# wuer5/OMGSR

Measured on AMD Instinct MI355X. Metric: SR images/sec, higher is better.
Workload: dtype fp16; 1 GPU; OMGSR-S 256->1024, batch=4/GPU, accurate tier (fp32 stream, fp16 MFMA operands + split corrections), tiled VAE 256/64; global_batch=4, latent_tile=64, tile_overlap=32, world_size=1, parallelism=dp1, weights=seeded random, SD2.1-base shapes

## Files before the change

include/omgsr_hip.h:

```cpp
#ifndef OMGSR_HIP_H
#define OMGSR_HIP_H

#include <stdint.h>

#ifdef __cplusplus
extern "C" {
#endif

#define OMGSR_E_BADARG (-1)
#define OMGSR_E_SHAPE (-2)
#define OMGSR_E_ARCH (-3)

#define OMGSR_ACT_NONE 0
#define OMGSR_ACT_SILU 1
#define OMGSR_ACT_GELU_TANH 2
#define OMGSR_ACT_GEGLU 3

#define OMGSR_OUT_BF16 0
#define OMGSR_OUT_F32 1

#define OMGSR_LAYOUT_NHWC 0
#define OMGSR_LAYOUT_T 1

#define OMGSR_EL_16 0
#define OMGSR_EL_F32 1
#define OMGSR_EL_SPLIT 2
#define OMGSR_EL_MX 3
#define OMGSR_EL_MX6 4
#define OMGSR_EL_MXFP8 5

#define OMGSR_DT_BF16 0
#define OMGSR_DT_F16 1
int omgsr_set_compute_dtype(int dtype);
int omgsr_get_compute_dtype(void);

int omgsr_abi_version(void);
int omgsr_check_device(void);
const char* omgsr_error_string(int code);

typedef struct omgsr_igemm_args {
    const void* in;
    const void* weight;
    const float* bias;
    const float* gate;
    const void* residual;
    void* out;
    int32_t N, H, W, Cin;
    int32_t Cout;
    int32_t Cout_pad, K_pad;
    int32_t R, S, stride, pad_top, pad_left, upsample;
    int32_t Ho, Wo;
    int32_t act, out_dtype, out_layout;
    int32_t t_rows, t_ld;
    int32_t out_ld;
    int32_t batch;
    int64_t in_bstride, w_bstride, out_bstride;
    float alpha;
    const void* weight_cm;
    void* workspace;
    float* gn_partial;
    int32_t gn_groups;
    int32_t gn_entries;
    int32_t res_el;
    int32_t in_split;
    int64_t sample_rows;
    int32_t out_lo_off;
    int32_t in_ld;
    int32_t w_split;
    const void* weight_ph;
    int32_t mx_chunks16;
    int32_t mx_scale_w1, mx_scale_a1, mx_scale_w2, mx_scale_a2;
    int32_t out_mx;
    int32_t group_tiles;
    uint32_t* overflow_flag;
    const float* gn_scale_shift;
    int32_t gn_nimg;
    int32_t gn_act;
    int32_t in_el;
    int32_t mx_fmt;
    int32_t mxf8;
    int32_t mxf8_reserved;
    const uint8_t* in_scale;
    const uint8_t* w_scale;
} omgsr_igemm_args;
int32_t omgsr_igemm_gn_fusable(const omgsr_igemm_args* a);
int32_t omgsr_igemm_out_mx6_ok(const omgsr_igemm_args* a);
int omgsr_groupnorm_scale_shift(const float* mean, const float* rstd, const float* gamma, const float* beta, float* out, int32_t nimg, int32_t C,
                                int32_t G, void* stream);
int omgsr_igemm(const omgsr_igemm_args* a, void* stream);
int omgsr_igemm_multi_plan(omgsr_igemm_args* args, int32_t count);
int omgsr_igemm_multi(const omgsr_igemm_args* args, int32_t count, void* stream);
int omgsr_set_batch_invariant(int on);
int64_t omgsr_igemm_workspace_bytes(const omgsr_igemm_args* a);
int32_t omgsr_igemm_gn_slots(const omgsr_igemm_args* a);
int32_t omgsr_igemm_gn_entries(const omgsr_igemm_args* a);

int omgsr_groupnorm_nchunk(int64_t HW);
int omgsr_groupnorm_stats(const void* x, float* partial, float* mean, float* rstd, float* var_out,
                          int32_t N, int64_t HW, int32_t C, int32_t G, float eps, int32_t x_el, void* stream);
int omgsr_groupnorm_finalize(const float* partial, float* mean, float* rstd, float* var_out, int32_t N,
                             int32_t nslot, int32_t G, int32_t entries, double count, float eps, void* stream);
int omgsr_groupnorm_partial(const void* x, float* partial, int32_t N, int64_t HW, int32_t C, int32_t G, int32_t x_el, void* stream);
#define OMGSR_GN_MAX_GROUPS 8
typedef struct omgsr_gn_merge_args {
    const float* partial[OMGSR_GN_MAX_GROUPS];
    double count[OMGSR_GN_MAX_GROUPS];
    float weight[OMGSR_GN_MAX_GROUPS];
    int32_t tiles[OMGSR_GN_MAX_GROUPS];
    int32_t nslot[OMGSR_GN_MAX_GROUPS];
    int32_t entries[OMGSR_GN_MAX_GROUPS];
    int32_t ngroups;
} omgsr_gn_merge_args;
int omgsr_groupnorm_finalize_merged(const omgsr_gn_merge_args* a, float* mean, float* rstd, float* var_out,
                                    int32_t N, int32_t G, float eps, void* stream);
int omgsr_groupnorm_apply(const void* x, void* y, const float* mean, const float* rstd,
                          const float* gamma, const float* beta, int32_t N, int64_t HW, int32_t C,
                          int32_t G, int32_t act, int32_t x_el, int32_t y_el, void* y2, int32_t y2_el, uint32_t* overflow_flag, void* stream);
int omgsr_groupnorm_apply_shared(const void* x, void* y, const float* mean, const float* rstd,
                                 const float* gamma, const float* beta, int32_t rows, int64_t HW, int32_t C,
                                 int32_t G, int32_t act, int32_t stat_rows, int32_t x_el, int32_t y_el, void* y2, int32_t y2_el,
                                 uint32_t* overflow_flag, void* stream);

int omgsr_layernorm(const void* x, void* y, const float* a, const float* b, int64_t rows, int32_t C,
                    float eps, int32_t x_el, int32_t y_el, void* stream);
int omgsr_quantize_mxfp8(const void* x, int32_t x_el, int64_t rows, int32_t K, int64_t x_ld, void* codes, void* scales, void* stream);
int omgsr_to_operand(const float* x, void* y, int64_t rows, int32_t C, int32_t y_el, uint32_t* overflow_flag, void* stream);
int omgsr_transpose_split(const float* x, void* y, int32_t B, int32_t L, int32_t C, int64_t ld, void* stream);

typedef struct omgsr_attn_args {
    const void* q; const void* k; const void* vt; void* o;
    int32_t B, H, D, Lq, Lk;
    int64_t q_ld, k_ld, vt_ld, o_ld;
    int64_t q_bstride, k_bstride, vt_bstride, o_bstride;
    float scale;
    int32_t o_lo_off;
    int32_t o_mx;
    int32_t q_lo_off;
    int32_t k_lo_off;
    int32_t p_split;
    int32_t reserved1;
    int64_t vt_lo_off;
    int32_t qkv_el;
    int32_t qkv_reserved;
    const uint8_t* q_scale;
    const uint8_t* k_scale;
    const uint8_t* vt_scale;
    int64_t q_sld, k_sld, vt_sld;
    int64_t q_sbstride, k_sbstride, vt_sbstride;
} omgsr_attn_args;
int omgsr_set_attention_defer_max(float log2_threshold);
int omgsr_attention(const omgsr_attn_args* a, void* stream);

int omgsr_softmax_rows(const float* s, void* p, int64_t rows, int32_t L, int32_t Lvalid, void* stream);
int omgsr_softmax_rows_split(const float* s, void* p, int64_t rows, int32_t L, int32_t Lvalid, void* stream);

int omgsr_rmsnorm_rope(void* x, const float* w, const float* w2, int32_t Lsplit, const float* cos_t, const float* sin_t, int32_t B,
                       int32_t L, int32_t H, int32_t D, int64_t ld, int32_t col0, int32_t pos0,
                       float eps, void* stream);
int omgsr_rmsnorm_rope_mxfp8(const void* x, const float* w, const float* w2, int32_t Lsplit, const float* cos_t, const float* sin_t, int32_t B,
                             int32_t L, int32_t H, int32_t D, int64_t ld, int32_t col0, int32_t pos0, float eps, void* codes, void* scales,
                             int64_t c_ld, int64_t s_ld, void* stream);

int omgsr_nchw_to_nhwc(const void* src, void* dst, int32_t N, int32_t C, int32_t H, int32_t W,
                       int32_t Cpad, int32_t src_dtype, int32_t dst_el, void* stream);
int omgsr_nhwc_to_nchw(const void* src, void* dst, int32_t N, int32_t C, int32_t H, int32_t W,
                       int32_t ld, int32_t dst_dtype, int32_t do_clamp, float lo, float hi, int32_t src_el, void* stream);
int omgsr_copy_channels(const void* src, void* dst, int64_t rows, int32_t C, int32_t src_ld,
                        int32_t dst_ld, int32_t dst_off, int32_t el, void* stream);
int omgsr_vae_sample(const void* moments, const float* eps, void* z, int64_t rows, int32_t C,
                     int32_t ld_out, float shift, float scale, int32_t el, void* stream);
int omgsr_axpby(const void* x, const void* y, void* out, int64_t n, float a, float b, float c, float d,
                int32_t bf16_steps, int32_t el, void* stream);
int omgsr_linear_f32(const float* x, const float* w, const float* b, float* y, int32_t rows, int32_t K, int32_t N,
                     int32_t silu_in, void* stream);
int omgsr_tile_accumulate(const void* tile, const float* w, float* acc, int32_t N, int32_t C,
                          int32_t th, int32_t tw, int32_t tile_ld, int32_t H, int32_t W, int32_t y0,
                          int32_t x0, int32_t tile_el, void* stream);
int omgsr_tile_normalise(const float* acc, const float* wsum, void* out, int32_t N, int64_t HW,
                         int32_t C, int32_t ld, int32_t out_el, void* stream);
int omgsr_crop_nhwc(const void* src, void* dst, int32_t N, int32_t H, int32_t W, int32_t C, int32_t y0,
                    int32_t x0, int32_t th, int32_t tw, int32_t el, void* stream);
int omgsr_paste_nhwc(const void* src, void* dst, int32_t N, int32_t C, int32_t sH, int32_t sW, int32_t sy0,
                     int32_t sx0, int32_t dH, int32_t dW, int32_t dy0, int32_t dx0, int32_t th, int32_t tw,
                     int32_t el, void* stream);
int omgsr_resize_nearest_exact_nhwc(const void* src, void* dst, int32_t N, int32_t H, int32_t W, int32_t C, int32_t Ho, int32_t Wo,
                                    float scale_y, float scale_x, int32_t el, void* stream);
int omgsr_flux_pack(const void* src, void* dst, int32_t N, int32_t H, int32_t W, int32_t C, int32_t ld,
                    int32_t dir, int32_t el, void* stream);

int omgsr_image_to_model_input(const uint8_t* img_hwc3, void* out_nhwc8, int32_t N, int32_t H, int32_t W, int32_t out_el, void* stream);
#define OMGSR_COLORFIX_NONE 0
#define OMGSR_COLORFIX_ADAIN 1
#define OMGSR_COLORFIX_WAVELET 2
int64_t omgsr_colorfix_workspace_bytes(int32_t N, int32_t H, int32_t W, int32_t method);
int omgsr_colorfix(const void* sr_nhwc, int32_t sr_ld, const uint8_t* src_hwc3, uint8_t* out_hwc3, void* workspace,
                   int32_t N, int32_t H, int32_t W, int32_t method, int32_t sr_el, void* stream);

int omgsr_resample_u8(const uint8_t* src, uint8_t* dst, const int32_t* bounds, const int32_t* kk, int32_t ksize,
                      int32_t N, int32_t Hin, int32_t Win, int32_t out_size, int32_t axis, void* stream);

int omgsr_timing_enable(int on);
int omgsr_timing_reset(void);
typedef struct omgsr_timing_entry { int32_t kind; float ms; double flops; double bytes; int64_t m, n, k; int32_t variant; int32_t stage; } omgsr_timing_entry;
int omgsr_timing_collect(omgsr_timing_entry* out, int cap);
int omgsr_timing_stage(int stage);
int omgsr_mfma_peak(int32_t iters, float* tflops, void* stream);

#ifdef __cplusplus
}
#endif
#endif
```

omgsr_amd/_lib.py:

```python
from __future__ import annotations

import ctypes as C
import os

import torch

from .build import lib_path

ABI_VERSION = 20


class OmgsrError(RuntimeError):
    pass


class IgemmArgs(C.Structure):
    _fields_ = [
        ("in_", C.c_void_p), ("weight", C.c_void_p), ("bias", C.c_void_p), ("gate", C.c_void_p),
        ("residual", C.c_void_p), ("out", C.c_void_p),
        ("N", C.c_int32), ("H", C.c_int32), ("W", C.c_int32), ("Cin", C.c_int32),
        ("Cout", C.c_int32), ("Cout_pad", C.c_int32), ("K_pad", C.c_int32),
        ("R", C.c_int32), ("S", C.c_int32), ("stride", C.c_int32), ("pad_top", C.c_int32),
        ("pad_left", C.c_int32), ("upsample", C.c_int32),
        ("Ho", C.c_int32), ("Wo", C.c_int32),
        ("act", C.c_int32), ("out_dtype", C.c_int32), ("out_layout", C.c_int32),
        ("t_rows", C.c_int32), ("t_ld", C.c_int32), ("out_ld", C.c_int32),
        ("batch", C.c_int32),
        ("in_bstride", C.c_int64), ("w_bstride", C.c_int64), ("out_bstride", C.c_int64),
        ("alpha", C.c_float), ("weight_cm", C.c_void_p), ("workspace", C.c_void_p),
        ("gn_partial", C.c_void_p), ("gn_groups", C.c_int32), ("gn_entries", C.c_int32),
        ("res_el", C.c_int32), ("in_split", C.c_int32), ("sample_rows", C.c_int64), ("out_lo_off", C.c_int32),
        ("in_ld", C.c_int32), ("w_split", C.c_int32), ("weight_ph", C.c_void_p), ("mx_chunks16", C.c_int32), ("mx_scale_w1", C.c_int32), ("mx_scale_a1", C.c_int32),
        ("mx_scale_w2", C.c_int32), ("mx_scale_a2", C.c_int32), ("out_mx", C.c_int32), ("group_tiles", C.c_int32), ("overflow_flag", C.c_void_p),
        ("gn_scale_shift", C.c_void_p), ("gn_nimg", C.c_int32), ("gn_act", C.c_int32), ("in_el", C.c_int32), ("mx_fmt", C.c_int32),
        ("mxf8", C.c_int32), ("mxf8_reserved", C.c_int32), ("in_scale", C.c_void_p), ("w_scale", C.c_void_p),
    ]


GN_MAX_GROUPS = 8


class GnMergeArgs(C.Structure):
    _fields_ = [("partial", C.c_void_p * GN_MAX_GROUPS), ("count", C.c_double * GN_MAX_GROUPS),
                ("weight", C.c_float * GN_MAX_GROUPS), ("tiles", C.c_int32 * GN_MAX_GROUPS),
                ("nslot", C.c_int32 * GN_MAX_GROUPS), ("entries", C.c_int32 * GN_MAX_GROUPS), ("ngroups", C.c_int32)]


class AttnArgs(C.Structure):
    _fields_ = [
        ("q", C.c_void_p), ("k", C.c_void_p), ("vt", C.c_void_p), ("o", C.c_void_p),
        ("B", C.c_int32), ("H", C.c_int32), ("D", C.c_int32), ("Lq", C.c_int32), ("Lk", C.c_int32),
        ("q_ld", C.c_int64), ("k_ld", C.c_int64), ("vt_ld", C.c_int64), ("o_ld", C.c_int64),
        ("q_bstride", C.c_int64), ("k_bstride", C.c_int64), ("vt_bstride", C.c_int64), ("o_bstride", C.c_int64),
        ("scale", C.c_float), ("o_lo_off", C.c_int32), ("o_mx", C.c_int32), ("q_lo_off", C.c_int32), ("k_lo_off", C.c_int32), ("p_split", C.c_int32),
        ("reserved1", C.c_int32), ("vt_lo_off", C.c_int64),
        ("qkv_el", C.c_int32), ("qkv_reserved", C.c_int32), ("q_scale", C.c_void_p), ("k_scale", C.c_void_p), ("vt_scale", C.c_void_p),
        ("q_sld", C.c_int64), ("k_sld", C.c_int64), ("vt_sld", C.c_int64), ("q_sbstride", C.c_int64), ("k_sbstride", C.c_int64),
        ("vt_sbstride", C.c_int64),
    ]


class TimingEntry(C.Structure):
    _fields_ = [("kind", C.c_int32), ("ms", C.c_float), ("flops", C.c_double), ("bytes", C.c_double),
                ("m", C.c_int64), ("n", C.c_int64), ("k", C.c_int64), ("variant", C.c_int32), ("stage", C.c_int32)]


_P, _I, _L, _F = C.c_void_p, C.c_int32, C.c_int64, C.c_float

SIGNATURES = {
    "omgsr_abi_version": (C.c_int, []),
    "omgsr_check_device": (C.c_int, []),
    "omgsr_set_compute_dtype": (C.c_int, [C.c_int]),
    "omgsr_get_compute_dtype": (C.c_int, []),
    "omgsr_error_string": (C.c_char_p, [C.c_int]),
    "omgsr_igemm": (C.c_int, [C.POINTER(IgemmArgs), _P]),
    "omgsr_igemm_multi_plan": (C.c_int, [C.POINTER(IgemmArgs), _I]),
    "omgsr_igemm_multi": (C.c_int, [C.POINTER(IgemmArgs), _I, _P]),
    "omgsr_set_batch_invariant": (C.c_int, [C.c_int]),
    "omgsr_set_attention_defer_max": (C.c_int, [C.c_float]),
    "omgsr_igemm_workspace_bytes": (C.c_int64, [C.POINTER(IgemmArgs)]),
    "omgsr_igemm_gn_slots": (C.c_int32, [C.POINTER(IgemmArgs)]),
    "omgsr_igemm_gn_entries": (C.c_int32, [C.POINTER(IgemmArgs)]),
    "omgsr_igemm_gn_fusable": (C.c_int32, [C.POINTER(IgemmArgs)]),
    "omgsr_igemm_out_mx6_ok": (C.c_int32, [C.POINTER(IgemmArgs)]),
    "omgsr_groupnorm_scale_shift": (C.c_int, [_P, _P, _P, _P, _P, _I, _I, _I, _P]),
    "omgsr_groupnorm_finalize": (C.c_int, [_P, _P, _P, _P, _I, _I, _I, _I, C.c_double, _F, _P]),
    "omgsr_groupnorm_partial": (C.c_int, [_P, _P, _I, _L, _I, _I, _I, _P]),
    "omgsr_groupnorm_finalize_merged": (C.c_int, [C.POINTER(GnMergeArgs), _P, _P, _P, _I, _I, _F, _P]),
    "omgsr_groupnorm_apply_shared": (C.c_int, [_P, _P, _P, _P, _P, _P, _I, _L, _I, _I, _I, _I, _I, _I, _P, _I, _P, _P]),
    "omgsr_image_to_model_input": (C.c_int, [_P, _P, _I, _I, _I, _I, _P]),
    "omgsr_colorfix_workspace_bytes": (C.c_int64, [_I, _I, _I, _I]),
    "omgsr_colorfix": (C.c_int, [_P, _I, _P, _P, _P, _I, _I, _I, _I, _I, _P]),
    "omgsr_groupnorm_nchunk": (C.c_int, [_L]),
    "omgsr_groupnorm_stats": (C.c_int, [_P, _P, _P, _P, _P, _I, _L, _I, _I, _F, _I, _P]),
    "omgsr_groupnorm_apply": (C.c_int, [_P, _P, _P, _P, _P, _P, _I, _L, _I, _I, _I, _I, _I, _P, _I, _P, _P]),
    "omgsr_layernorm": (C.c_int, [_P, _P, _P, _P, _L, _I, _F, _I, _I, _P]),
    "omgsr_resize_nearest_exact_nhwc": (C.c_int, [_P, _P, _I, _I, _I, _I, _I, _I, _F, _F, _I, _P]),
    "omgsr_transpose_split": (C.c_int, [_P, _P, _I, _I, _I, _L, _P]),
    "omgsr_to_operand": (C.c_int, [_P, _P, _L, _I, _I, _P, _P]),
    "omgsr_quantize_mxfp8": (C.c_int, [_P, _I, _L, _I, _L, _P, _P, _P]),
    "omgsr_attention": (C.c_int, [C.POINTER(AttnArgs), _P]),
    "omgsr_softmax_rows": (C.c_int, [_P, _P, _L, _I, _I, _P]),
    "omgsr_softmax_rows_split": (C.c_int, [_P, _P, _L, _I, _I, _P]),
    "omgsr_rmsnorm_rope": (C.c_int, [_P, _P, _P, _I, _P, _P, _I, _I, _I, _I, _L, _I, _I, _F, _P]),
    "omgsr_rmsnorm_rope_mxfp8": (C.c_int, [_P, _P, _P, _I, _P, _P, _I, _I, _I, _I, _L, _I, _I, _F, _P, _P, _L, _L, _P]),
    "omgsr_nchw_to_nhwc": (C.c_int, [_P, _P, _I, _I, _I, _I, _I, _I, _I, _P]),
    "omgsr_nhwc_to_nchw": (C.c_int, [_P, _P, _I, _I, _I, _I, _I, _I, _I, _F, _F, _I, _P]),
    "omgsr_copy_channels": (C.c_int, [_P, _P, _L, _I, _I, _I, _I, _I, _P]),
    "omgsr_vae_sample": (C.c_int, [_P, _P, _P, _L, _I, _I, _F, _F, _I, _P]),
    "omgsr_axpby": (C.c_int, [_P, _P, _P, _L, _F, _F, _F, _F, _I, _I, _P]),
    "omgsr_linear_f32": (C.c_int, [_P, _P, _P, _P, _I, _I, _I, _I, _P]),
    "omgsr_tile_accumulate": (C.c_int, [_P, _P, _P, _I, _I, _I, _I, _I, _I, _I, _I, _I, _I, _P]),
    "omgsr_tile_normalise": (C.c_int, [_P, _P, _P, _I, _L, _I, _I, _I, _P]),
    "omgsr_crop_nhwc": (C.c_int, [_P, _P, _I, _I, _I, _I, _I, _I, _I, _I, _I, _P]),
    "omgsr_paste_nhwc": (C.c_int, [_P, _P] + [_I] * 13 + [_P]),
    "omgsr_flux_pack": (C.c_int, [_P, _P, _I, _I, _I, _I, _I, _I, _I, _P]),
    "omgsr_resample_u8": (C.c_int, [_P, _P, _P, _P, _I, _I, _I, _I, _I, _I, _P]),
    "omgsr_timing_enable": (C.c_int, [C.c_int]),
    "omgsr_timing_reset": (C.c_int, []),
    "omgsr_timing_stage": (C.c_int, [C.c_int]),
    "omgsr_timing_collect": (C.c_int, [C.POINTER(TimingEntry), C.c_int]),
    "omgsr_mfma_peak": (C.c_int, [_I, C.POINTER(C.c_float), _P]),
}

_lib = None


def load(path: str | None = None):
    global _lib
    if _lib is not None:
        return _lib
    path = path or os.environ.get("OMGSR_HIP_LIB") or lib_path()
    if not os.path.isfile(path):
        raise OmgsrError(
            f"{path} not found: build it with `python -m omgsr_amd.build` (hipcc --offload-arch=gfx950). "
            "The OMGSR MI355X path has no CPU fallback.")
    lib = C.CDLL(path)
    for name, (res, args) in SIGNATURES.items():
        try:
            fn = getattr(lib, name)
        except AttributeError as e:
            raise OmgsrError(f"{path} does not export {name}") from e
        fn.restype = res
        fn.argtypes = args
    if lib.omgsr_abi_version() != ABI_VERSION:
        raise OmgsrError(f"ABI mismatch: library {lib.omgsr_abi_version()} vs binding {ABI_VERSION}; rebuild")
    _lib = lib
    return lib


def check(code: int, what: str = "") -> None:
    if code != 0:
        msg = load().omgsr_error_string(code)
        raise OmgsrError(f"{what}: {msg.decode() if msg else code} (code {code})")
```

omgsr_amd/csrc/elementwise.hip:

```cpp
#include "common.hip.h"
#include "../../include/omgsr_hip.h"
#include "timing.hip.h"
#include <string.h>
#include <type_traits>

namespace omgsr {
TimingState& timing_state() { static TimingState s; return s; }
static int g_compute_dtype = 0;
int compute_dtype() { return g_compute_dtype; }
}

namespace {

template <typename T> OMGSR_DEVINL float round_to(float x) { return (float)(T)x; }

template <typename SRC, typename T, int DEL>
__global__ void nchw_to_nhwc_kernel(const SRC* __restrict__ src, void* __restrict__ dst, int N, int C, int64_t HW, int Cpad) {
    const int ng = Cpad >> 3;
    const int64_t i = (int64_t)blockIdx.x * blockDim.x + threadIdx.x;
    const int64_t total = (int64_t)N * HW * ng;
    if (i >= total) return;
    const int g = (int)(i % ng);
    const int64_t pix = i / ng;
    const int n = (int)(pix / HW);
// ... 60 lines not shown
    __shared__ float tile[64][65];
    const int b = blockIdx.z, l0 = blockIdx.x * 64, c0 = blockIdx.y * 64;
    const float* xb = x + (int64_t)b * L * C;
    for (int i = threadIdx.x; i < 64 * 64; i += 256) {
        const int l = i >> 6, c = i & 63;
        tile[l][c] = (l0 + l < L && c0 + c < C) ? xb[(int64_t)(l0 + l) * C + c0 + c] : 0.0f;
    }
    __syncthreads();
    T* yb = y + (int64_t)b * 2 * C * ld;
    for (int i = threadIdx.x; i < 64 * 8; i += 256) {
        const int c = i >> 3, g = (i & 7) * 8;
        if (c0 + c >= C || l0 + g >= L) continue;
        float hi[8], lo[8];
#pragma unroll
        for (int e = 0; e < 8; ++e) {
            const float v = tile[g + e][c];
            const T h = (T)v;
            hi[e] = (float)h;
            lo[e] = v - hi[e];
        }
        T* dh = yb + (int64_t)(c0 + c) * ld + l0 + g;
        T* dl = dh + (int64_t)C * ld;
        if (l0 + g + 8 <= L) {
            *reinterpret_cast<u32x4_t*>(dh) = pack8<T>(hi);
            *reinterpret_cast<u32x4_t*>(dl) = pack8<T>(lo);
        } else {
            for (int e = 0; e < 8 && l0 + g + e < L; ++e) { dh[e] = (T)hi[e]; dl[e] = (T)lo[e]; }
        }
    }
}

template <typename T>
__global__ void vae_sample_kernel(const T* __restrict__ mom, const float* __restrict__ eps, T* __restrict__ z, int64_t rows,
                                  int C, int ld_out, float shift, float scale) {
    const int64_t i = (int64_t)blockIdx.x * blockDim.x + threadIdx.x;
    if (i >= rows * ld_out) return;
    const int c = (int)(i % ld_out);
    const int64_t r = i / ld_out;
    float out = 0.0f;
    if (c < C) {
        const float mu = (float)mom[r * 2 * C + c];
        float lv = (float)mom[r * 2 * C + C + c];
        lv = fminf(fmaxf(lv, -30.0f), 20.0f);
        out = ((mu + __expf(0.5f * lv) * eps[r * C + c]) - shift) * scale;
    }
    z[i] = (T)out;
}

template <typename T>
__global__ void axpby_kernel(const T* __restrict__ x, const T* __restrict__ y, T* __restrict__ out, int64_t n, float a,
                             float b, float c, float d, int steps) {
    const int64_t i = (int64_t)blockIdx.x * blockDim.x + threadIdx.x;
    if (i >= n) return;
    const float xv = (float)x[i];
    const float yv = y ? (float)y[i] : 0.0f;
    float v;
    if (steps) {
        const float t0 = (a == 1.0f) ? xv : round_to<T>(xv * a);
        const float t1 = y ? round_to<T>(yv * b) : 0.0f;
        v = y ? round_to<T>(t0 + t1) : t0;
        if (c != 0.0f) v = round_to<T>(v + c);
        if (d != 1.0f) v = round_to<T>(v * d);
    } else {
        v = (xv * a + yv * b + c) * d;
    }
    out[i] = (T)v;
}

template <typename T>
__global__ void tile_accumulate_kernel(const T* __restrict__ tile, const float* __restrict__ w, float* __restrict__ acc, int N,
                                       int C, int th, int tw, int tile_ld, int H, int W, int y0, int x0) {
    const int64_t i = (int64_t)blockIdx.x * blockDim.x + threadIdx.x;
    const int64_t total = (int64_t)N * th * tw * C;
    if (i >= total) return;
    const int c = (int)(i % C);
    int64_t r = i / C;
    const int x = (int)(r % tw); r /= tw;
    const int y = (int)(r % th);
    const int n = (int)(r / th);
    const float wv = w[y * tw + x];
    const float tv = tile ? (float)tile[(((int64_t)n * th + y) * tw + x) * tile_ld + c] : 1.0f;
    acc[(((int64_t)n * H + y0 + y) * W + x0 + x) * C + c] += tv * wv;
}

template <typename T>
__global__ void tile_normalise_kernel(const float* __restrict__ acc, const float* __restrict__ wsum, T* __restrict__ out, int N,
                                      int64_t HW, int C, int ld) {
    const int64_t i = (int64_t)blockIdx.x * blockDim.x + threadIdx.x;
    if (i >= (int64_t)N * HW * ld) return;
    const int c = (int)(i % ld);
    const int64_t pix = i / ld;
    float v = 0.0f;
    if (c < C) v = acc[pix * C + c] / wsum[pix % HW];
    out[i] = (T)v;
}

__global__ void crop_kernel(const u32x4_t* __restrict__ src, u32x4_t* __restrict__ dst, int N, int H, int W, int ng, int y0, int x0, int th,
                            int tw) {
    const int64_t i = (int64_t)blockIdx.x * blockDim.x + threadIdx.x;
    if (i >= (int64_t)N * th * tw * ng) return;
    const int g = (int)(i % ng);
    int64_t r = i / ng;
    const int x = (int)(r % tw); r /= tw;
    const int y = (int)(r % th);
    const int n = (int)(r / th);
    dst[i] = src[(((int64_t)n * H + y0 + y) * W + x0 + x) * ng + g];
}

__global__ void resize_nearest_exact_kernel(const u32x4_t* __restrict__ src, u32x4_t* __restrict__ dst, int N, int H, int W, int ng, int Ho, int Wo,
                                            float sy, float sx) {
    const int64_t i = (int64_t)blockIdx.x * blockDim.x + threadIdx.x;
    if (i >= (int64_t)N * Ho * Wo * ng) return;
    const int g = (int)(i % ng);
    int64_t r = i / ng;
    const int x = (int)(r % Wo); r /= Wo;
    const int y = (int)(r % Ho);
    const int n = (int)(r / Ho);
    int iy = (int)floorf((float)(((double)y + 0.5) * (double)sy)), ix = (int)floorf((float)(((double)x + 0.5) * (double)sx));
    iy = iy < H - 1 ? iy : H - 1;
    ix = ix < W - 1 ? ix : W - 1;
    dst[i] = src[(((int64_t)n * H + iy) * W + ix) * ng + g];
}

__global__ void paste_kernel(const u32x4_t* __restrict__ src, u32x4_t* __restrict__ dst, int N, int ng, int sH, int sW, int sy0, int sx0,
                             int dH, int dW, int dy0, int dx0, int th, int tw) {
    const int64_t i = (int64_t)blockIdx.x * blockDim.x + threadIdx.x;
    if (i >= (int64_t)N * th * tw * ng) return;
    const int g = (int)(i % ng);
    int64_t r = i / ng;
    const int x = (int)(r % tw); r /= tw;
    const int y = (int)(r % th);
    const int n = (int)(r / th);
    dst[(((int64_t)n * dH + dy0 + y) * dW + dx0 + x) * ng + g] = src[(((int64_t)n * sH + sy0 + y) * sW + sx0 + x) * ng + g];
}

template <typename E>
__global__ void flux_pack_kernel(const E* __restrict__ src, E* __restrict__ dst, int N, int H, int W, int C, int ld, int dir) {
    const int64_t i = (int64_t)blockIdx.x * blockDim.x + threadIdx.x;
    if (i >= (int64_t)N * H * W * C) return;
    const int c = (int)(i % C);
    int64_t r = i / C;
    const int x = (int)(r % W); r /= W;
    const int y = (int)(r % H);
    const int n = (int)(r / H);
    const int64_t nhwc = (((int64_t)n * H + y) * W + x) * ld + c;
    const int64_t tok = (((int64_t)n * (H / 2) + (y >> 1)) * (W / 2) + (x >> 1)) * (4 * C) + c * 4 + (y & 1) * 2 + (x & 1);
    if (dir == 0) dst[tok] = src[nhwc]; else dst[nhwc] = src[tok];
}

inline dim3 grid1d(int64_t total, int block = 256) { return dim3((unsigned)((total + block - 1) / block)); }

}

extern "C" int omgsr_abi_version(void) { return 20; }

extern "C" int omgsr_set_compute_dtype(int dtype) {
    if (dtype != OMGSR_DT_BF16 && dtype != OMGSR_DT_F16) return OMGSR_E_BADARG;
    omgsr::g_compute_dtype = dtype;
    return 0;
}
extern "C" int omgsr_get_compute_dtype(void) { return omgsr::g_compute_dtype; }

extern "C" int omgsr_check_device(void) {
    int dev = 0;
    if (hipGetDevice(&dev) != hipSuccess) return OMGSR_E_ARCH;
    hipDeviceProp_t prop;
    if (hipGetDeviceProperties(&prop, dev) != hipSuccess) return OMGSR_E_ARCH;
    return strncmp(prop.gcnArchName, "gfx950", 6) == 0 ? 0 : OMGSR_E_ARCH;
}

extern "C" const char* omgsr_error_string(int code) {
    switch (code) {
        case 0: return "success";
        case OMGSR_E_BADARG: return "omgsr: bad argument (null pointer or non-positive dimension)";
        case OMGSR_E_SHAPE: return "omgsr: shape/alignment not supported by the gfx950 kernel";
        case OMGSR_E_ARCH: return "omgsr: current device is not gfx950 (MI355X)";
        default: return code > 0 ? hipGetErrorString((hipError_t)code) : "omgsr: unknown error";
    }
}

extern "C" int omgsr_nchw_to_nhwc(const void* src, void* dst, int32_t N, int32_t C, int32_t H, int32_t W, int32_t Cpad,
                                  int32_t src_dtype, int32_t dst_el, void* stream) {
    if (!src || !dst || N <= 0 || C <= 0 || H <= 0 || W <= 0) return OMGSR_E_BADARG;
    if ((Cpad & 7) || Cpad < C) return OMGSR_E_SHAPE;
    hipStream_t st = (hipStream_t)stream;
    const int64_t HW = (int64_t)H * W, total = (int64_t)N * HW * (Cpad >> 3);
    omgsr::TimingScope ts(OMGSR_TK_ELT, 0.0, 2.0 * N * HW * (C + Cpad), st);
    if (dst_el != OMGSR_EL_16 && dst_el != OMGSR_EL_F32) return OMGSR_E_BADARG;
    if (src_dtype == 1 && dst_el == OMGSR_EL_F32) OMGSR_DISPATCH_T(hipLaunchKernelGGL((nchw_to_nhwc_kernel<float, T, 1>), grid1d(total), dim3(256), 0, st, (const float*)src, dst, N, C, HW, Cpad));
    else if (src_dtype == 1) OMGSR_DISPATCH_T(hipLaunchKernelGGL((nchw_to_nhwc_kernel<float, T, 0>), grid1d(total), dim3(256), 0, st, (const float*)src, dst, N, C, HW, Cpad));
    else if (dst_el == OMGSR_EL_F32) OMGSR_DISPATCH_T(hipLaunchKernelGGL((nchw_to_nhwc_kernel<T, T, 1>), grid1d(total), dim3(256), 0, st, (const T*)src, dst, N, C, HW, Cpad));
    else OMGSR_DISPATCH_T(hipLaunchKernelGGL((nchw_to_nhwc_kernel<T, T, 0>), grid1d(total), dim3(256), 0, st, (const T*)src, dst, N, C, HW, Cpad));
    return (int)hipGetLastError();
}

extern "C" int omgsr_nhwc_to_nchw(const void* src, void* dst, int32_t N, int32_t C, int32_t H, int32_t W, int32_t ld,
                                  int32_t dst_dtype, int32_t do_clamp, float lo, float hi, int32_t src_el, void* stream) {
    if (!src || !dst || N <= 0 || C <= 0 || H <= 0 || W <= 0 || ld < C) return OMGSR_E_BADARG;
    hipStream_t st = (hipStream_t)stream;
    const int64_t HW = (int64_t)H * W, total = (int64_t)N * C * HW;
    omgsr::TimingScope ts(OMGSR_TK_ELT, 0.0, 4.0 * total, st);
    if (src_el == OMGSR_EL_F32) {
        if (dst_dtype == 1) hipLaunchKernelGGL((nhwc_to_nchw_kernel<float, float>), grid1d(total), dim3(256), 0, st, (const float*)src, (float*)dst, N, C, HW, ld, do_clamp, lo, hi);
        else OMGSR_DISPATCH_T(hipLaunchKernelGGL((nhwc_to_nchw_kernel<T, float>), grid1d(total), dim3(256), 0, st, (const float*)src, (T*)dst, N, C, HW, ld, do_clamp, lo, hi));
    } else if (dst_dtype == 1) OMGSR_DISPATCH_T(hipLaunchKernelGGL((nhwc_to_nchw_kernel<float, T>), grid1d(total), dim3(256), 0, st, (const T*)src, (float*)dst, N, C, HW, ld, do_clamp, lo, hi));
    else OMGSR_DISPATCH_T(hipLaunchKernelGGL((nhwc_to_nchw_kernel<T, T>), grid1d(total), dim3(256), 0, st, (const T*)src, (T*)dst, N, C, HW, ld, do_clamp, lo, hi));
    return (int)hipGetLastError();
}

extern "C" int omgsr_copy_channels(const void* src, void* dst, int64_t rows, int32_t C, int32_t src_ld, int32_t dst_ld,
                                   int32_t dst_off, int32_t el, void* stream) {
    if (!src || !dst || rows <= 0 || C <= 0 || (el != OMGSR_EL_16 && el != OMGSR_EL_F32)) return OMGSR_E_BADARG;
    if ((C & 7) || (src_ld & 7) || (dst_ld & 7) || (dst_off & 7) || dst_off + C > dst_ld || src_ld < C) return OMGSR_E_SHAPE;
    hipStream_t st = (hipStream_t)stream;
    const int sh = el == OMGSR_EL_F32 ? 2 : 3;
    omgsr::TimingScope ts(OMGSR_TK_ELT, 0.0, (el == OMGSR_EL_F32 ? 8.0 : 4.0) * rows * C, st);
    hipLaunchKernelGGL(copy_channels_kernel, grid1d(rows * (C >> sh)), dim3(256), 0, st, (const u32x4_t*)src, (u32x4_t*)dst, rows, C >> sh,
                       src_ld >> sh, dst_ld >> sh, dst_off >> sh);
    return (int)hipGetLastError();
}

extern "C" int omgsr_to_operand(const float* x, void* y, int64_t rows, int32_t C, int32_t y_el, uint32_t* overflow_flag, void* stream) {
    if (!x || !y || rows <= 0 || C <= 0 || (y_el != OMGSR_EL_16 && y_el != OMGSR_EL_SPLIT && y_el != OMGSR_EL_MX && y_el != OMGSR_EL_MX6)) return OMGSR_E_BADARG;
    if (C & 7) return OMGSR_E_SHAPE;
    hipStream_t st = (hipStream_t)stream;
    omgsr::TimingScope ts(OMGSR_TK_ELT, 0.0, (y_el == OMGSR_EL_16 ? 6.0 : 8.0) * rows * C, st);
    if (y_el == OMGSR_EL_MX || y_el == OMGSR_EL_MX6) {
        if ((C & 63) || omgsr::compute_dtype() != 1) return OMGSR_E_SHAPE;
        if (y_el == OMGSR_EL_MX6) hipLaunchKernelGGL((to_operand_kernel<f16_t, 4>), grid1d(rows * (C >> 3)), dim3(256), 0, st, x, y, rows, C, overflow_flag);
        else hipLaunchKernelGGL((to_operand_kernel<f16_t, 3>), grid1d(rows * (C >> 3)), dim3(256), 0, st, x, y, rows, C, overflow_flag);
    } else if (y_el == OMGSR_EL_SPLIT) OMGSR_DISPATCH_T(hipLaunchKernelGGL((to_operand_kernel<T, 2>), grid1d(rows * (C >> 3)), dim3(256), 0, st, x, y, rows, C, overflow_flag));
    else OMGSR_DISPATCH_T(hipLaunchKernelGGL((to_operand_kernel<T, 0>), grid1d(rows * (C >> 3)), dim3(256), 0, st, x, y, rows, C, overflow_flag));
    return (int)hipGetLastError();
}

extern "C" int omgsr_transpose_split(const float* x, void* y, int32_t B, int32_t L, int32_t C, int64_t ld, void* stream) {
    if (!x || !y || B <= 0 || L <= 0 || C <= 0) return OMGSR_E_BADARG;
    if (ld < L || (ld & 7)) return OMGSR_E_SHAPE;
    hipStream_t st = (hipStream_t)stream;
    omgsr::TimingScope ts(OMGSR_TK_ELT, 0.0, 8.0 * (double)B * L * C, st);
    const dim3 grid((unsigned)((L + 63) / 64), (unsigned)((C + 63) / 64), (unsigned)B);
    OMGSR_DISPATCH_T(hipLaunchKernelGGL(transpose_split_kernel<T>, grid, dim3(256), 0, st, x, (T*)y, L, C, ld));
    return (int)hipGetLastError();
}

extern "C" int omgsr_vae_sample(const void* moments, const float* eps, void* z, int64_t rows, int32_t C, int32_t ld_out,
                                float shift, float scale, int32_t el, void* stream) {
    if (!moments || !eps || !z || rows <= 0 || C <= 0 || ld_out < C) return OMGSR_E_BADARG;
    hipStream_t st = (hipStream_t)stream;
    omgsr::TimingScope ts(OMGSR_TK_ELT, 0.0, 10.0 * rows * C, st);
    if (el == OMGSR_EL_F32) hipLaunchKernelGGL(vae_sample_kernel<float>, grid1d(rows * ld_out), dim3(256), 0, st, (const float*)moments, eps, (float*)z, rows, C, ld_out, shift, scale);
    else OMGSR_DISPATCH_T(hipLaunchKernelGGL(vae_sample_kernel<T>, grid1d(rows * ld_out), dim3(256), 0, st, (const T*)moments, eps, (T*)z, rows, C, ld_out, shift, scale));
    return (int)hipGetLastError();
}

extern "C" int omgsr_axpby(const void* x, const void* y, void* out, int64_t n, float a, float b, float c, float d,
                           int32_t bf16_steps, int32_t el, void* stream) {
    if (!x || !out || n <= 0) return OMGSR_E_BADARG;
    hipStream_t st = (hipStream_t)stream;
    omgsr::TimingScope ts(OMGSR_TK_ELT, 0.0, 6.0 * n, st);
    if (el == OMGSR_EL_F32) hipLaunchKernelGGL(axpby_kernel<float>, grid1d(n), dim3(256), 0, st, (const float*)x, (const float*)y, (float*)out, n, a, b, c, d, 0);
    else OMGSR_DISPATCH_T(hipLaunchKernelGGL(axpby_kernel<T>, grid1d(n), dim3(256), 0, st, (const T*)x, (const T*)y, (T*)out, n, a, b, c, d, bf16_steps));
    return (int)hipGetLastError();
}

namespace {
__global__ __launch_bounds__(256) void linear_f32_kernel(const float* __restrict__ x, const float* __restrict__ w, const float* __restrict__ b,
                                                         float* __restrict__ y, int rows, int K, int N, int silu_in) {
    const int64_t o = (int64_t)blockIdx.x * 4 + (threadIdx.x >> 6);
    if (o >= (int64_t)rows * N) return;
    const int r = (int)(o / N), n = (int)(o % N), lane = threadIdx.x & 63;
    const float* xr = x + (int64_t)r * K;
    const float* wn = w + (int64_t)n * K;
    float s = 0.f;
    for (int k = lane; k < K; k += 64) {
        float xv = xr[k];
        if (silu_in) xv = xv / (1.0f + expf(-xv));
        s = fmaf(xv, wn[k], s);
    }
    s = wave_sum(s);
    if (lane == 0) y[o] = s + (b ? b[n] : 0.f);
}
}

extern "C" int omgsr_linear_f32(const float* x, const float* w, const float* b, float* y, int32_t rows, int32_t K, int32_t N,
                                int32_t silu_in, void* stream) {
    if (!x || !w || !y || rows <= 0 || K <= 0 || N <= 0) return OMGSR_E_BADARG;
    hipStream_t st = (hipStream_t)stream;
    omgsr::TimingScope ts(OMGSR_TK_ELT, 2.0 * rows * K * N, 4.0 * ((double)N * K + (double)rows * (K + N)), st);
    const int64_t outs = (int64_t)rows * N;
    hipLaunchKernelGGL(linear_f32_kernel, dim3((unsigned)((outs + 3) / 4)), dim3(256), 0, st, x, w, b, y, rows, K, N, silu_in);
    return (int)hipGetLastError();
}

extern "C" int omgsr_tile_accumulate(const void* tile, const float* w, float* acc, int32_t N, int32_t C, int32_t th, int32_t tw,
                                     int32_t tile_ld, int32_t H, int32_t W, int32_t y0, int32_t x0, int32_t tile_el, void* stream) {
    if (!w || !acc || N <= 0 || C <= 0 || th <= 0 || tw <= 0) return OMGSR_E_BADARG;
    if (y0 < 0 || x0 < 0 || y0 + th > H || x0 + tw > W || (tile && tile_ld < C)) return OMGSR_E_SHAPE;
    hipStream_t st = (hipStream_t)stream;
    const int64_t total = (int64_t)N * th * tw * C;
    omgsr::TimingScope ts(OMGSR_TK_ELT, 0.0, 10.0 * total, st);
    if (tile_el == OMGSR_EL_F32) hipLaunchKernelGGL(tile_accumulate_kernel<float>, grid1d(total), dim3(256), 0, st, (const float*)tile, w, acc, N, C, th, tw, tile_ld, H, W, y0, x0);
    else OMGSR_DISPATCH_T(hipLaunchKernelGGL(tile_accumulate_kernel<T>, grid1d(total), dim3(256), 0, st, (const T*)tile, w, acc, N, C, th, tw, tile_ld, H, W, y0, x0));
    return (int)hipGetLastError();
}

extern "C" int omgsr_tile_normalise(const float* acc, const float* wsum, void* out, int32_t N, int64_t HW, int32_t C, int32_t ld,
// ... 85 lines not shown
```

omgsr_amd/csrc/norm.hip:

```cpp
#include "common.hip.h"
#include <type_traits>
#include "../../include/omgsr_hip.h"
#include "timing.hip.h"
#include "mxfp8.hip.h"
#include <stdlib.h>

namespace {

constexpr int GN_PPC = 256;
static inline int gn_ppc(const int64_t HW) { return HW >= 32768 ? GN_PPC : (HW >= 8192 ? 128 : (HW >= 2048 ? 32 : 16)); }

template <typename T, bool XF32>
__global__ __launch_bounds__(256) void gn_partial_kernel(const void* __restrict__ x, float* __restrict__ partial,
                                                          int64_t HW, int C, int G, int nchunk, int ppc) {
    extern __shared__ __attribute__((aligned(16))) float gn_lds[];
    const int t = threadIdx.x;
    const int n = blockIdx.y, chunk = blockIdx.x;
    const int nch8 = C >> 3;
    const int TP = nch8 < 256 ? nch8 : 256;
    const int P = 256 / TP;
    float* csum = gn_lds;
    float* csq = gn_lds + P * C;
    const int64_t p0 = (int64_t)chunk * ppc;
    const int npx = (int)((HW - p0) < ppc ? (HW - p0) : ppc);
    if (t < TP * P) {
        const int pl = t / TP;
        const int64_t base = ((int64_t)n * HW + p0) * C;
        for (int c8 = t % TP; c8 < nch8; c8 += TP) {
            float s[8], q[8];
#pragma unroll
            for (int e = 0; e < 8; ++e) { s[e] = 0.0f; q[e] = 0.0f; }
            int px = pl;
            for (; px + 3 * P < npx; px += 4 * P) {
                float r[4][8];
#pragma unroll
                for (int u = 0; u < 4; ++u) load8<T, XF32>(x, base + (int64_t)(px + u * P) * C + c8 * 8, r[u]);
#pragma unroll
                for (int u = 0; u < 4; ++u) {
#pragma unroll
                    for (int e = 0; e < 8; ++e) { s[e] += r[u][e]; q[e] += r[u][e] * r[u][e]; }
                }
            }
            for (; px < npx; px += P) {
                float f[8];
                load8<T, XF32>(x, base + (int64_t)px * C + c8 * 8, f);
#pragma unroll
                for (int e = 0; e < 8; ++e) { s[e] += f[e]; q[e] += f[e] * f[e]; }
            }
#pragma unroll
            for (int e = 0; e < 8; ++e) {
                csum[pl * C + c8 * 8 + e] = s[e];
                csq[pl * C + c8 * 8 + e] = q[e];
            }
        }
    }
    __syncthreads();
    const int cpg = C / G;
    if (t < G) {
        float s = 0.0f, q = 0.0f;
        for (int c = t * cpg; c < (t + 1) * cpg; ++c)
            for (int pl = 0; pl < P; ++pl) { s += csum[pl * C + c]; q += csq[pl * C + c]; }
        float* o = partial + (((int64_t)n * nchunk + chunk) * G + t) * 2;
        o[0] = s; o[1] = q;
    }
}

__global__ void gn_finalize_kernel(const float* __restrict__ partial, float* __restrict__ mean, float* __restrict__ rstd,
                                   float* __restrict__ var_out, int N, int G, int nchunk, double count, float eps, int entries) {
    const int i = blockIdx.x;
    const int lane = threadIdx.x;
    const int n = i / G, g = i - n * G;
    double s = 0.0, q = 0.0;
    const int epg = entries / G;
    for (int c = lane; c < nchunk; c += 64) {
        const float* p = partial + (((int64_t)n * nchunk + c) * entries + g * epg) * 2;
        for (int j = 0; j < epg; ++j) { s += (double)p[2 * j]; q += (double)p[2 * j + 1]; }
    }
#pragma unroll
    for (int o = 32; o > 0; o >>= 1) { s += __shfl_xor(s, o); q += __shfl_xor(q, o); }
    if (lane != 0) return;
    const double m = s / count;
    double v = q / count - m * m;
    if (v < 0.0) v = 0.0;
    mean[i] = (float)m;
    rstd[i] = (float)(1.0 / sqrt(v + (double)eps));
    if (var_out) var_out[i] = (float)v;
}

template <typename T>
__global__ __launch_bounds__(256) void gn_apply_kernel(const T* __restrict__ x, T* __restrict__ y,
                                                        const float* __restrict__ mean, const float* __restrict__ rstd,
                                                        const float* __restrict__ gamma, const float* __restrict__ beta,
                                                        int64_t HW, int C, int G, int act, int64_t px_per_block, int stat_rows) {
    extern __shared__ __attribute__((aligned(16))) float gn_lds[];
    float* sc = gn_lds;
    float* sh = gn_lds + C;
    const int t = threadIdx.x, n = blockIdx.y;
    const int ns = n % stat_rows;
    const int cpg = C / G;
    for (int c = t; c < C; c += 256) {
        const int g = c / cpg;
        const float r = rstd[ns * G + g], m = mean[ns * G + g];
        const float a = r * (gamma ? gamma[c] : 1.0f);
        sc[c] = a;
        sh[c] = (beta ? beta[c] : 0.0f) - m * a;
    }
    __syncthreads();
    const int nch8 = C >> 3;
    const int64_t p0 = (int64_t)blockIdx.x * px_per_block;
    int64_t p1 = p0 + px_per_block; if (p1 > HW) p1 = HW;
    const int total = (int)((p1 - p0) * nch8);
    const T* xb = x + ((int64_t)n * HW + p0) * C;
    T* yb = y + ((int64_t)n * HW + p0) * C;
    const int step8 = 256 % nch8;
    int c8 = t % nch8;
    int i = t;
    for (; i + 256 < total; i += 512) {
        const u32x4_t r0 = *reinterpret_cast<const u32x4_t*>(xb + (int64_t)i * 8);
        const u32x4_t r1 = *reinterpret_cast<const u32x4_t*>(xb + (int64_t)(i + 256) * 8);
        int c8b = c8 + step8; if (c8b >= nch8) c8b -= nch8;
        float f[8], h[8];
        unpack8<T>(r0, f); unpack8<T>(r1, h);
        const f32x4_t* sa = reinterpret_cast<const f32x4_t*>(sc + c8 * 8);
        const f32x4_t* ha = reinterpret_cast<const f32x4_t*>(sh + c8 * 8);
        const f32x4_t* sb = reinterpret_cast<const f32x4_t*>(sc + c8b * 8);
        const f32x4_t* hb = reinterpret_cast<const f32x4_t*>(sh + c8b * 8);
        const f32x4_t sa0 = sa[0], sa1 = sa[1], ha0 = ha[0], ha1 = ha[1], sb0 = sb[0], sb1 = sb[1], hb0 = hb[0], hb1 = hb[1];
#pragma unroll
        for (int e = 0; e < 8; ++e) {
            const float v = f[e] * (e < 4 ? sa0[e & 3] : sa1[e & 3]) + (e < 4 ? ha0[e & 3] : ha1[e & 3]);
            const float w = h[e] * (e < 4 ? sb0[e & 3] : sb1[e & 3]) + (e < 4 ? hb0[e & 3] : hb1[e & 3]);
            f[e] = (act == OMGSR_ACT_SILU) ? silu_f(v) : v;
            h[e] = (act == OMGSR_ACT_SILU) ? silu_f(w) : w;
        }
        *reinterpret_cast<u32x4_t*>(yb + (int64_t)i * 8) = pack8<T>(f);
        *reinterpret_cast<u32x4_t*>(yb + (int64_t)(i + 256) * 8) = pack8<T>(h);
        c8 = c8b + step8; if (c8 >= nch8) c8 -= nch8;
    }
    for (; i < total; i += 256) {
        float f[8];
        unpack8<T>(*reinterpret_cast<const u32x4_t*>(xb + (int64_t)i * 8), f);
#pragma unroll
        for (int e = 0; e < 8; ++e) {
            const float v = f[e] * sc[c8 * 8 + e] + sh[c8 * 8 + e];
            f[e] = (act == OMGSR_ACT_SILU) ? silu_f(v) : v;
        }
        *reinterpret_cast<u32x4_t*>(yb + (int64_t)i * 8) = pack8<T>(f);
        c8 += step8; if (c8 >= nch8) c8 -= nch8;
    }
}

template <typename T, bool XF32, int YEL, int Y2EL = -1>
__global__ __launch_bounds__(256) void gn_apply_any_kernel(const void* __restrict__ x, void* __restrict__ y,
                                                            const float* __restrict__ mean, const float* __restrict__ rstd,
                                                            const float* __restrict__ gamma, const float* __restrict__ beta,
                                                            int64_t HW, int C, int G, int act, int64_t px_per_block, int stat_rows,
                                                            void* __restrict__ y2 = nullptr, unsigned* __restrict__ ovf = nullptr) {
    extern __shared__ __attribute__((aligned(16))) float gn_lds[];
    float amax = 0.0f;
    auto note8 = [&](const float (&v)[8]) {
        if constexpr (Y2EL >= 0 && std::is_same<T, f16_t>::value) {
#pragma unroll
            for (int e = 0; e < 8; ++e) amax = fmaxf(amax, fabsf(v[e]));
        }
    };
    float* sc = gn_lds;
    float* sh = gn_lds + C;
    const int t = threadIdx.x, n = blockIdx.y;
    const int ns = n % stat_rows;
    const int cpg = C / G;
    for (int c = t; c < C; c += 256) {
        const int g = c / cpg;
        const float r = rstd[ns * G + g], m = mean[ns * G + g];
        const float a = r * (gamma ? gamma[c] : 1.0f);
        sc[c] = a;
        sh[c] = (beta ? beta[c] : 0.0f) - m * a;
    }
    __syncthreads();
    const int nch8 = C >> 3;
    const int64_t p0 = (int64_t)blockIdx.x * px_per_block;
    int64_t p1 = p0 + px_per_block; if (p1 > HW) p1 = HW;
    const int total = (int)((p1 - p0) * nch8);
    const int64_t pix0 = (int64_t)n * HW + p0;
    const int step8 = 256 % nch8, stepp = 256 / nch8;
    const int ldy = YEL == 2 ? 2 * C : C;
    int c8 = t % nch8, px = t / nch8;
    auto advance = [&](int& cc, int& pp) {
        cc += step8; pp += stepp;
        if (cc >= nch8) { cc -= nch8; ++pp; }
    };
    auto transform = [&](float (&f)[8], const int cc) {
        const f32x4_t* sa = reinterpret_cast<const f32x4_t*>(sc + cc * 8);
        const f32x4_t* ha = reinterpret_cast<const f32x4_t*>(sh + cc * 8);
        const f32x4_t sa0 = sa[0], sa1 = sa[1], ha0 = ha[0], ha1 = ha[1];
#pragma unroll
        for (int e = 0; e < 8; ++e) {
            const float v = f[e] * (e < 4 ? sa0[e & 3] : sa1[e & 3]) + (e < 4 ? ha0[e & 3] : ha1[e & 3]);
            f[e] = (act == OMGSR_ACT_SILU) ? silu_f(v) : v;
        }
    };
    auto put = [&](const int64_t pix, const int cc8, const float (&v)[8]) {
        if constexpr (YEL == 3) store8_mx<T>(y, pix * 4 * C, C, cc8 * 8, v);
        else if constexpr (YEL == 4) store8_mx6<T>(y, pix * 4 * C, C, cc8 * 8, v);
        else store8<T, YEL>(y, pix * ldy + cc8 * 8, C, v);
    };
    auto put2 = [&](const int64_t pix, const int cc8, const float (&v)[8]) {
        if constexpr (Y2EL == 3) store8_mx<T>(y2, pix * 4 * C, C, cc8 * 8, v);
        else if constexpr (Y2EL >= 0) store8<T, Y2EL>(y2, pix * (Y2EL == 2 ? 2 * C : C) + cc8 * 8, C, v);
    };
    int i = t;
    for (; i + 256 < total; i += 512) {
        int c8b = c8, pxb = px;
        advance(c8b, pxb);
        float f[8], h[8];
        load8<T, XF32>(x, (pix0 + px) * C + c8 * 8, f);
        load8<T, XF32>(x, (pix0 + pxb) * C + c8b * 8, h);
        if constexpr (Y2EL >= 0) {
            note8(f); note8(h);
            put2(pix0 + px, c8, f);
            put2(pix0 + pxb, c8b, h);
        }
        transform(f, c8);
        transform(h, c8b);
        put(pix0 + px, c8, f);
        put(pix0 + pxb, c8b, h);
        c8 = c8b; px = pxb;
        advance(c8, px);
    }
    for (; i < total; i += 256) {
        float f[8];
        load8<T, XF32>(x, (pix0 + px) * C + c8 * 8, f);
        if constexpr (Y2EL >= 0) { note8(f); put2(pix0 + px, c8, f); }
        transform(f, c8);
        put(pix0 + px, c8, f);
        advance(c8, px);
    }
    if constexpr (Y2EL >= 0 && std::is_same<T, f16_t>::value) {
        if (ovf && __any(amax > 65504.0f) && (t & 63) == 0) atomicOr(ovf, 1u);
        if (Y2EL == 3 && ovf && __any(amax > 448.0f) && (t & 63) == 0) atomicOr(ovf, 2u);
    }
}

__global__ void gn_scale_shift_kernel(const float* __restrict__ mean, const float* __restrict__ rstd, const float* __restrict__ gamma,
                                      const float* __restrict__ beta, float* __restrict__ out, int total, int C, int G) {
    const int i = blockIdx.x * blockDim.x + threadIdx.x;
    if (i >= total) return;
    const int n = i / C, c = i - n * C, g = c / (C / G);
    const float r = rstd[n * G + g], m = mean[n * G + g];
    const float a = r * (gamma ? gamma[c] : 1.0f);
    *reinterpret_cast<f32x2_t*>(out + 2 * (int64_t)i) = (f32x2_t){a, (beta ? beta[c] : 0.0f) - m * a};
}
OMGSR_DEVINL void load_affine8(const float* __restrict__ v, const int c, const float dflt, float (&o)[8]) {
    if (v) {
        const f32x4_t lo = *reinterpret_cast<const f32x4_t*>(v + c), hi = *reinterpret_cast<const f32x4_t*>(v + c + 4);
#pragma unroll
        for (int e = 0; e < 4; ++e) { o[e] = lo[e]; o[4 + e] = hi[e]; }
    } else {
#pragma unroll
        for (int e = 0; e < 8; ++e) o[e] = dflt;
    }
}

template <typename T, int MAXCH, int RPW, bool XF32 = false, int YEL = 0>
__global__ __launch_bounds__(256) void layernorm_kernel(const void* __restrict__ x, void* __restrict__ y,
                                                         const float* __restrict__ a, const float* __restrict__ b,
                                                         int64_t rows, int C, float eps) {
    const int lane = threadIdx.x & 63;
    const int64_t row0 = ((int64_t)blockIdx.x * 4 + (threadIdx.x >> 6)) * RPW;
    if (row0 >= rows) return;
    const int nch8 = C >> 3;
    float f[RPW][MAXCH][8];
    float s[RPW];
#pragma unroll
    for (int r = 0; r < RPW; ++r) {
        s[r] = 0.0f;
        const bool live = row0 + r < rows;
#pragma unroll
        for (int i = 0; i < MAXCH; ++i) {
            const int c8 = lane + 64 * i;
#pragma unroll
            for (int e = 0; e < 8; ++e) f[r][i][e] = 0.0f;
            if (live && c8 < nch8) load8<T, XF32>(x, (row0 + r) * C + c8 * 8, f[r][i]);
        }
    }
    constexpr bool PRE = MAXCH <= 3;
    float av[PRE ? MAXCH : 1][8], bv[PRE ? MAXCH : 1][8];
    if constexpr (PRE) {
#pragma unroll
        for (int i = 0; i < MAXCH; ++i) {
            const int c8 = lane + 64 * i;
            load_affine8(c8 < nch8 ? a : nullptr, c8 * 8, 1.0f, av[i]);
            load_affine8(c8 < nch8 ? b : nullptr, c8 * 8, 0.0f, bv[i]);
        }
    }
#pragma unroll
    for (int r = 0; r < RPW; ++r)
#pragma unroll
        for (int i = 0; i < MAXCH; ++i)
#pragma unroll
            for (int e = 0; e < 8; ++e) s[r] += f[r][i][e];
    float mu[RPW], q[RPW];
#pragma unroll
    for (int o = 32; o > 0; o >>= 1)
#pragma unroll
        for (int r = 0; r < RPW; ++r) s[r] += __shfl_xor(s[r], o);
#pragma unroll
    for (int r = 0; r < RPW; ++r) {
        mu[r] = s[r] / (float)C;
        q[r] = 0.0f;
#pragma unroll
        for (int i = 0; i < MAXCH; ++i) {
            if (lane + 64 * i < nch8) {
#pragma unroll
                for (int e = 0; e < 8; ++e) { const float d = f[r][i][e] - mu[r]; q[r] += d * d; }
            }
        }
    }
#pragma unroll
    for (int o = 32; o > 0; o >>= 1)
#pragma unroll
        for (int r = 0; r < RPW; ++r) q[r] += __shfl_xor(q[r], o);
#pragma unroll
    for (int r = 0; r < RPW; ++r) {
        if (row0 + r >= rows) break;
        const float rs = rsqrtf(q[r] / (float)C + eps);
#pragma unroll
        for (int i = 0; i < MAXCH; ++i) {
            const int c8 = lane + 64 * i;
            if (c8 < nch8) {
                float o8[8], ga[8], be[8];
                if constexpr (!PRE) { load_affine8(a, c8 * 8, 1.0f, ga); load_affine8(b, c8 * 8, 0.0f, be); }
#pragma unroll
                for (int e = 0; e < 8; ++e)
                    o8[e] = (f[r][i][e] - mu[r]) * rs * (PRE ? av[PRE ? i : 0][e] : ga[e]) + (PRE ? bv[PRE ? i : 0][e] : be[e]);
                if constexpr (YEL == 3) {
                    if constexpr (std::is_same<T, f16_t>::value) store8_mx<T>(y, (row0 + r) * 4 * (int64_t)C, C, c8 * 8, o8);
                } else store8<T, YEL>(y, (row0 + r) * (YEL == 2 ? 2 * C : C) + c8 * 8, C, o8);
            }
        }
    }
}

template <typename T, int MAXV, bool XF32 = false, int YEL = 0>
__global__ __launch_bounds__(256) void layernorm_block_kernel(const void* __restrict__ x, void* __restrict__ y,
                                                               const float* __restrict__ a, const float* __restrict__ b,
                                                               int C, float eps) {
    __shared__ float red[2][4];
    const int t = threadIdx.x, lane = t & 63, wave = t >> 6;
    const int64_t row = blockIdx.x;
    const int nch8 = C >> 3;
    float f[MAXV][8];
    float s = 0.0f;
#pragma unroll
    for (int i = 0; i < MAXV; ++i) {
        const int c8 = t + 256 * i;
#pragma unroll
        for (int e = 0; e < 8; ++e) f[i][e] = 0.0f;
        if (c8 < nch8) load8<T, XF32>(x, row * C + c8 * 8, f[i]);
#pragma unroll
        for (int e = 0; e < 8; ++e) s += f[i][e];
    }
    s = wave_sum(s);
    if (lane == 0) red[0][wave] = s;
    __syncthreads();
    const float mu = (red[0][0] + red[0][1] + red[0][2] + red[0][3]) / (float)C;
    float q = 0.0f;
#pragma unroll
    for (int i = 0; i < MAXV; ++i) {
        if (t + 256 * i < nch8) {
#pragma unroll
            for (int e = 0; e < 8; ++e) { const float d = f[i][e] - mu; q += d * d; }
        }
    }
    q = wave_sum(q);
    if (lane == 0) red[1][wave] = q;
    __syncthreads();
    const float rs = rsqrtf((red[1][0] + red[1][1] + red[1][2] + red[1][3]) / (float)C + eps);
#pragma unroll
    for (int i = 0; i < MAXV; ++i) {
        const int c8 = t + 256 * i;
        if (c8 < nch8) {
            float o8[8], ga[8], be[8];
            load_affine8(a, c8 * 8, 1.0f, ga); load_affine8(b, c8 * 8, 0.0f, be);
#pragma unroll
            for (int e = 0; e < 8; ++e) o8[e] = (f[i][e] - mu) * rs * ga[e] + be[e];
            if constexpr (YEL == 3) {
                if constexpr (std::is_same<T, f16_t>::value) store8_mx<T>(y, row * 4 * (int64_t)C, C, c8 * 8, o8);
            } else store8<T, YEL>(y, row * (YEL == 2 ? 2 * C : C) + c8 * 8, C, o8);
        }
    }
}

template <typename T, int MAXV, bool SPLIT = false>
// ... 65 lines not shown
    float f[8];
    unpack8<T>(*reinterpret_cast<const u32x4_t*>(px), f);
    float q = 0.0f;
#pragma unroll
    for (int e = 0; e < 8; ++e) q += f[e] * f[e];
#pragma unroll
    for (int o = 8; o > 0; o >>= 1) q += __shfl_xor(q, o);
    const float r = rsqrtf(q / (float)D + eps);
    const float* wt = (w2 && (int)(row % L) >= Lsplit) ? w2 : w;
    float wv[8];
    load_affine8(wt, h * D + sub * 8, 1.0f, wv);
#pragma unroll
    for (int e = 0; e < 8; ++e) f[e] = f[e] * r * wv[e];
    if (cos_t) {
        const int pos = pos0 + (int)(row % L);
        float cp[8], sp[8];
        load_affine8(cos_t, (int)((int64_t)pos * D) + sub * 8, 1.0f, cp);
        load_affine8(sin_t, (int)((int64_t)pos * D) + sub * 8, 0.0f, sp);
#pragma unroll
        for (int e = 0; e < 8; e += 2) {
            const float a = f[e], b = f[e + 1];
            f[e] = a * cp[e] - b * sp[e];
            f[e + 1] = b * cp[e + 1] + a * sp[e + 1];
        }
    }
    *reinterpret_cast<u32x4_t*>(px) = pack8<T>(f);
}

__global__ __launch_bounds__(256) void rmsnorm_rope_mxfp8_kernel(const bf16_t* __restrict__ x, const float* __restrict__ w, const float* __restrict__ w2,
                                                                  int Lsplit, const float* __restrict__ cos_t, const float* __restrict__ sin_t,
                                                                  int64_t rows, int L, int H, int D, int64_t ld, int col0, int pos0, float eps,
                                                                  unsigned char* __restrict__ codes, unsigned char* __restrict__ scales, int64_t c_ld,
                                                                  int64_t s_ld) {
    const int64_t gid = (int64_t)blockIdx.x * 16 + (threadIdx.x >> 4);
    if (gid >= rows * H) return;
    const int sub = threadIdx.x & 15;
    const int64_t row = gid / H;
    const int h = (int)(gid - row * H);
    const bf16_t* px = x + row * ld + col0 + h * D + sub * 8;
    float f[8];
    unpack8<bf16_t>(*reinterpret_cast<const u32x4_t*>(px), f);
    float q = 0.0f;
#pragma unroll
    for (int e = 0; e < 8; ++e) q += f[e] * f[e];
#pragma unroll
    for (int o = 8; o > 0; o >>= 1) q += __shfl_xor(q, o);
    const float r = rsqrtf(q / (float)D + eps);
    const float* wt = (w2 && (int)(row % L) >= Lsplit) ? w2 : w;
    float wv[8];
    load_affine8(wt, h * D + sub * 8, 1.0f, wv);
#pragma unroll
    for (int e = 0; e < 8; ++e) f[e] = f[e] * r * wv[e];
    if (cos_t) {
        const int pos = pos0 + (int)(row % L);
        float cp[8], sp[8];
        load_affine8(cos_t, (int)((int64_t)pos * D) + sub * 8, 1.0f, cp);
        load_affine8(sin_t, (int)((int64_t)pos * D) + sub * 8, 0.0f, sp);
#pragma unroll
        for (int e = 0; e < 8; e += 2) {
            const float a = f[e], b = f[e + 1];
            f[e] = a * cp[e] - b * sp[e];
            f[e + 1] = b * cp[e + 1] + a * sp[e + 1];
        }
    }
    float mx = 0.0f;
#pragma unroll
    for (int e = 0; e < 8; ++e) mx = fmaxf(mx, fabsf(f[e]));
    mx = fmaxf(mx, __shfl_xor(mx, 1));
    mx = fmaxf(mx, __shfl_xor(mx, 2));
    const int s = mxfp8_scale(mx);
    u32x2_t out = {0u, 0u};
#pragma unroll
    for (int e = 0; e < 8; ++e) out[e >> 2] |= mxfp8_code(f[e], s) << (8 * (e & 3));
    *reinterpret_cast<u32x2_t*>(codes + row * c_ld + col0 + h * D + sub * 8) = out;
    if ((sub & 3) == 0) scales[row * s_ld + col0 / 32 + h * (D / 32) + (sub >> 2)] = (unsigned char)s;
}

}

extern "C" int omgsr_groupnorm_scale_shift(const float* mean, const float* rstd, const float* gamma, const float* beta, float* out, int32_t nimg,
                                           int32_t C, int32_t G, void* stream) {
    if (!mean || !rstd || !out || nimg <= 0 || C <= 0 || G <= 0 || (C % G)) return OMGSR_E_BADARG;
    const int total = nimg * C;
    hipLaunchKernelGGL(gn_scale_shift_kernel, dim3((total + 255) / 256), dim3(256), 0, (hipStream_t)stream, mean, rstd, gamma, beta, out, total, C, G);
    return (int)hipGetLastError();
}

extern "C" int omgsr_groupnorm_nchunk(int64_t HW) { const int ppc = gn_ppc(HW); return (int)((HW + ppc - 1) / ppc); }

extern "C" int omgsr_groupnorm_stats(const void* x, float* partial, float* mean, float* rstd, float* var_out,
                                     int32_t N, int64_t HW, int32_t C, int32_t G, float eps, int32_t x_el, void* stream) {
    if (!x || !partial || !mean || !rstd || N <= 0 || HW <= 0 || C <= 0 || G <= 0) return OMGSR_E_BADARG;
    if ((C & 7) || (C % G) || G > 256 || C > 8192) return OMGSR_E_SHAPE;
    hipStream_t st = (hipStream_t)stream;
    const int nchunk = omgsr_groupnorm_nchunk(HW);
    omgsr::TimingScope ts(OMGSR_TK_GN, 0.0, (x_el == OMGSR_EL_F32 ? 4.0 : 2.0) * N * (double)HW * C, st);
    const int tp = (C >> 3) < 256 ? (C >> 3) : 256;
    const size_t lds = 2 * (size_t)(256 / tp) * C * sizeof(float);
    if (x_el == OMGSR_EL_F32) OMGSR_DISPATCH_T(hipLaunchKernelGGL((gn_partial_kernel<T, true>), dim3(nchunk, N), dim3(256), lds, st, x, partial, HW, C, G, nchunk, gn_ppc(HW)));
    else OMGSR_DISPATCH_T(hipLaunchKernelGGL((gn_partial_kernel<T, false>), dim3(nchunk, N), dim3(256), lds, st, x, partial, HW, C, G, nchunk, gn_ppc(HW)));
    const int tot = N * G;
    hipLaunchKernelGGL(gn_finalize_kernel, dim3(tot), dim3(64), 0, st, partial, mean, rstd, var_out,
                       N, G, nchunk, (double)HW * (C / G), eps, G);
    return (int)hipGetLastError();
}

extern "C" int omgsr_groupnorm_finalize(const float* partial, float* mean, float* rstd, float* var_out, int32_t N,
                                        int32_t nslot, int32_t G, int32_t entries, double count, float eps, void* stream) {
    if (!partial || !mean || !rstd || N <= 0 || nslot <= 0 || G <= 0 || count <= 0.0 || entries < G || (entries % G)) return OMGSR_E_BADARG;
    hipLaunchKernelGGL(gn_finalize_kernel, dim3(N * G), dim3(64), 0, (hipStream_t)stream, partial, mean, rstd, var_out,
                       N, G, nslot, count, eps, entries);
    return (int)hipGetLastError();
}

namespace {
__global__ __launch_bounds__(256) void gn_finalize_merged_kernel(const omgsr_gn_merge_args a, float* __restrict__ mean, float* __restrict__ rstd,
                                                                  float* __restrict__ var_out, int N, int G, float eps) {
    __shared__ double red[4][2];
    const int i = blockIdx.x, lane = threadIdx.x & 63, wave = threadIdx.x >> 6;
    const int n = i / G, g = i - n * G;
    double m_acc = 0.0, v_acc = 0.0;
    int pair = 0;
    for (int k = 0; k < a.ngroups; ++k) {
        const float* partial = a.partial[k];
        const int nslot = a.nslot[k];
        for (int t = 0; t < a.tiles[k]; ++t, ++pair) {
            if ((pair & 3) != wave) continue;
            const int row = t * N + n;
            double s = 0.0, q = 0.0;
            const int entries = a.entries[k], epg = entries / G;
            for (int c = lane; c < nslot; c += 64) {
                const float* pp = partial + (((int64_t)row * nslot + c) * entries + g * epg) * 2;
                for (int j = 0; j < epg; ++j) { s += (double)pp[2 * j]; q += (double)pp[2 * j + 1]; }
            }
#pragma unroll
            for (int o = 32; o > 0; o >>= 1) { s += __shfl_xor(s, o); q += __shfl_xor(q, o); }
            const double m = s / a.count[k];
            double v = q / a.count[k] - m * m;
            if (v < 0.0) v = 0.0;
            m_acc += (double)a.weight[k] * m;
            v_acc += (double)a.weight[k] * v;
        }
    }
    if (lane == 0) { red[wave][0] = m_acc; red[wave][1] = v_acc; }
    __syncthreads();
    if (threadIdx.x != 0) return;
    const double mm = ((red[0][0] + red[1][0]) + red[2][0]) + red[3][0];
    const double vv = ((red[0][1] + red[1][1]) + red[2][1]) + red[3][1];
    mean[i] = (float)mm;
    rstd[i] = (float)(1.0 / sqrt(vv + (double)eps));
    if (var_out) var_out[i] = (float)vv;
}

}
namespace {
int gn_apply_launch(const void* x, void* y, const float* mean, const float* rstd, const float* gamma,
                    const float* beta, int32_t N, int64_t HW, int32_t C, int32_t G, int32_t act, int32_t stat_rows, int32_t x_el,
                    int32_t y_el, void* y2, int32_t y2_el, uint32_t* ovf, void* stream);
}

extern "C" int omgsr_groupnorm_partial(const void* x, float* partial, int32_t N, int64_t HW, int32_t C, int32_t G, int32_t x_el, void* stream) {
    if (!x || !partial || N <= 0 || HW <= 0 || C <= 0 || G <= 0) return OMGSR_E_BADARG;
    if ((C & 7) || (C % G) || G > 256 || C > 8192) return OMGSR_E_SHAPE;
    hipStream_t st = (hipStream_t)stream;
    const int nchunk = omgsr_groupnorm_nchunk(HW);
    omgsr::TimingScope ts(OMGSR_TK_GN, 0.0, (x_el == OMGSR_EL_F32 ? 4.0 : 2.0) * N * (double)HW * C, st);
    const int tp = (C >> 3) < 256 ? (C >> 3) : 256;
    const size_t lds = 2 * (size_t)(256 / tp) * C * sizeof(float);
    if (x_el == OMGSR_EL_F32) OMGSR_DISPATCH_T(hipLaunchKernelGGL((gn_partial_kernel<T, true>), dim3(nchunk, N), dim3(256), lds, st, x, partial, HW, C, G, nchunk, gn_ppc(HW)));
    else OMGSR_DISPATCH_T(hipLaunchKernelGGL((gn_partial_kernel<T, false>), dim3(nchunk, N), dim3(256), lds, st, x, partial, HW, C, G, nchunk, gn_ppc(HW)));
    return (int)hipGetLastError();
}

extern "C" int omgsr_groupnorm_finalize_merged(const omgsr_gn_merge_args* a, float* mean, float* rstd, float* var_out,
                                               int32_t N, int32_t G, float eps, void* stream) {
    if (!a || !mean || !rstd || N <= 0 || G <= 0 || a->ngroups <= 0 || a->ngroups > OMGSR_GN_MAX_GROUPS) return OMGSR_E_BADARG;
    for (int k = 0; k < a->ngroups; ++k)
        if (!a->partial[k] || a->tiles[k] <= 0 || a->nslot[k] <= 0 || a->count[k] <= 0.0 || a->entries[k] < G || (a->entries[k] % G)) return OMGSR_E_BADARG;
    hipLaunchKernelGGL(gn_finalize_merged_kernel, dim3(N * G), dim3(256), 0, (hipStream_t)stream, *a, mean, rstd, var_out, N, G, eps);
    return (int)hipGetLastError();
}

extern "C" int omgsr_groupnorm_apply_shared(const void* x, void* y, const float* mean, const float* rstd, const float* gamma,
                                            const float* beta, int32_t rows, int64_t HW, int32_t C, int32_t G, int32_t act,
                                            int32_t stat_rows, int32_t x_el, int32_t y_el, void* y2, int32_t y2_el, uint32_t* overflow_flag,
                                            void* stream) {
    if (stat_rows <= 0 || rows % stat_rows) return OMGSR_E_BADARG;
    return gn_apply_launch(x, y, mean, rstd, gamma, beta, rows, HW, C, G, act, stat_rows, x_el, y_el, y2, y2_el, overflow_flag, stream);
}

extern "C" int omgsr_groupnorm_apply(const void* x, void* y, const float* mean, const float* rstd, const float* gamma,
                                     const float* beta, int32_t N, int64_t HW, int32_t C, int32_t G, int32_t act,
                                     int32_t x_el, int32_t y_el, void* y2, int32_t y2_el, uint32_t* overflow_flag, void* stream) {
    return gn_apply_launch(x, y, mean, rstd, gamma, beta, N, HW, C, G, act, N, x_el, y_el, y2, y2_el, overflow_flag, stream);
}

namespace {
int gn_apply_launch(const void* x, void* y, const float* mean, const float* rstd, const float* gamma,
                    const float* beta, int32_t N, int64_t HW, int32_t C, int32_t G, int32_t act, int32_t stat_rows, int32_t x_el,
                    int32_t y_el, void* y2, int32_t y2_el, uint32_t* ovf, void* stream) {
    if (!x || !y || !mean || !rstd || N <= 0 || HW <= 0 || C <= 0 || G <= 0) return OMGSR_E_BADARG;
    if ((x_el != OMGSR_EL_16 && x_el != OMGSR_EL_F32) || (y_el != OMGSR_EL_16 && y_el != OMGSR_EL_SPLIT && y_el != OMGSR_EL_MX && y_el != OMGSR_EL_MX6)) return OMGSR_E_BADARG;
    if ((y_el == OMGSR_EL_MX || y_el == OMGSR_EL_MX6) && ((C & 63) || omgsr::compute_dtype() != 1)) return OMGSR_E_SHAPE;
    if (y2 && (x_el != OMGSR_EL_F32 || (y2_el != OMGSR_EL_16 && y2_el != OMGSR_EL_SPLIT && y2_el != OMGSR_EL_MX))) return OMGSR_E_BADARG;
    if (y2 && y2_el == OMGSR_EL_MX && ((C & 63) || omgsr::compute_dtype() != 1)) return OMGSR_E_SHAPE;
    if ((C & 7) || (C % G) || C > 8192) return OMGSR_E_SHAPE;
    if (act != OMGSR_ACT_NONE && act != OMGSR_ACT_SILU) return OMGSR_E_BADARG;
    hipStream_t st = (hipStream_t)stream;
    static const char* ppe = getenv("OMGSR_GN_BLOCK_ELEMS");
    static const int64_t belems = ppe ? atol(ppe) : 16384;
    int64_t ppb = (belems + C - 1) / C;
    if (ppb < 1) ppb = 1;
    if (((HW + ppb - 1) / ppb) * N < 512) {
        ppb = (HW * N + 511) / 512;
        if (ppb < 8) ppb = 8;
    }
    const int nblk = (int)((HW + ppb - 1) / ppb);
    omgsr::TimingScope ts(OMGSR_TK_GN, 0.0, ((x_el == OMGSR_EL_F32 ? 4.0 : 2.0) + (y_el == OMGSR_EL_16 ? 2.0 : 4.0) +
                                             (y2 ? (y2_el == OMGSR_EL_16 ? 2.0 : 4.0) : 0.0)) * N * (double)HW * C, st);
    const size_t lds = 2 * C * sizeof(float);
    const dim3 grid(nblk, N);
#define OMGSR_GN_ANY2(YE, Y2) OMGSR_DISPATCH_T(hipLaunchKernelGGL((gn_apply_any_kernel<T, true, YE, Y2>), grid, dim3(256), lds, st, x, y, mean, rstd, gamma, beta, HW, C, G, act, ppb, stat_rows, y2, ovf))
#define OMGSR_GN_ANY(XF, YE) OMGSR_DISPATCH_T(hipLaunchKernelGGL((gn_apply_any_kernel<T, XF, YE>), grid, dim3(256), lds, st, x, y, mean, rstd, gamma, beta, HW, C, G, act, ppb, stat_rows))
    if (y_el == OMGSR_EL_MX6) {
        using T = f16_t;
#define OMGSR_GN_6(XF, Y2) hipLaunchKernelGGL((gn_apply_any_kernel<T, XF, 4, Y2>), grid, dim3(256), lds, st, x, y, mean, rstd, gamma, beta, HW, C, G, act, ppb, stat_rows, y2, ovf)
        if (y2 && y2_el == OMGSR_EL_MX) OMGSR_GN_6(true, 3);
        else if (y2 && y2_el == OMGSR_EL_SPLIT) OMGSR_GN_6(true, 2);
        else if (y2) OMGSR_GN_6(true, 0);
        else if (x_el == OMGSR_EL_F32) hipLaunchKernelGGL((gn_apply_any_kernel<T, true, 4>), grid, dim3(256), lds, st, x, y, mean, rstd, gamma, beta, HW, C, G, act, ppb, stat_rows, nullptr, nullptr);
        else hipLaunchKernelGGL((gn_apply_any_kernel<T, false, 4>), grid, dim3(256), lds, st, x, y, mean, rstd, gamma, beta, HW, C, G, act, ppb, stat_rows, nullptr, nullptr);
#undef OMGSR_GN_6
    } else if (y2 && y2_el == OMGSR_EL_MX) {
        using T = f16_t;
        if (y_el == OMGSR_EL_MX) hipLaunchKernelGGL((gn_apply_any_kernel<T, true, 3, 3>), grid, dim3(256), lds, st, x, y, mean, rstd, gamma, beta, HW, C, G, act, ppb, stat_rows, y2, ovf);
        else if (y_el == OMGSR_EL_SPLIT) hipLaunchKernelGGL((gn_apply_any_kernel<T, true, 2, 3>), grid, dim3(256), lds, st, x, y, mean, rstd, gamma, beta, HW, C, G, act, ppb, stat_rows, y2, ovf);
        else hipLaunchKernelGGL((gn_apply_any_kernel<T, true, 0, 3>), grid, dim3(256), lds, st, x, y, mean, rstd, gamma, beta, HW, C, G, act, ppb, stat_rows, y2, ovf);
    } else if (y_el == OMGSR_EL_MX) {
        using T = f16_t;
        if (y2 && y2_el == OMGSR_EL_SPLIT) hipLaunchKernelGGL((gn_apply_any_kernel<T, true, 3, 2>), grid, dim3(256), lds, st, x, y, mean, rstd, gamma, beta, HW, C, G, act, ppb, stat_rows, y2, ovf);
        else if (y2) hipLaunchKernelGGL((gn_apply_any_kernel<T, true, 3, 0>), grid, dim3(256), lds, st, x, y, mean, rstd, gamma, beta, HW, C, G, act, ppb, stat_rows, y2, ovf);
        else if (x_el == OMGSR_EL_F32) hipLaunchKernelGGL((gn_apply_any_kernel<T, true, 3>), grid, dim3(256), lds, st, x, y, mean, rstd, gamma, beta, HW, C, G, act, ppb, stat_rows, nullptr, nullptr);
        else hipLaunchKernelGGL((gn_apply_any_kernel<T, false, 3>), grid, dim3(256), lds, st, x, y, mean, rstd, gamma, beta, HW, C, G, act, ppb, stat_rows, nullptr, nullptr);
    } else if (y2) {
        if (y_el == OMGSR_EL_SPLIT && y2_el == OMGSR_EL_SPLIT) OMGSR_GN_ANY2(2, 2);
        else if (y_el == OMGSR_EL_SPLIT) OMGSR_GN_ANY2(2, 0);
        else if (y2_el == OMGSR_EL_SPLIT) OMGSR_GN_ANY2(0, 2);
        else OMGSR_GN_ANY2(0, 0);
    } else if (x_el == OMGSR_EL_F32 && y_el == OMGSR_EL_SPLIT) OMGSR_GN_ANY(true, 2);
    else if (x_el == OMGSR_EL_F32) OMGSR_GN_ANY(true, 0);
    else if (y_el == OMGSR_EL_SPLIT) OMGSR_GN_ANY(false, 2);
    else OMGSR_DISPATCH_T(hipLaunchKernelGGL(gn_apply_kernel<T>, grid, dim3(256), lds, st, (const T*)x,
                                             (T*)y, mean, rstd, gamma, beta, HW, C, G, act, ppb, stat_rows));
#undef OMGSR_GN_ANY
#undef OMGSR_GN_ANY2
    return (int)hipGetLastError();
}
}

namespace {
template <bool XF32, int YEL>
int layernorm_launch(const void* x, void* y, const float* a, const float* b, int64_t rows, int32_t C, float eps, hipStream_t st) {
    const int nch = ((C >> 3) + 63) / 64;
    auto grid = [&](int rpw) { return dim3((unsigned)((rows + 4 * rpw - 1) / (4 * rpw))); };
    if (nch <= 1) OMGSR_DISPATCH_T(hipLaunchKernelGGL((layernorm_kernel<T, 1, 4, XF32, YEL>), grid(4), dim3(256), 0, st, x, y, a, b, rows, C, eps));
    else if (nch <= 2) OMGSR_DISPATCH_T(hipLaunchKernelGGL((layernorm_kernel<T, 2, 4, XF32, YEL>), grid(4), dim3(256), 0, st, x, y, a, b, rows, C, eps));
    else if (nch <= 3) OMGSR_DISPATCH_T(hipLaunchKernelGGL((layernorm_kernel<T, 3, 2, XF32, YEL>), grid(2), dim3(256), 0, st, x, y, a, b, rows, C, eps));
    else if (rows >= (1ll << 31)) return OMGSR_E_SHAPE;
    else OMGSR_DISPATCH_T(hipLaunchKernelGGL((layernorm_block_kernel<T, 2, XF32, YEL>), dim3((unsigned)rows), dim3(256), 0, st, x, y, a, b, C, eps));
    return (int)hipGetLastError();
}
}

extern "C" int omgsr_layernorm(const void* x, void* y, const float* a, const float* b, int64_t rows, int32_t C,
                               float eps, int32_t x_el, int32_t y_el, void* stream) {
    if (!x || !y || rows <= 0 || C <= 0) return OMGSR_E_BADARG;
    if ((x_el != OMGSR_EL_16 && x_el != OMGSR_EL_F32) || (y_el != OMGSR_EL_16 && y_el != OMGSR_EL_SPLIT && y_el != OMGSR_EL_MX)) return OMGSR_E_BADARG;
    if ((C & 7) || C > 64 * 8 * 8) return OMGSR_E_SHAPE;
    if (y_el == OMGSR_EL_MX && (x_el != OMGSR_EL_F32 || omgsr::compute_dtype() != 1 || (C & 63))) return OMGSR_E_SHAPE;
    hipStream_t st = (hipStream_t)stream;
    omgsr::TimingScope ts(OMGSR_TK_LN, 0.0, ((x_el == OMGSR_EL_F32 ? 4.0 : 2.0) + (y_el != OMGSR_EL_16 ? 4.0 : 2.0)) * (double)rows * C, st);
    if (y_el == OMGSR_EL_MX) return layernorm_launch<true, 3>(x, y, a, b, rows, C, eps, st);
    if (x_el == OMGSR_EL_F32 && y_el == OMGSR_EL_SPLIT) return layernorm_launch<true, 2>(x, y, a, b, rows, C, eps, st);
    if (x_el == OMGSR_EL_F32) return layernorm_launch<true, 0>(x, y, a, b, rows, C, eps, st);
    if (y_el == OMGSR_EL_SPLIT) return layernorm_launch<false, 2>(x, y, a, b, rows, C, eps, st);
    return layernorm_launch<false, 0>(x, y, a, b, rows, C, eps, st);
}

extern "C" int omgsr_softmax_rows(const float* s, void* p, int64_t rows, int32_t L, int32_t Lvalid, void* stream) {
    if (!s || !p || rows <= 0 || L <= 0 || Lvalid <= 0 || Lvalid > L) return OMGSR_E_BADARG;
    if ((L & 3) || L > 256 * 4 * 16 || rows >= (1ll << 31)) return OMGSR_E_SHAPE;
    hipStream_t st = (hipStream_t)stream;
    omgsr::TimingScope ts(OMGSR_TK_SOFTMAX, 0.0, 6.0 * (double)rows * L, st);
    const int nv = (L / 4 + 255) / 256;
    if (nv <= 1) OMGSR_DISPATCH_T(hipLaunchKernelGGL((softmax_rows_kernel<T, 1>), dim3((unsigned)rows), dim3(256), 0, st, s, (T*)p, L, Lvalid));
    else if (nv <= 4) OMGSR_DISPATCH_T(hipLaunchKernelGGL((softmax_rows_kernel<T, 4>), dim3((unsigned)rows), dim3(256), 0, st, s, (T*)p, L, Lvalid));
    else OMGSR_DISPATCH_T(hipLaunchKernelGGL((softmax_rows_kernel<T, 16>), dim3((unsigned)rows), dim3(256), 0, st, s, (T*)p, L, Lvalid));
    return (int)hipGetLastError();
}

extern "C" int omgsr_softmax_rows_split(const float* s, void* p, int64_t rows, int32_t L, int32_t Lvalid, void* stream) {
    if (!s || !p || rows <= 0 || L <= 0 || Lvalid <= 0 || Lvalid > L) return OMGSR_E_BADARG;
    if ((L & 3) || L > 256 * 4 * 16 || rows >= (1ll << 31)) return OMGSR_E_SHAPE;
    hipStream_t st = (hipStream_t)stream;
    omgsr::TimingScope ts(OMGSR_TK_SOFTMAX, 0.0, 8.0 * (double)rows * L, st);
    const int nv = (L / 4 + 255) / 256;
    if (nv <= 1) OMGSR_DISPATCH_T(hipLaunchKernelGGL((softmax_rows_kernel<T, 1, true>), dim3((unsigned)rows), dim3(256), 0, st, s, (T*)p, L, Lvalid));
    else if (nv <= 4) OMGSR_DISPATCH_T(hipLaunchKernelGGL((softmax_rows_kernel<T, 4, true>), dim3((unsigned)rows), dim3(256), 0, st, s, (T*)p, L, Lvalid));
    else OMGSR_DISPATCH_T(hipLaunchKernelGGL((softmax_rows_kernel<T, 16, true>), dim3((unsigned)rows), dim3(256), 0, st, s, (T*)p, L, Lvalid));
    return (int)hipGetLastError();
}

extern "C" int omgsr_rmsnorm_rope_mxfp8(const void* x, const float* w, const float* w2, int32_t Lsplit, const float* cos_t, const float* sin_t, int32_t B,
                                        int32_t L, int32_t H, int32_t D, int64_t ld, int32_t col0, int32_t pos0, float eps, void* codes, void* scales,
                                        int64_t c_ld, int64_t s_ld, void* stream) {
    if (!x || !w || !codes || !scales || B <= 0 || L <= 0 || H <= 0) return OMGSR_E_BADARG;
    if (D != 128 || (ld & 7) || (col0 & 127) || (c_ld & 15) || (s_ld & 3) || c_ld < (int64_t)col0 + (int64_t)H * D || s_ld < ((int64_t)col0 + (int64_t)H * D) / 32 ||
        ((cos_t == nullptr) != (sin_t == nullptr)) || omgsr::compute_dtype() != 0)
        return OMGSR_E_SHAPE;
    hipStream_t st = (hipStream_t)stream;
    const int64_t rows = (int64_t)B * L;
    const int64_t groups = rows * H;
    omgsr::TimingScope ts(OMGSR_TK_ELT, 0.0, (2.0 + 1.0 + 1.0 / 32.0) * (double)groups * D, st);
    hipLaunchKernelGGL(rmsnorm_rope_mxfp8_kernel, dim3((unsigned)((groups + 15) / 16)), dim3(256), 0, st, (const bf16_t*)x, w, w2, Lsplit, cos_t, sin_t,
                       rows, L, H, D, ld, col0, pos0, eps, (unsigned char*)codes, (unsigned char*)scales, c_ld, s_ld);
    return (int)hipGetLastError();
}

extern "C" int omgsr_rmsnorm_rope(void* x, const float* w, const float* w2, int32_t Lsplit, const float* cos_t, const float* sin_t, int32_t B, int32_t L,
                                  int32_t H, int32_t D, int64_t ld, int32_t col0, int32_t pos0, float eps, void* stream) {
    if (!x || !w || B <= 0 || L <= 0 || H <= 0) return OMGSR_E_BADARG;
    if (D != 128 || (ld & 7) || (col0 & 7) || ((cos_t == nullptr) != (sin_t == nullptr))) return OMGSR_E_SHAPE;
    hipStream_t st = (hipStream_t)stream;
    const int64_t rows = (int64_t)B * L;
    const int64_t groups = rows * H;
    omgsr::TimingScope ts(OMGSR_TK_ELT, 0.0, 4.0 * (double)groups * D, st);
    OMGSR_DISPATCH_T(hipLaunchKernelGGL(rmsnorm_rope_kernel<T>, dim3((unsigned)((groups + 15) / 16)), dim3(256), 0, st, (T*)x, w, w2, Lsplit, cos_t,
                                        sin_t, rows, L, H, D, ld, col0, pos0, eps));
    return (int)hipGetLastError();
}
```

omgsr_amd/diffusers_api/autoencoder_kl.py:

```python
from __future__ import annotations

import os
from types import SimpleNamespace
from typing import Optional

import torch
import torch.nn as nn

from .. import ops
from ..nn import Conv2d, GroupNorm, Linear
from .modeling_utils import ConfigDict, ModelMixin

SD21_VAE_CONFIG = dict(in_channels=3, out_channels=3, block_out_channels=[128, 256, 512, 512], layers_per_block=2,
                       latent_channels=4, norm_num_groups=32, scaling_factor=0.18215, shift_factor=None,
                       use_quant_conv=True, use_post_quant_conv=True, act_fn="silu", sample_size=768)
FLUX_VAE_CONFIG = dict(in_channels=3, out_channels=3, block_out_channels=[128, 256, 512, 512], layers_per_block=2,
                       latent_channels=16, norm_num_groups=32, scaling_factor=0.3611, shift_factor=0.1159,
                       use_quant_conv=False, use_post_quant_conv=False, act_fn="silu", sample_size=1024)


class ResnetBlock2D(nn.Module):
    def __init__(self, in_channels: int, out_channels: int, temb_channels: Optional[int], groups: int, eps: float):
        super().__init__()
        self.in_channels, self.out_channels = in_channels, out_channels
        self.norm1 = GroupNorm(groups, in_channels, eps=eps)
        self.conv1 = Conv2d(in_channels, out_channels, 3, padding=1)
        self.time_emb_proj = Linear(temb_channels, out_channels) if temb_channels else None
        self.norm2 = GroupNorm(groups, out_channels, eps=eps)
        self.conv2 = Conv2d(out_channels, out_channels, 3, padding=1)
        self.use_in_shortcut = in_channels != out_channels
        self.conv_shortcut = Conv2d(in_channels, out_channels, 1) if self.use_in_shortcut else None
        self.nonlinearity = nn.SiLU()

    def nhwc(self, x, conv1_bias=None, out_for=None):
        if self.conv_shortcut is not None and x.dtype == torch.float32:
            h, xc = self.norm1.nhwc(x, ops.ACT_SILU, split=self.conv1.in_split(), also_cast=self.conv_shortcut.in_split())
            h = self.conv1.nhwc(h, bias_override=conv1_bias, gn_groups=self.norm2.num_groups)
        else:
            xc = x
            h = self.conv1.nhwc(x, gn=self.norm1.spec(x, ops.ACT_SILU), bias_override=conv1_bias, gn_groups=self.norm2.num_groups)
        g2 = self.norm2.spec(h, ops.ACT_SILU)
        sc = self.conv_shortcut.nhwc(xc, pad=0) if self.conv_shortcut is not None else x
        if out_for is not None:
            return self.conv2.nhwc(h, gn=g2, residual=sc, out_dtype=ops.OUT_BF16, out_split=out_for.in_split())
        return self.conv2.nhwc(h, gn=g2, residual=sc, gn_groups=self.norm1.num_groups)

    def forward(self, x, temb=None):
        if temb is not None or self.time_emb_proj is not None:
            raise NotImplementedError("ResnetBlock2D.forward: the UNet folds the time embedding at fixed t* (UNet2DConditionModel.nhwc)")
        return _nchw_call(self.nhwc, x, self.out_channels)


class Downsample2D(nn.Module):
    def __init__(self, channels: int, padding: int):
        super().__init__()
        self.padding = padding
        self.conv = Conv2d(channels, channels, 3, stride=2, padding=padding)

    def nhwc(self, x, gn_groups: int = 0):
        pad = (0, 1, 0, 1) if self.padding == 0 else self.padding
        return self.conv.nhwc(x, pad=pad, gn_groups=gn_groups)

    def forward(self, x):
        return _nchw_call(self.nhwc, x, self.conv.out_channels)


class Upsample2D(nn.Module):
    def __init__(self, channels: int):
        super().__init__()
        self.conv = Conv2d(channels, channels, 3, padding=1)
        self.conv.phase_upsample = True

    def nhwc(self, x, gn_groups: int = 0):
        return self.conv.nhwc(x, upsample=True, gn_groups=gn_groups)

    def forward(self, x, output_size=None):
        if output_size is not None:
            raise NotImplementedError("Upsample2D.forward: explicit output_size (odd latent shapes) is outside the hot path (SURVEY A.6)")
        return _nchw_call(self.nhwc, x, self.conv.out_channels)


MATERIALISED_MAX_KEYS = 16384


def _parse_fused_knob(value: Optional[str]) -> Optional[bool]:
    return {"0": False, "1": True}.get((value or "").strip())


_ENV_FUSED = _parse_fused_knob(os.environ.get("OMGSR_VAE_ATTN_FUSED"))


def vae_attention_route(L: int, precise: bool, attn_split: bool, switch: Optional[bool], env: Optional[bool] = None) -> str:
    if precise and attn_split:
        if L > MATERIALISED_MAX_KEYS:
            raise ValueError(f"the range-fallback VAE attention is limited to {MATERIALISED_MAX_KEYS} keys (got {L}): its split probabilities "
                             "and split V^T run on the materialised path only; tile the VAE or use the accurate tier's fp16 operands")
        return "materialised"
    if switch is None:
        switch = env
    if switch is not None:
        return "fused" if switch else "materialised"
    return "fused" if L > MATERIALISED_MAX_KEYS else "materialised"


class VaeAttention(nn.Module):

    fused: Optional[bool] = None

    def __init__(self, channels: int, groups: int):
        super().__init__()
        self.heads = 1
        self.scale = channels ** -0.5
        self.group_norm = GroupNorm(groups, channels, eps=1e-6)
        self.to_q = Linear(channels, channels)
        self.to_k = Linear(channels, channels)
        self.to_v = Linear(channels, channels)
        self.to_out = nn.ModuleList([Linear(channels, channels), nn.Dropout(0.0)])
        self.norm_cross = None

    def qkv_split(self) -> int:
        return self.to_q.in_split()

    def nhwc(self, x):
        return self.attend(self.group_norm.nhwc(x, split=self.qkv_split()), x)

    def forward(self, hidden_states, encoder_hidden_states=None, attention_mask=None, temb=None):
        if encoder_hidden_states is not None or attention_mask is not None:
            raise NotImplementedError("VaeAttention is the VAE mid block's unmasked self-attention")
        return _nchw_call(self.nhwc, hidden_states, hidden_states.shape[1])

    def attend(self, g, residual):
        N, H, W, Cg = g.shape
        Cc = residual.shape[-1]
        L = H * W
        x = residual
        g = g.reshape(N, L, Cg)
        Lp = ops._round_up(L, 128)
        full = ops.attn_split()
        qk2 = ops.precise() and (getattr(self, "qk_split", False) or full)
        route = vae_attention_route(L, ops.precise(), full, self.fused, _ENV_FUSED)
        q = self.to_q.nhwc(g, out_dtype=ops.OUT_BF16, out_split=2 if qk2 else 1)
        k = self.to_k.nhwc(g, out_dtype=ops.OUT_BF16, out_split=2 if qk2 else 1)
        if route == "fused":
            vt = ops.linear_t(g, self.to_v.packed(), L)
            o = ops.attention(q, k, vt, self.heads, Cc, self.scale, out_split=self.to_out[0].in_split(),
                              q_lo_col=Cc if qk2 else None, k_lo_col=Cc if qk2 else None, p_split=False)
            out = self.to_out[0].nhwc(o, residual=x.reshape(N, L, Cc), gn_groups=self.group_norm.num_groups)
            return ops.carry_gn(out, out.reshape(N, H, W, Cc))
        if qk2:
            k = ops.split_rows_hhl(k, Lp)
        elif Lp != L:
            kp = torch.zeros((N, Lp, Cc), device=x.device, dtype=ops.act_dtype())
            kp[:, :L] = k
            k = kp
        s = ops.bmm_nt(q, k, alpha=self.scale, out_dtype=ops.OUT_F32, both_split=qk2)
        if full:
            vts = ops.transpose_split(self.to_v.nhwc(g, out_dtype=ops.OUT_F32), Lp)
            vt = torch.cat([vts[:, :Cc], vts[:, :Cc], vts[:, Cc:]], dim=-1)
            p = ops.softmax_rows(s, valid=L, split=True)
            del s, vts
            o = ops.bmm_nt(p, vt, out_split=self.to_out[0].in_split(), both_split=True)
        else:
            vt = ops.linear_t(g, self.to_v.packed(), L, ld=Lp)
            p = ops.softmax_rows(s, valid=L)
            del s
            o = ops.bmm_nt(p, vt, out_split=self.to_out[0].in_split())
        out = self.to_out[0].nhwc(o, residual=x.reshape(N, L, Cc), gn_groups=self.group_norm.num_groups)
        return ops.carry_gn(out, out.reshape(N, H, W, Cc))

    def prepare_attention_mask(self, attention_mask, target_length, batch_size, out_dim=3):
        return attention_mask

    def head_to_batch_dim(self, tensor, out_dim=3):
        B, L, Cc = tensor.shape
        t = tensor.reshape(B, L, self.heads, Cc // self.heads).permute(0, 2, 1, 3)
        return t.reshape(B * self.heads, L, Cc // self.heads) if out_dim == 3 else t

    def batch_to_head_dim(self, tensor):
        BH, L, d = tensor.shape
        return tensor.reshape(BH // self.heads, self.heads, L, d).permute(0, 2, 1, 3).reshape(BH // self.heads, L, d * self.heads)

    def get_attention_scores(self, query, key, attention_mask=None):
        if attention_mask is not None:
            raise NotImplementedError("VaeAttention.get_attention_scores: the VAE mid block is never masked")
        B, Lq, d = query.shape
        Lk = key.shape[1]
        dp, Lkp = ops._round_up(d, 32), ops._round_up(Lk, 128)
        q = torch.zeros((B, Lq, dp), device=query.device, dtype=ops.act_dtype()); q[..., :d] = query
# ... 191 lines not shown
```

omgsr_amd/diffusers_api/unet_2d_condition.py:

```python
from __future__ import annotations

import math
from types import SimpleNamespace
from typing import Optional

import torch
import torch.nn as nn

from .. import ops
from ..nn import Conv2d, GroupNorm, InputCache, LayerNorm, Linear, _key, bump_cache_epoch
from .autoencoder_kl import Downsample2D, ResnetBlock2D, Upsample2D
from .modeling_utils import ConfigDict, ModelMixin

SD21_UNET_CONFIG = dict(
    in_channels=4, out_channels=4, sample_size=64, block_out_channels=[320, 640, 1280, 1280],
    down_block_types=["CrossAttnDownBlock2D", "CrossAttnDownBlock2D", "CrossAttnDownBlock2D", "DownBlock2D"],
    up_block_types=["UpBlock2D", "CrossAttnUpBlock2D", "CrossAttnUpBlock2D", "CrossAttnUpBlock2D"],
    layers_per_block=2, attention_head_dim=[5, 10, 20, 20], cross_attention_dim=1024,
    use_linear_projection=True, norm_num_groups=32, norm_eps=1e-5, flip_sin_to_cos=True, freq_shift=0,
    downsample_padding=1, act_fn="silu", mid_block_scale_factor=1, upcast_attention=False)


def timestep_sinusoid(t: torch.Tensor, dim: int, flip_sin_to_cos: bool, freq_shift: float) -> torch.Tensor:
    half = dim // 2
# ... 107 lines not shown
    def __init__(self, dim: int, heads: int, dim_head: int, cross_attention_dim: int):
        super().__init__()
        self.norm1 = LayerNorm(dim, eps=1e-5)
        self.attn1 = Attention(dim, heads, dim_head)
        self.norm2 = LayerNorm(dim, eps=1e-5)
        self.attn2 = Attention(dim, heads, dim_head, cross_attention_dim=cross_attention_dim)
        self.norm3 = LayerNorm(dim, eps=1e-5)
        self.ff = FeedForward(dim)

    def nhwc(self, y, ehs, out_for=None):
        y = self.attn1.self_nhwc(self.norm1.nhwc(y, split=self.attn1.in_split()), y)
        y = self.attn2.cross_nhwc(self.norm2.nhwc(y, split=self.attn2.in_split()), ehs, y)
        return self.ff.nhwc(self.norm3.nhwc(y, split=self.ff.net[0].proj.in_split()), y, out_for=out_for)


class Transformer2DModel(nn.Module):
    def __init__(self, channels: int, heads: int, dim_head: int, cross_attention_dim: int, groups: int):
        super().__init__()
        self.norm = GroupNorm(groups, channels, eps=1e-6)
        self.proj_in = Linear(channels, channels)
        self.transformer_blocks = nn.ModuleList([BasicTransformerBlock(channels, heads, dim_head, cross_attention_dim)])
        self.proj_out = Linear(channels, channels)

    def nhwc(self, x, ehs, out_for=None):
        N, H, W, Cc = x.shape
        res = x.reshape(N, H * W, Cc)
        y = self.proj_in.nhwc(self.norm.nhwc(x, split=self.proj_in.in_split()).reshape(N, H * W, -1))
        nb = len(self.transformer_blocks)
        for i, blk in enumerate(self.transformer_blocks):
            y = blk.nhwc(y, ehs, out_for=self.proj_out if i == nb - 1 else None)
        if out_for is not None:
            out = self.proj_out.nhwc(y, residual=res, out_dtype=ops.OUT_BF16, out_split=out_for.in_split())
            return out.reshape(N, H, W, -1)
        out = self.proj_out.nhwc(y, residual=res, gn_groups=self.norm.num_groups)
        return ops.carry_gn(out, out.reshape(N, H, W, Cc))


class _DownBlock(nn.Module):
    def __init__(self, cin, cout, temb, layers, heads, cross_dim, groups, eps, add_down, down_pad, with_attn):
        super().__init__()
        self.resnets = nn.ModuleList([ResnetBlock2D(cin if j == 0 else cout, cout, temb, groups, eps) for j in range(layers)])
        self.attentions = nn.ModuleList([Transformer2DModel(cout, heads, cout // heads, cross_dim, groups) for _ in range(layers)]) if with_attn else None
        self.downsamplers = nn.ModuleList([Downsample2D(cout, down_pad)]) if add_down else None


class _UpBlock(nn.Module):
    def __init__(self, in_channels, prev_out, cout, temb, layers, heads, cross_dim, groups, eps, add_up, with_attn):
        super().__init__()
        rs = []
        for j in range(layers):
            skip = in_channels if j == layers - 1 else cout
            rin = prev_out if j == 0 else cout
            rs.append(ResnetBlock2D(rin + skip, cout, temb, groups, eps))
        self.resnets = nn.ModuleList(rs)
        self.attentions = nn.ModuleList([Transformer2DModel(cout, heads, cout // heads, cross_dim, groups) for _ in range(layers)]) if with_attn else None
        self.upsamplers = nn.ModuleList([Upsample2D(cout)]) if add_up else None


class _MidBlock(nn.Module):
    def __init__(self, ch, temb, heads, cross_dim, groups, eps):
        super().__init__()
        self.resnets = nn.ModuleList([ResnetBlock2D(ch, ch, temb, groups, eps), ResnetBlock2D(ch, ch, temb, groups, eps)])
        self.attentions = nn.ModuleList([Transformer2DModel(ch, heads, ch // heads, cross_dim, groups)])


class UNet2DConditionModel(ModelMixin):
    default_config = SD21_UNET_CONFIG

    def __init__(self, **cfg):
        super().__init__()
        c = ConfigDict({**SD21_UNET_CONFIG, **cfg})
        self.config = c
        boc = c.block_out_channels
        temb = boc[0] * 4
        heads = c.attention_head_dim if isinstance(c.attention_head_dim, (list, tuple)) else [c.attention_head_dim] * len(boc)
        g, eps = c.norm_num_groups, c.norm_eps
        self.conv_in = Conv2d(c.in_channels, boc[0], 3, padding=1)
        self.time_embedding = TimestepEmbedding(boc[0], temb)
        downs, out_ch = [], boc[0]
        for i, t in enumerate(c.down_block_types):
            in_ch, out_ch = out_ch, boc[i]
            downs.append(_DownBlock(in_ch, out_ch, temb, c.layers_per_block, heads[i], c.cross_attention_dim, g, eps,
                                    add_down=i < len(boc) - 1, down_pad=c.downsample_padding,
                                    with_attn=t == "CrossAttnDownBlock2D"))
        self.down_blocks = nn.ModuleList(downs)
        self.mid_block = _MidBlock(boc[-1], temb, heads[-1], c.cross_attention_dim, g, eps)
        rev, rheads = list(reversed(boc)), list(reversed(heads))
        ups, out_ch = [], rev[0]
        for i, t in enumerate(c.up_block_types):
            prev, out_ch = out_ch, rev[i]
            in_ch = rev[min(i + 1, len(boc) - 1)]
            ups.append(_UpBlock(in_ch, prev, out_ch, temb, c.layers_per_block + 1, rheads[i], c.cross_attention_dim, g, eps,
                                add_up=i < len(boc) - 1, with_attn=t == "CrossAttnUpBlock2D"))
        self.up_blocks = nn.ModuleList(ups)
        self.conv_norm_out = GroupNorm(g, boc[0], eps=eps)
        self.conv_act = nn.SiLU()
        self.conv_out = Conv2d(boc[0], c.out_channels, 3, padding=1)
        self._temb_cache: dict = {}

    def _resnets(self):
        for b in self.down_blocks:
            yield from b.resnets
        yield from self.mid_block.resnets
        for b in self.up_blocks:
            yield from b.resnets

    def _fold_key(self, timestep) -> tuple:
        t = int(timestep) if not torch.is_tensor(timestep) else int(timestep.reshape(-1)[0].item())
        deps = [self.time_embedding.linear_1.weight, self.time_embedding.linear_1.bias, self.time_embedding.linear_2.weight,
                self.time_embedding.linear_2.bias]
        for r in self._resnets():
            deps += [r.time_emb_proj.weight, r.time_emb_proj.bias, r.conv1.bias]
        return (t, _key(*deps))

    def _folded_biases(self, timestep) -> dict:
        key = self._fold_key(timestep)
        t = key[0]
        if key not in self._temb_cache:
            bump_cache_epoch()
            dev = self.conv_in.weight.device
            with torch.no_grad():
                tt = torch.tensor([t], dtype=torch.int64, device=dev)
                emb = self.time_embedding.fp32(timestep_sinusoid(tt, self.config.block_out_channels[0],
                                                                 self.config.flip_sin_to_cos, self.config.freq_shift))
                out = {}
                for r in self._resnets():
                    v = ops.linear_f32(emb, r.time_emb_proj.weight, r.time_emb_proj.bias, silu_in=True)[0]
                    out[id(r)] = (r.conv1.bias.float() + v).contiguous()
            self._temb_cache = {key: out}
        return self._temb_cache[key]

    def nhwc(self, x: torch.Tensor, timestep, ehs: torch.Tensor) -> torch.Tensor:
        fb = self._folded_biases(timestep)
        g = self.config.norm_num_groups
        h = self.conv_in.nhwc(x, gn_groups=g)
        skips = [h]
        for blk in self.down_blocks:
            for j, r in enumerate(blk.resnets):
                h = r.nhwc(h, fb[id(r)])
                if blk.attentions is not None:
                    h = blk.attentions[j].nhwc(h, ehs)
                skips.append(h)
            if blk.downsamplers is not None:
                h = blk.downsamplers[0].nhwc(h, gn_groups=g)
                skips.append(h)
        m = self.mid_block
        h = m.resnets[0].nhwc(h, fb[id(m.resnets[0])])
        h = m.attentions[0].nhwc(h, ehs)
        h = m.resnets[1].nhwc(h, fb[id(m.resnets[1])])
        for blk in self.up_blocks:
            up = blk.upsamplers[0].conv if blk.upsamplers is not None else None
            for j, r in enumerate(blk.resnets):
                last = up if j == len(blk.resnets) - 1 else None
                h = ops.concat_channels(h, skips.pop())
                h = r.nhwc(h, fb[id(r)], out_for=last if blk.attentions is None else None)
                if blk.attentions is not None:
                    h = blk.attentions[j].nhwc(h, ehs, out_for=last)
            if blk.upsamplers is not None:
                h = blk.upsamplers[0].nhwc(h)
        return self.conv_out.nhwc(h, gn=self.conv_norm_out.spec(h, ops.ACT_SILU))

    def forward(self, sample: torch.Tensor, timestep, encoder_hidden_states: torch.Tensor, return_dict: bool = True):
        x = ops.nchw_to_nhwc(sample.contiguous(), 8)
        y = self.nhwc(x, timestep, encoder_hidden_states)
        out_dtype = ops.io_dtype(sample)
        out = ops.nhwc_to_nchw(y, channels=self.config.out_channels, dtype=out_dtype)
        return SimpleNamespace(sample=out) if return_dict else (out,)
```

omgsr_amd/nn.py:

```python
from __future__ import annotations

import dataclasses
from typing import Optional

import torch
import torch.nn as nn

from . import ops


def _key(*tensors) -> tuple:
    return ops.mode_key() + tuple((t.data_ptr(), t._version, str(t.device), t.dtype, tuple(t.shape)) if torch.is_tensor(t) else t for t in tensors)


_CACHE_EPOCH = 0


def cache_epoch() -> int:
    return _CACHE_EPOCH


def bump_cache_epoch() -> None:
    global _CACHE_EPOCH
    _CACHE_EPOCH += 1


_REBUILD_LOG = None


def begin_rebuild_log() -> None:
    global _REBUILD_LOG
    _REBUILD_LOG = []


def end_rebuild_log() -> list:
    global _REBUILD_LOG
    log, _REBUILD_LOG = _REBUILD_LOG or [], None
    return log


def _log_rebuild(invalidate) -> None:
    if _REBUILD_LOG is not None:
        _REBUILD_LOG.append(invalidate)


class InputCache:

    def __init__(self):
        self._inputs, self._versions, self._wkey, self._value = None, None, None, None

    def prime(self, inputs: tuple, wkey: tuple, value) -> None:
        self._value, self._inputs, self._wkey = value, tuple(inputs), wkey
        self._versions = tuple(None if t is None else t._version for t in inputs)
        bump_cache_epoch()

    def invalidate(self) -> None:
        self._inputs, self._versions, self._wkey, self._value = None, None, None, None
        bump_cache_epoch()

    def get(self, inputs: tuple, wkey: tuple, builder):
        same = (self._inputs is not None and len(self._inputs) == len(inputs) and self._wkey == wkey and
                all(a is b for a, b in zip(self._inputs, inputs)) and
                self._versions == tuple(None if t is None else t._version for t in inputs))
        if not same:
            bump_cache_epoch()
            _log_rebuild(self.invalidate)
            self._value = builder()
            self._inputs, self._wkey = tuple(inputs), wkey
            self._versions = tuple(None if t is None else t._version for t in inputs)
        return self._value


class _Packed:

    def _drop_packed(self) -> None:
        self._pk, self._pk_key = None, None
        bump_cache_epoch()

    def _packed(self, builder, *tensors):
        k = _key(*tensors)
        if getattr(self, "_pk_key", None) != k:
            bump_cache_epoch()
            _log_rebuild(self._drop_packed)
            self._pk = builder()
            self._pk_key = k
        return self._pk


class _Operand:
    op_split = 1
    w_split = 1
    out_inner16 = False

    def in_split(self) -> int:
        return self.op_split if ops.precise() else 1

    def in_wsplit(self) -> int:
        return self.w_split if ops.precise() else 1


class Conv2d(nn.Conv2d, _Packed, _Operand):
    phase_upsample = False

    def packed(self) -> ops.PackedWeight:
        sp, wsp, ph = self.in_split(), self.in_wsplit(), self.phase_upsample
        return self._packed(lambda: ops.pack_conv_weight(self.weight, self.bias, cout_multiple=8, split=sp, w_split=wsp, upsample_phases=ph),
                            self.weight, self.bias, sp, wsp, ph)

    def nhwc(self, x, *, pad=None, upsample=False, act=ops.ACT_NONE, residual=None, bias_override=None, stride=None, gn_groups=0,
             out_dtype=ops.OUT_STREAM, out_split=1, gn=None):
        pw = self.packed()
        if bias_override is not None:
            pw = dataclasses.replace(pw, bias=bias_override)
        p = self.padding[0] if pad is None else pad
        if out_dtype == ops.OUT_STREAM and self.out_inner16 and ops.precise():
            out_dtype = ops.OUT_BF16
        return ops.conv2d(x, pw, stride=stride or self.stride[0], pad=p, upsample=upsample, act=act, residual=residual,
                          gn_groups=gn_groups, out_dtype=out_dtype, out_split=out_split, gn=gn)

    def nhwc_multi(self, xs, *, pad=None, upsample=False, act=ops.ACT_NONE, residuals=None, stride=None, gn_groups=0,
                   out_dtype=ops.OUT_STREAM, out_split=1, gn=None):
        pw = self.packed()
        p = self.padding[0] if pad is None else pad
        if out_dtype == ops.OUT_STREAM and self.out_inner16 and ops.precise():
            out_dtype = ops.OUT_BF16
        return ops.conv2d_multi(list(xs), pw, stride=stride or self.stride[0], pad=p, upsample=upsample, act=act, residuals=residuals,
                                gn_groups=gn_groups, out_dtype=out_dtype, out_split=out_split, gn=gn)

    def forward(self, x):
        y = self.nhwc(ops.nchw_to_nhwc(x.contiguous(), ops._round_up(self.in_channels, 8)))
        return ops.nhwc_to_nchw(y, channels=self.out_channels,
                                dtype=ops.io_dtype(x))


class Linear(nn.Linear, _Packed, _Operand):
    fp8 = False

    def packed(self) -> ops.PackedWeight:
        if self.fp8:
            return self._packed(lambda: ops.pack_linear_weight_mxfp8(self.weight, self.bias), self.weight, self.bias, "fp8")
        sp, wsp = self.in_split(), self.in_wsplit()
        return self._packed(lambda: ops.pack_linear_weight(self.weight, self.bias, split=sp, w_split=wsp), self.weight, self.bias, sp, wsp)

    def nhwc(self, x, *, act=ops.ACT_NONE, residual=None, gate=None, out_dtype=ops.OUT_STREAM, gn_groups=0, out_split=1):
        return ops.linear(x, self.packed(), act=act, residual=residual, gate=gate, out_dtype=out_dtype, gn_groups=gn_groups,
                          out_split=out_split)

    def forward(self, x):
        y = self.nhwc(x.to(ops.stream_dtype()).contiguous())
        return y.to(x.dtype)


class GroupNorm(nn.GroupNorm, _Packed):
    def _affine(self):
        return self._packed(lambda: (self.weight.detach().float().contiguous(), self.bias.detach().float().contiguous()),
                            self.weight, self.bias)

    def nhwc(self, x, act=ops.ACT_NONE, split=1, also_cast=0):
        g, b = self._affine()
        return ops.group_norm(x, g, b, self.num_groups, self.eps, act, split=split, also_cast=also_cast)

    def stats(self, x):
        return ops.group_norm_stats(x, self.num_groups, self.eps)

    def spec(self, x, act=ops.ACT_NONE) -> "ops.GnSpec":
        mean, rstd, _ = self.stats(x)
        return self.spec_stats(mean, rstd, act)

    def spec_stats(self, mean, rstd, act=ops.ACT_NONE) -> "ops.GnSpec":
        g, b = self._affine()
        return ops.GnSpec(mean, rstd, g, b, self.num_groups, act)

    def apply_stats(self, x, mean, rstd, act=ops.ACT_NONE, split=1, also_cast=0):
        g, b = self._affine()
        if mean.shape[0] != x.shape[0]:
            return ops.group_norm_apply_shared(x, mean, rstd, g, b, self.num_groups, act, split=split, also_cast=also_cast)
        return ops.group_norm_apply(x, mean, rstd, g, b, self.num_groups, act, split=split, also_cast=also_cast)

    def forward(self, x):
        shp = x.shape
        x4 = x.reshape(shp[0], shp[1], -1, 1) if x.dim() == 3 else x
        y = self.nhwc(ops.nchw_to_nhwc(x4.contiguous()))
        return ops.nhwc_to_nchw(y, dtype=ops.io_dtype(x)).to(x.dtype).reshape(shp)


class LayerNorm(nn.LayerNorm, _Packed):
    def _affine(self):
        if not self.elementwise_affine:
            return None, None
        return self._packed(lambda: (self.weight.detach().float().contiguous(), self.bias.detach().float().contiguous()),
                            self.weight, self.bias)

    def nhwc(self, x, a=None, b=None, split=1):
        if a is None and b is None:
            a, b = self._affine()
        return ops.layer_norm(x, a, b, self.eps, split=split)

    def forward(self, x):
        return self.nhwc(x.to(ops.stream_dtype()).contiguous()).to(x.dtype)


class RMSNormWeight(nn.Module):

    def __init__(self, dim: int, eps: float):
        super().__init__()
        self.eps = eps
        self.weight = nn.Parameter(torch.ones(dim))

    def w32(self):
        return self.weight.detach().float().contiguous()
```

omgsr_amd/ops.py:

```python
from __future__ import annotations

import ctypes as C
import os
from dataclasses import dataclass
from typing import Optional

import torch

from . import _lib
from ._lib import AttnArgs, IgemmArgs, check

ACT_NONE, ACT_SILU, ACT_GELU_TANH, ACT_GEGLU = 0, 1, 2, 3
OUT_STREAM, OUT_BF16, OUT_F32 = -1, 0, 1
LAYOUT_NHWC, LAYOUT_T = 0, 1
EL_16, EL_F32, EL_SPLIT, EL_MX, EL_MX6, EL_MXFP8 = 0, 1, 2, 3, 4, 5
MX_LO_SHIFT = 11


def _el_of_split(split: int) -> int:
    return {1: EL_16, 2: EL_SPLIT, 3: EL_MX, 4: EL_MX6}[split]


_ACT = torch.bfloat16
_PRECISE = False
# ... 824 lines not shown
    check(_lib.load().omgsr_transpose_split(x.data_ptr(), out.data_ptr(), B, L, Cc, ld, _stream()), "omgsr_transpose_split")
    return out


def bmm_nt(a_mat: torch.Tensor, b_mat: torch.Tensor, *, alpha: float = 1.0, out_dtype: int = OUT_BF16, out_split: int = 1,
           both_split: bool = False) -> torch.Tensor:
    _req(a_mat, act_dtype(), "a")
    _req(b_mat, act_dtype(), "b")
    B, M, K = a_mat.shape
    Bb, Np, Kb = b_mat.shape
    if both_split:
        if Bb != B or K % 64 or Kb * 2 != K * 3:
            raise ValueError(f"bmm_nt(both_split): incompatible shapes {tuple(a_mat.shape)} x {tuple(b_mat.shape)}")
    elif Bb != B or Kb != K or K % 32:
        raise ValueError(f"bmm_nt: incompatible shapes {tuple(a_mat.shape)} x {tuple(b_mat.shape)}")
    if Np % 128:
        bp = torch.zeros((B, _round_up(Np, 128), Kb), device=b_mat.device, dtype=act_dtype())
        bp[:, :Np] = b_mat
        full = bmm_nt(a_mat, bp, alpha=alpha, out_dtype=out_dtype, out_split=out_split, both_split=both_split)
        Npp = bp.shape[1]
        if out_split == 2 and out_dtype == OUT_BF16:
            return torch.cat([full[:, :, :Np], full[:, :, Npp:Npp + Np]], dim=-1).contiguous()
        return full[:, :, :Np].contiguous()
    split = out_split if out_dtype == OUT_BF16 else 1
    out = torch.empty((B, M, Np * split), device=a_mat.device, dtype=act_dtype() if out_dtype == OUT_BF16 else torch.float32)
    a = IgemmArgs()
    a.in_, a.weight, a.bias, a.gate, a.residual, a.out = a_mat.data_ptr(), b_mat.data_ptr(), None, None, None, out.data_ptr()
    a.N, a.H, a.W, a.Cin = 1, 1, M, Kb
    a.Cout, a.Cout_pad, a.K_pad = Np, Np, Kb
    if both_split:
        a.in_ld, a.in_split, a.w_split = K, 1, 1
        a.overflow_flag = _ovf(a_mat.device)
    a.R, a.S, a.stride, a.pad_top, a.pad_left, a.upsample = 1, 1, 1, 0, 0, 0
    a.Ho, a.Wo = 1, M
    a.act, a.out_dtype, a.out_layout = ACT_NONE, out_dtype, LAYOUT_NHWC
    a.t_rows, a.t_ld = 0, 0
    a.out_lo_off = Np if split == 2 else 0
    a.out_ld = Np * split if split == 2 else 0
    a.batch, a.in_bstride, a.w_bstride, a.out_bstride = B, M * K, Np * Kb, M * Np * split
    a.alpha = alpha
    check(_lib.load().omgsr_igemm(C.byref(a), _stream()), "omgsr_igemm(bmm_nt)")
    return out


def split_rows_hhl(x: torch.Tensor, pad_rows: int = 0) -> torch.Tensor:
    B, L, C2 = x.shape
    Cc = C2 // 2
    out = (torch.zeros if pad_rows > L else torch.empty)((B, max(L, pad_rows), 3 * Cc), device=x.device, dtype=x.dtype)
    out[:, :L, :Cc] = x[:, :, :Cc]
    out[:, :L, Cc:2 * Cc] = x[:, :, :Cc]
    out[:, :L, 2 * Cc:] = x[:, :, Cc:]
    return out



def _fused_gn(x: torch.Tensor, groups: int, N: int):
    fused = getattr(x, "_omgsr_gn", None)
    if fused is not None and fused[1] == groups and fused[2] == x.data_ptr() and fused[3] == x._version and fused[0].shape[0] == N:
        return fused[0]
    return None


def group_norm_stats(x: torch.Tensor, groups: int, eps: float):
    xel = _el(x, "x")
    N, Cc = x.shape[0], x.shape[-1]
    HW = x.numel() // (N * Cc)
    lib = _lib.load()
    mean = torch.empty((N, groups), device=x.device, dtype=torch.float32)
    rstd = torch.empty_like(mean)
    var = torch.empty_like(mean)
    fused = _fused_gn(x, groups, N)
    if fused is not None:
        check(lib.omgsr_groupnorm_finalize(fused.data_ptr(), mean.data_ptr(), rstd.data_ptr(), var.data_ptr(), N,
                                           fused.shape[1], groups, fused.shape[2], float(HW) * (Cc // groups), eps, _stream()),
              "omgsr_groupnorm_finalize")
        return mean, rstd, var
    nchunk = lib.omgsr_groupnorm_nchunk(HW)
    partial = torch.empty((N, nchunk, groups, 2), device=x.device, dtype=torch.float32)
    check(lib.omgsr_groupnorm_stats(x.data_ptr(), partial.data_ptr(), mean.data_ptr(), rstd.data_ptr(), var.data_ptr(),
                                    N, HW, Cc, groups, eps, xel, _stream()), "omgsr_groupnorm_stats")
    return mean, rstd, var


def group_norm_partial(x: torch.Tensor, groups: int) -> torch.Tensor:
    xel = _el(x, "x")
    N, Cc = x.shape[0], x.shape[-1]
    fused = _fused_gn(x, groups, N)
    if fused is not None:
        return fused
    HW = x.numel() // (N * Cc)
    lib = _lib.load()
    partial = torch.empty((N, lib.omgsr_groupnorm_nchunk(HW), groups, 2), device=x.device, dtype=torch.float32)
    check(lib.omgsr_groupnorm_partial(x.data_ptr(), partial.data_ptr(), N, HW, Cc, groups, xel, _stream()), "omgsr_groupnorm_partial")
    return partial


def group_norm_stats_merged(tensors, tiles, N: int, groups: int, eps: float):
    if len(tensors) > _lib.GN_MAX_GROUPS:
        raise ValueError(f"at most {_lib.GN_MAX_GROUPS} tile shape groups")
    a = _lib.GnMergeArgs()
    keep = []
    tot = float(sum(t.shape[1] * t.shape[2] * tiles[k] for k, t in enumerate(tensors)))
    for k, t in enumerate(tensors):
        part = group_norm_partial(t, groups)
        keep.append(part)
        a.partial[k] = part.data_ptr()
        a.nslot[k] = part.shape[1]
        a.entries[k] = part.shape[2]
        a.tiles[k] = tiles[k]
        a.count[k] = float(t.shape[1] * t.shape[2] * (t.shape[3] // groups))
        a.weight[k] = t.shape[1] * t.shape[2] / tot
    a.ngroups = len(tensors)
    dev = tensors[0].device
    mean = torch.empty((N, groups), device=dev, dtype=torch.float32)
    rstd = torch.empty_like(mean)
    var = torch.empty_like(mean)
    check(_lib.load().omgsr_groupnorm_finalize_merged(C.byref(a), mean.data_ptr(), rstd.data_ptr(), var.data_ptr(), N, groups,
                                                      eps, _stream()), "omgsr_groupnorm_finalize_merged")
    return mean, rstd, var


def _operand_like(x: torch.Tensor, split: int) -> torch.Tensor:
    if split not in (1, 2, 3, 4):
        raise ValueError("split must be 1, 2, 3 (MX) or 4 (MX6)")
    return torch.empty((*x.shape[:-1], x.shape[-1] * min(split, 2)), device=x.device, dtype=_ACT)


def _cast_twin(x: torch.Tensor, xel: int, also_cast: int):
    if not also_cast:
        return None
    if xel != EL_F32:
        if also_cast != 1:
            raise ValueError("a 16-bit tensor cannot be split")
        return x
    return _operand_like(x, also_cast)


def group_norm_apply_shared(x: torch.Tensor, mean: torch.Tensor, rstd: torch.Tensor, gamma, beta, groups: int,
                            act: int = ACT_NONE, split: int = 1, also_cast: int = 0):
    xel = _el(x, "x")
    rows, Cc = x.shape[0], x.shape[-1]
    HW = x.numel() // (rows * Cc)
    y = _operand_like(x, split)
    y2 = _cast_twin(x, xel, also_cast)
    fused = y2 is not None and y2 is not x
    check(_lib.load().omgsr_groupnorm_apply_shared(x.data_ptr(), y.data_ptr(), mean.data_ptr(), rstd.data_ptr(), _ptr(gamma),
                                                   _ptr(beta), rows, HW, Cc, groups, act, mean.shape[0], xel,
                                                   _el_of_split(split), y2.data_ptr() if fused else None,
                                                   _el_of_split(also_cast) if also_cast else EL_16, _ovf(x.device) if fused else None, _stream()),
          "omgsr_groupnorm_apply_shared")
    return (y, y2) if also_cast else y


def group_norm_apply(x: torch.Tensor, mean: torch.Tensor, rstd: torch.Tensor, gamma: Optional[torch.Tensor],
                     beta: Optional[torch.Tensor], groups: int, act: int = ACT_NONE, inplace: bool = False, split: int = 1,
                     also_cast: int = 0):
    xel = _el(x, "x")
    N, Cc = x.shape[0], x.shape[-1]
    HW = x.numel() // (N * Cc)
    y = x if (inplace and xel == EL_16 and split == 1 and not also_cast) else _operand_like(x, split)
    y2 = _cast_twin(x, xel, also_cast)
    fused = y2 is not None and y2 is not x
    check(_lib.load().omgsr_groupnorm_apply(x.data_ptr(), y.data_ptr(), mean.data_ptr(), rstd.data_ptr(), _ptr(gamma),
                                            _ptr(beta), N, HW, Cc, groups, act, xel, _el_of_split(split),
                                            y2.data_ptr() if fused else None, _el_of_split(also_cast) if also_cast else EL_16,
                                            _ovf(x.device) if fused else None, _stream()),
          "omgsr_groupnorm_apply")
    return (y, y2) if also_cast else y


def group_norm(x: torch.Tensor, gamma, beta, groups: int, eps: float, act: int = ACT_NONE, split: int = 1, also_cast: int = 0):
    mean, rstd, _ = group_norm_stats(x, groups, eps)
    return group_norm_apply(x, mean, rstd, gamma, beta, groups, act, split=split, also_cast=also_cast)



def layer_norm(x: torch.Tensor, a: Optional[torch.Tensor], b: Optional[torch.Tensor], eps: float, split: int = 1) -> torch.Tensor:
    xel = _el(x, "x")
    Cc = x.shape[-1]
    rows = x.numel() // Cc
    y = _operand_like(x, split)
    check(_lib.load().omgsr_layernorm(x.data_ptr(), y.data_ptr(), _ptr(a), _ptr(b), rows, Cc, eps, xel, _el_of_split(split), _stream()),
          "omgsr_layernorm")
    return y



def attention(q: torch.Tensor, k: torch.Tensor, vt: torch.Tensor, heads: int, head_dim: int, scale: float,
              *, q_col: int = 0, k_col: int = 0, Lk: Optional[int] = None, out: Optional[torch.Tensor] = None,
              o_col: int = 0, out_split: int = 1, o_lo_col: Optional[int] = None, q_lo_col: Optional[int] = None,
              k_lo_col: Optional[int] = None, p_split: bool = True) -> torch.Tensor:
    mx = [isinstance(x, Mxfp8) for x in (q, k, vt)]
    if any(mx):
        if not all(mx):
            raise ValueError("attention: q, k and vt are all MXFP8 or none is")
        if out_split != 1 or q_lo_col is not None or k_lo_col is not None:
            raise ValueError("attention: MXFP8 operands take a plain bf16 output and no two-term splits")
        return _attention_mxfp8(q, k, vt, heads, head_dim, scale, q_col, k_col, Lk, out, o_col)
    if head_dim == 512:
        if out_split == 3:
            raise ValueError("attention: head_dim 512 writes a plain or two-term-split output (out_split 1 or 2), not the MX form")
        if vt.shape[1] == 2 * heads * head_dim:
            raise ValueError("attention: head_dim 512 takes a single V^T; the two-term-split V^T is limited to head_dim 64")
        if q_lo_col is not None and k_lo_col is not None and p_split:
            raise ValueError("attention: head_dim 512 takes split q / k with p_split=False; split probabilities are limited to head_dim 64")
    _req(q, act_dtype(), "q"); _req(k, act_dtype(), "k"); _req(vt, act_dtype(), "vt")
    B, Lq = q.shape[0], q.shape[1]
    Bk = k.shape[0]
    Lk = Lk if Lk is not None else k.shape[1]
    inner = heads * head_dim
    if out is None:
        out = torch.empty((B, Lq, inner * min(out_split, 2)), device=q.device, dtype=act_dtype())
    a = AttnArgs()
    esz = 2
    a.q = q.data_ptr() + q_col * esz
    a.k = k.data_ptr() + k_col * esz
    a.vt = vt.data_ptr()
    a.o = out.data_ptr() + o_col * esz
    a.B, a.H, a.D, a.Lq, a.Lk = B, heads, head_dim, Lq, Lk
    a.q_ld, a.k_ld, a.vt_ld, a.o_ld = q.shape[-1], k.shape[-1], vt.shape[-1], out.shape[-1]
    a.q_bstride = Lq * q.shape[-1]
    a.k_bstride = 0 if Bk == 1 and B > 1 else k.shape[1] * k.shape[-1]
    a.vt_bstride = 0 if Bk == 1 and B > 1 else vt.shape[1] * vt.shape[-1]
    a.o_bstride = Lq * out.shape[-1]
    a.scale = scale
    a.o_lo_off = 0 if out_split != 2 else ((o_lo_col - o_col) if o_lo_col is not None else inner)
    a.o_mx = int(out_split == 3)
    if (q_lo_col is None) != (k_lo_col is None):
        raise ValueError("attention: q_lo_col and k_lo_col come together")
    a.q_lo_off = 0 if q_lo_col is None else q_lo_col - q_col
    a.k_lo_off = 0 if k_lo_col is None else k_lo_col - k_col
    a.p_split = int(q_lo_col is not None and p_split)
    if vt.shape[1] == 2 * inner:
        if q_lo_col is None:
            raise ValueError("attention: a split V^T comes with split q / k")
        a.vt_lo_off = inner * vt.shape[-1]
    elif vt.shape[1] != inner:
        raise ValueError(f"attention: vt has {vt.shape[1]} rows, expected {inner} (or {2 * inner} as a two-term split)")
    if out_split == 3 and o_col != 0:
        raise ValueError("attention: an MX output owns its whole row (o_col must be 0)")
    check(_lib.load().omgsr_attention(C.byref(a), _stream()), "omgsr_attention")
    return out


def _attention_mxfp8(q: Mxfp8, k: Mxfp8, vt: Mxfp8, heads: int, head_dim: int, scale: float, q_col: int, k_col: int, Lk: Optional[int],
                     out: Optional[torch.Tensor], o_col: int) -> torch.Tensor:
    if _PRECISE or _ACT != torch.bfloat16:
        raise ValueError("MXFP8 attention needs the bf16 compute type (the fp8 tier)")
    if head_dim != 128:
        raise ValueError(f"MXFP8 attention needs head_dim 128, got {head_dim}")
    for name, t in (("q", q), ("k", k), ("vt", vt)):
        _req(t.codes, torch.uint8, name); _req(t.scales, torch.uint8, name + " scales")
        if t.codes.dim() != 3 or t.scales.shape != (*t.codes.shape[:-1], t.codes.shape[-1] // 32):
            raise ValueError(f"attention: {name} is not an [B, rows, ld] MXFP8 operand")
    if q_col % 128 or k_col % 128:
        raise ValueError("attention: MXFP8 q / k columns must be multiples of 128")
    B, Lq = q.codes.shape[0], q.codes.shape[1]
    Bk = k.codes.shape[0]
    Lk = Lk if Lk is not None else k.codes.shape[1]
    inner = heads * head_dim
    ld = vt.codes.shape[-1]
    if vt.codes.shape[1] != inner:
        raise ValueError(f"attention: vt has {vt.codes.shape[1]} rows, expected {inner}")
    if ld % 128 or ld < Lk:
        raise ValueError(f"attention: an MXFP8 V^T needs ld % 128 == 0 and ld >= Lk, got ld {ld} for Lk {Lk}")
    if out is None:
        out = torch.empty((B, Lq, inner), device=q.codes.device, dtype=torch.bfloat16)
    _req(out, torch.bfloat16, "out")
    bcast = Bk == 1 and B > 1
    a = AttnArgs()
    a.qkv_el = EL_MXFP8
    a.q, a.k, a.vt = q.codes.data_ptr() + q_col, k.codes.data_ptr() + k_col, vt.codes.data_ptr()
    a.q_scale, a.k_scale, a.vt_scale = q.scales.data_ptr() + q_col // 32, k.scales.data_ptr() + k_col // 32, vt.scales.data_ptr()
    a.o = out.data_ptr() + o_col * 2
    a.B, a.H, a.D, a.Lq, a.Lk = B, heads, head_dim, Lq, Lk
    a.q_ld, a.k_ld, a.vt_ld, a.o_ld = q.codes.shape[-1], k.codes.shape[-1], ld, out.shape[-1]
    a.q_sld, a.k_sld, a.vt_sld = q.scales.shape[-1], k.scales.shape[-1], vt.scales.shape[-1]
    a.q_bstride, a.q_sbstride = Lq * a.q_ld, Lq * a.q_sld
    a.k_bstride, a.k_sbstride = (0, 0) if bcast else (k.codes.shape[1] * a.k_ld, k.codes.shape[1] * a.k_sld)
    a.vt_bstride, a.vt_sbstride = (0, 0) if bcast else (inner * ld, inner * a.vt_sld)
    a.o_bstride = Lq * out.shape[-1]
    a.scale = scale
    check(_lib.load().omgsr_attention(C.byref(a), _stream()), "omgsr_attention")
    return out


def softmax_rows(s: torch.Tensor, valid: Optional[int] = None, split: bool = False) -> torch.Tensor:
    _req(s, torch.float32, "s")
    L = s.shape[-1]
    rows = s.numel() // L
    p = torch.empty(s.shape[:-1] + ((2 * L) if split else L,), device=s.device, dtype=act_dtype())
    fn = _lib.load().omgsr_softmax_rows_split if split else _lib.load().omgsr_softmax_rows
    check(fn(s.data_ptr(), p.data_ptr(), rows, L, valid or L, _stream()), "omgsr_softmax_rows")
    return p


def rmsnorm_rope_(x: torch.Tensor, w: torch.Tensor, cos: Optional[torch.Tensor], sin: Optional[torch.Tensor],
                  heads: int, head_dim: int, col0: int = 0, pos0: int = 0, eps: float = 1e-6,
                  w_after: Optional[torch.Tensor] = None, split_at: int = 0) -> torch.Tensor:
    _req(x, act_dtype(), "x"); _req(w, torch.float32, "w")
    B, L, ld = x.shape
    if tuple(w.shape) != (heads, head_dim) or (w_after is not None and tuple(w_after.shape) != (heads, head_dim)):
        raise ValueError(f"rmsnorm_rope_: w must be [{heads}, {head_dim}], got {tuple(w.shape)}")
    if cos is not None and (cos.shape[0] < pos0 + L or sin.shape[0] < pos0 + L or cos.shape[-1] != head_dim):
        raise ValueError(f"rmsnorm_rope_: rope tables {tuple(cos.shape)} do not cover positions {pos0}..{pos0 + L - 1} x {head_dim}")
    check(_lib.load().omgsr_rmsnorm_rope(x.data_ptr(), w.data_ptr(), _ptr(w_after), split_at, _ptr(cos), _ptr(sin), B, L, heads, head_dim, ld,
                                         col0, pos0, eps, _stream()), "omgsr_rmsnorm_rope")
    return x


def rmsnorm_rope_mxfp8(x: torch.Tensor, w: torch.Tensor, cos: Optional[torch.Tensor], sin: Optional[torch.Tensor], heads: int, head_dim: int,
                       pos0: int = 0, eps: float = 1e-6, w_after: Optional[torch.Tensor] = None, split_at: int = 0,
                       out: Optional[Mxfp8] = None) -> Mxfp8:
    _req(x, torch.bfloat16, "x"); _req(w, torch.float32, "w")
    if _PRECISE or _ACT != torch.bfloat16:
        raise ValueError("rmsnorm_rope_mxfp8 needs the bf16 compute type (the fp8 tier)")
    B, L, ld = x.shape
    if ld % 128:
        raise ValueError(f"rmsnorm_rope_mxfp8: row length {ld} is not a multiple of 128")
    if tuple(w.shape) != (heads, head_dim) or (w_after is not None and tuple(w_after.shape) != (heads, head_dim)):
        raise ValueError(f"rmsnorm_rope_mxfp8: w must be [{heads}, {head_dim}], got {tuple(w.shape)}")
    if cos is not None and (cos.shape[0] < pos0 + L or sin.shape[0] < pos0 + L or cos.shape[-1] != head_dim):
        raise ValueError(f"rmsnorm_rope_mxfp8: rope tables {tuple(cos.shape)} do not cover positions {pos0}..{pos0 + L - 1} x {head_dim}")
    if out is None:
        out = Mxfp8(torch.empty((B, L, ld), device=x.device, dtype=torch.uint8), torch.empty((B, L, ld // 32), device=x.device, dtype=torch.uint8))
    elif out.codes.shape != (B, L, ld) or out.scales.shape != (B, L, ld // 32) or not (out.codes.is_contiguous() and out.scales.is_contiguous()):
# ... 160 lines not shown
```

omgsr_amd/pipelines/vaehook.py:

```python
from __future__ import annotations

import math
from typing import Dict, List, Tuple

import torch

from .. import ops


def get_best_tile_size(lowerbound: int, upperbound: int) -> int:
    divider = 32
    while divider >= 2:
        rem = lowerbound % divider
        if rem == 0:
            return lowerbound
        cand = lowerbound - rem + divider
        if cand <= upperbound:
            return cand
        divider //= 2
    return lowerbound


def split_tiles(h: int, w: int, tile_size: int, pad: int, is_decoder: bool) -> Tuple[List[List[int]], List[List[int]]]:
    nh = max(math.ceil((h - 2 * pad) / tile_size), 1)
    nw = max(math.ceil((w - 2 * pad) / tile_size), 1)
    th = get_best_tile_size(math.ceil((h - 2 * pad) / nh), tile_size)
    tw = get_best_tile_size(math.ceil((w - 2 * pad) / nw), tile_size)
    ins, outs = [], []
    for i in range(nh):
        for j in range(nw):
            ib = [pad + j * tw, min(pad + (j + 1) * tw, w), pad + i * th, min(pad + (i + 1) * th, h)]
            ob = [ib[0] if ib[0] > pad else 0, ib[1] if ib[1] < w - pad else w,
                  ib[2] if ib[2] > pad else 0, ib[3] if ib[3] < h - pad else h]
            outs.append([v * 8 if is_decoder else v // 8 for v in ob])
            ins.append([max(0, ib[0] - pad), min(w, ib[1] + pad), max(0, ib[2] - pad), min(h, ib[3] + pad)])
    return ins, outs


class VAEHook:
    def __init__(self, net, tile_size, is_decoder, fast_decoder, fast_encoder, color_fix, to_gpu=False):
        self.net = net
        self.tile_size = tile_size
        self.is_decoder = is_decoder
        self.fast_mode = (fast_encoder and not is_decoder) or (fast_decoder and is_decoder)
        self.color_fix = color_fix and not is_decoder
        self.to_gpu = to_gpu
        self.pad = 11 if is_decoder else 32

    def _ops(self):
        net, dec = self.net, self.is_decoder
        seq = [("conv", net.conv_in, dict(gn_groups=net.conv_norm_out.num_groups))]

        def resblock(b, out_for=None):
            if b.conv_shortcut is None:
                seq.append(("res_push", None))
            seq.append(("gn", b.norm1, ops.ACT_SILU, b.conv1, b.conv_shortcut))
            seq.append(("conv", b.conv1, dict(gn_groups=b.norm2.num_groups)))
            seq.append(("gn", b.norm2, ops.ACT_SILU, b.conv2, None))
            seq.append(("conv_res", b.conv2, b.norm1.num_groups, out_for))

        def attn(a):
            seq.append(("res_push", None))
            seq.append(("gn", a.group_norm, ops.ACT_NONE, a.to_q, None))
            seq.append(("attn_res", a))

        def mid():
            resblock(net.mid_block.resnets[0]); attn(net.mid_block.attentions[0]); resblock(net.mid_block.resnets[1])

        if dec:
            mid()
            blocks = net.up_blocks
        else:
            blocks = net.down_blocks
        for i, blk in enumerate(blocks):
            samp = None if i == len(blocks) - 1 else (blk.upsamplers[0] if dec else blk.downsamplers[0])
            for j, r in enumerate(blk.resnets):
                resblock(r, out_for=samp.conv if (samp is not None and j == len(blk.resnets) - 1) else None)
            if samp is not None:
                g = blk.resnets[0].norm1.num_groups
                if dec:
                    seq.append(("conv", samp.conv, dict(upsample=True, gn_groups=g)))
                else:
                    seq.append(("conv", samp.conv, dict(pad=(0, 1, 0, 1) if samp.padding == 0 else samp.padding, gn_groups=g)))
        if not dec:
            mid()
        seq.append(("gn", net.conv_norm_out, ops.ACT_SILU, net.conv_out, None))
        seq.append(("conv", net.conv_out, {}))
        return seq

    @torch.no_grad()
    def __call__(self, x: torch.Tensor) -> torch.Tensor:
        N, H, W, _ = x.shape
        if max(H, W) <= self.pad * 2 + self.tile_size:
            return self.net.nhwc(x)
        return self.vae_tile_forward(x)

    def _run(self, seq, groups: Dict[tuple, torch.Tensor], counts: Dict[tuple, int], N: int, fixed=None, record=None):
        res: Dict[tuple, list] = {k: [] for k in groups}
        gi = 0
        pending = None
        for op in seq:
            kind = op[0]
            if kind == "gn":
                norm, act = op[1], op[2]
                G = norm.num_groups
                if fixed is not None:
                    mean, var = fixed[gi]
                    rstd = torch.rsqrt(var + 1e-6)
                else:
                    keys = list(groups)
                    mean, rstd, var = ops.group_norm_stats_merged([groups[k] for k in keys], [counts[k] for k in keys], N, G, 1e-6)
                if record is not None:
                    record.append((mean, var))
                gi += 1
                first = next(iter(groups.values()))
                is_conv3 = getattr(op[3], "kernel_size", None) == (3, 3)
                if is_conv3 and first.dtype != torch.float32:
                    pending = norm.spec_stats(mean, rstd, act)
                    if op[4] is not None:
                        for k in groups:
                            res[k].append(op[4].nhwc(groups[k], pad=0))
                    continue
                for k in groups:
                    if op[4] is not None:
                        groups[k], xc = norm.apply_stats(groups[k], mean, rstd, act, split=op[3].in_split(), also_cast=op[4].in_split())
                        res[k].append(op[4].nhwc(xc, pad=0))
                    else:
                        groups[k] = norm.apply_stats(groups[k], mean, rstd, act, split=op[3].in_split())
            elif kind == "conv":
                keys = list(groups)
                for k, y in zip(keys, op[1].nhwc_multi([groups[k] for k in keys], gn=pending, **op[2])):
                    groups[k] = y
                pending = None
            elif kind == "res_push":
                for k in groups:
                    res[k].append(op[1](groups[k]) if op[1] is not None else groups[k])
            elif kind == "conv_res":
                keys = list(groups)
                xs, rs = [groups[k] for k in keys], [res[k].pop() for k in keys]
                if op[3] is not None:
                    outs = op[1].nhwc_multi(xs, residuals=rs, out_dtype=ops.OUT_BF16, out_split=op[3].in_split(), gn=pending)
                else:
                    outs = op[1].nhwc_multi(xs, residuals=rs, gn_groups=op[2], gn=pending)
                pending = None
                for k, y in zip(keys, outs):
                    groups[k] = y
            elif kind == "attn_res":
                for k in groups:
                    groups[k] = op[1].attend(groups[k], residual=res[k].pop())
        return groups

    @torch.no_grad()
    def vae_tile_forward(self, x: torch.Tensor) -> torch.Tensor:
        N, H, W, _ = x.shape
        ins, outs = split_tiles(H, W, self.tile_size, self.pad, self.is_decoder)
        seq = self._ops()
        fixed = None
        if self.fast_mode:
            fixed = self._estimate(x, seq)
        order: Dict[tuple, List[int]] = {}
        for i, b in enumerate(ins):
            order.setdefault((b[3] - b[2], b[1] - b[0]), []).append(i)
        groups = {k: torch.cat([ops.crop_nhwc(x, ins[i][2], ins[i][0], k[0], k[1]) for i in idx], 0) for k, idx in order.items()}
        counts = {k: len(idx) for k, idx in order.items()}
        groups = self._run(seq, groups, counts, N, fixed=fixed)
        Ho, Wo = (H * 8, W * 8) if self.is_decoder else (H // 8, W // 8)
        Cout = next(iter(groups.values())).shape[-1]
        result = torch.zeros((N, Ho, Wo, Cout), device=x.device, dtype=next(iter(groups.values())).dtype)
        for k, idx in order.items():
            t = groups[k]
            for j, i in enumerate(idx):
                ib, ob = ins[i], outs[i]
                pb = [v * 8 if self.is_decoder else v // 8 for v in ib]
                mg = [ob[q] - pb[q] for q in range(4)]
                th, tw = ob[3] - ob[2], ob[1] - ob[0]
                ops.paste_nhwc(t[j * N:(j + 1) * N], result, mg[2], mg[0], ob[2], ob[0], th, tw)
        return result

    def _estimate(self, x: torch.Tensor, seq):
        N, H, W, Cp = x.shape
        scale = self.tile_size / max(H, W)
        xc = x.float()
        small = ops.resize_nearest_exact(x, scale).float()
        std_o, mean_o = torch.std_mean(xc, dim=[0, 1, 2], keepdim=True)
        std_n, mean_n = torch.std_mean(small, dim=[0, 1, 2], keepdim=True)
        std_n = torch.where(std_n == 0, torch.ones_like(std_n), std_n)
        small = ((small - mean_n) / std_n * std_o + mean_o).clamp_(min=float(xc.min()), max=float(xc.max()))
        small = small.to(ops.stream_dtype()).contiguous()
        record: list = []
        self._run(seq, {(small.shape[1], small.shape[2]): small}, {(small.shape[1], small.shape[2]): 1}, N, record=record)
        return record
```

Baseline: 20.46 images/s.

## Batch GroupNorm apply across tile groups and fuse skip-concat into GroupNorm

Adds a multi-group GroupNorm apply kernel so the tiled VAE normalizes all tile-shape groups in one launch instead of one launch per group. Adds a two-source finalize and apply path so UNet up-block resnets with fp32 streams can normalize the hidden state and the skip connection without first materializing their channel concatenation. Upsamplers are also given fused GroupNorm statistics in precise mode. This cuts launch count and a full concat copy, at the cost of more kernel variants and a per-block group lookup loop.

```diff
diff --git a/include/omgsr_hip.h b/include/omgsr_hip.h
--- a/include/omgsr_hip.h
+++ b/include/omgsr_hip.h
@@ -120,6 +120,22 @@
                                  const float* gamma, const float* beta, int32_t rows, int64_t HW, int32_t C,
                                  int32_t G, int32_t act, int32_t stat_rows, int32_t x_el, int32_t y_el, void* y2, int32_t y2_el,
                                  uint32_t* overflow_flag, void* stream);
+typedef struct omgsr_gn_apply_group {
+    const void* x;
+    void* y;
+    void* y2;
+    int64_t HW;
+    int32_t rows;
+    int32_t reserved;
+} omgsr_gn_apply_group;
+int omgsr_groupnorm_apply_multi(const omgsr_gn_apply_group* groups, int32_t ngroups, const float* mean, const float* rstd,
+                                const float* gamma, const float* beta, int32_t C, int32_t G, int32_t act, int32_t stat_rows,
+                                int32_t x_el, int32_t y_el, int32_t y2_el, uint32_t* overflow_flag, void* stream);
+int omgsr_groupnorm_finalize2(const float* partial_a, int32_t nslot_a, int32_t Ca, const float* partial_b, int32_t nslot_b, int32_t Cb,
+                              float* mean, float* rstd, float* var_out, int32_t N, int32_t G, double count, float eps, void* stream);
+int omgsr_groupnorm_apply2(const void* xa, const void* xb, int32_t Ca, void* y, const float* mean, const float* rstd, const float* gamma,
+                           const float* beta, int32_t N, int64_t HW, int32_t C, int32_t G, int32_t act, int32_t y_el, void* y2, int32_t y2_el,
+                           uint32_t* overflow_flag, void* stream);
 
 int omgsr_layernorm(const void* x, void* y, const float* a, const float* b, int64_t rows, int32_t C,
                     float eps, int32_t x_el, int32_t y_el, void* stream);
diff --git a/omgsr_amd/_lib.py b/omgsr_amd/_lib.py
--- a/omgsr_amd/_lib.py
+++ b/omgsr_amd/_lib.py
@@ -7,7 +7,7 @@
 
 from .build import lib_path
 
-ABI_VERSION = 20
+ABI_VERSION = 21
 
 
 class OmgsrError(RuntimeError):
@@ -44,6 +44,10 @@
     _fields_ = [("partial", C.c_void_p * GN_MAX_GROUPS), ("count", C.c_double * GN_MAX_GROUPS),
                 ("weight", C.c_float * GN_MAX_GROUPS), ("tiles", C.c_int32 * GN_MAX_GROUPS),
                 ("nslot", C.c_int32 * GN_MAX_GROUPS), ("entries", C.c_int32 * GN_MAX_GROUPS), ("ngroups", C.c_int32)]
+
+
+class GnApplyGroup(C.Structure):
+    _fields_ = [("x", C.c_void_p), ("y", C.c_void_p), ("y2", C.c_void_p), ("HW", C.c_int64), ("rows", C.c_int32), ("reserved", C.c_int32)]
 
 
 class AttnArgs(C.Structure):
@@ -88,6 +92,9 @@
     "omgsr_groupnorm_partial": (C.c_int, [_P, _P, _I, _L, _I, _I, _I, _P]),
     "omgsr_groupnorm_finalize_merged": (C.c_int, [C.POINTER(GnMergeArgs), _P, _P, _P, _I, _I, _F, _P]),
     "omgsr_groupnorm_apply_shared": (C.c_int, [_P, _P, _P, _P, _P, _P, _I, _L, _I, _I, _I, _I, _I, _I, _P, _I, _P, _P]),
+    "omgsr_groupnorm_apply_multi": (C.c_int, [C.POINTER(GnApplyGroup), _I, _P, _P, _P, _P, _I, _I, _I, _I, _I, _I, _I, _P, _P]),
+    "omgsr_groupnorm_finalize2": (C.c_int, [_P, _I, _I, _P, _I, _I, _P, _P, _P, _I, _I, C.c_double, _F, _P]),
+    "omgsr_groupnorm_apply2": (C.c_int, [_P, _P, _I, _P, _P, _P, _P, _P, _I, _L, _I, _I, _I, _I, _P, _I, _P, _P]),
     "omgsr_image_to_model_input": (C.c_int, [_P, _P, _I, _I, _I, _I, _P]),
     "omgsr_colorfix_workspace_bytes": (C.c_int64, [_I, _I, _I, _I]),
     "omgsr_colorfix": (C.c_int, [_P, _I, _P, _P, _P, _I, _I, _I, _I, _I, _P]),
diff --git a/omgsr_amd/csrc/elementwise.hip b/omgsr_amd/csrc/elementwise.hip
--- a/omgsr_amd/csrc/elementwise.hip
+++ b/omgsr_amd/csrc/elementwise.hip
@@ -236,7 +236,7 @@
 
 }
 
-extern "C" int omgsr_abi_version(void) { return 20; }
+extern "C" int omgsr_abi_version(void) { return 21; }
 
 extern "C" int omgsr_set_compute_dtype(int dtype) {
     if (dtype != OMGSR_DT_BF16 && dtype != OMGSR_DT_F16) return OMGSR_E_BADARG;
diff --git a/omgsr_amd/csrc/norm.hip b/omgsr_amd/csrc/norm.hip
--- a/omgsr_amd/csrc/norm.hip
+++ b/omgsr_amd/csrc/norm.hip
@@ -87,15 +87,48 @@
     if (var_out) var_out[i] = (float)v;
 }
 
+__global__ void gn_finalize2_kernel(const float* __restrict__ pa, const float* __restrict__ pb, float* __restrict__ mean, float* __restrict__ rstd,
+                                    float* __restrict__ var_out, int N, int G, int nslot_a, int nslot_b, int Ca, int Cb, double count, float eps) {
+    const int i = blockIdx.x;
+    const int lane = threadIdx.x;
+    const int n = i / G, g = i - n * G;
+    const int cpg = (Ca + Cb) / G;
+    const int c0 = g * cpg, c1 = c0 + cpg;
+    const int a0 = c0 < Ca ? c0 : Ca, a1 = c1 < Ca ? c1 : Ca;
+    const int b0 = (c0 > Ca ? c0 : Ca) - Ca, b1 = (c1 > Ca ? c1 : Ca) - Ca;
+    double s = 0.0, q = 0.0;
+    if (a1 > a0) {
+        for (int c = lane; c < nslot_a; c += 64) {
+            const float* p = pa + (((int64_t)n * nslot_a + c) * Ca) * 2;
+            for (int j = a0; j < a1; ++j) { s += (double)p[2 * j]; q += (double)p[2 * j + 1]; }
+        }
+    }
+    if (b1 > b0) {
+        for (int c = lane; c < nslot_b; c += 64) {
+            const float* p = pb + (((int64_t)n * nslot_b + c) * Cb) * 2;
+            for (int j = b0; j < b1; ++j) { s += (double)p[2 * j]; q += (double)p[2 * j + 1]; }
+        }
+    }
+#pragma unroll
+    for (int o = 32; o > 0; o >>= 1) { s += __shfl_xor(s, o); q += __shfl_xor(q, o); }
+    if (lane != 0) return;
+    const double m = s / count;
+    double v = q / count - m * m;
+    if (v < 0.0) v = 0.0;
+    mean[i] = (float)m;
+    rstd[i] = (float)(1.0 / sqrt(v + (double)eps));
+    if (var_out) var_out[i] = (float)v;
+}
+
 template <typename T>
-__global__ __launch_bounds__(256) void gn_apply_kernel(const T* __restrict__ x, T* __restrict__ y,
-                                                        const float* __restrict__ mean, const float* __restrict__ rstd,
-                                                        const float* __restrict__ gamma, const float* __restrict__ beta,
-                                                        int64_t HW, int C, int G, int act, int64_t px_per_block, int stat_rows) {
+OMGSR_DEVINL void gn_apply_body(const T* __restrict__ x, T* __restrict__ y,
+                                const float* __restrict__ mean, const float* __restrict__ rstd,
+                                const float* __restrict__ gamma, const float* __restrict__ beta,
+                                int64_t HW, int C, int G, int act, int64_t px_per_block, int stat_rows, const int n, const int bx) {
     extern __shared__ __attribute__((aligned(16))) float gn_lds[];
     float* sc = gn_lds;
     float* sh = gn_lds + C;
-    const int t = threadIdx.x, n = blockIdx.y;
+    const int t = threadIdx.x;
     const int ns = n % stat_rows;
     const int cpg = C / G;
     for (int c = t; c < C; c += 256) {
@@ -107,7 +140,7 @@
     }
     __syncthreads();
     const int nch8 = C >> 3;
-    const int64_t p0 = (int64_t)blockIdx.x * px_per_block;
+    const int64_t p0 = (int64_t)bx * px_per_block;
     int64_t p1 = p0 + px_per_block; if (p1 > HW) p1 = HW;
     const int total = (int)((p1 - p0) * nch8);
     const T* xb = x + ((int64_t)n * HW + p0) * C;
@@ -149,13 +182,21 @@
         c8 += step8; if (c8 >= nch8) c8 -= nch8;
     }
 }
-
-template <typename T, bool XF32, int YEL, int Y2EL = -1>
-__global__ __launch_bounds__(256) void gn_apply_any_kernel(const void* __restrict__ x, void* __restrict__ y,
-                                                            const float* __restrict__ mean, const float* __restrict__ rstd,
-                                                            const float* __restrict__ gamma, const float* __restrict__ beta,
-                                                            int64_t HW, int C, int G, int act, int64_t px_per_block, int stat_rows,
-                                                            void* __restrict__ y2 = nullptr, unsigned* __restrict__ ovf = nullptr) {
+template <typename T>
+__global__ __launch_bounds__(256) void gn_apply_kernel(const T* __restrict__ x, T* __restrict__ y,
+                                                        const float* __restrict__ mean, const float* __restrict__ rstd,
+                                                        const float* __restrict__ gamma, const float* __restrict__ beta,
+                                                        int64_t HW, int C, int G, int act, int64_t px_per_block, int stat_rows) {
+    gn_apply_body<T>(x, y, mean, rstd, gamma, beta, HW, C, G, act, px_per_block, stat_rows, (int)blockIdx.y, (int)blockIdx.x);
+}
+
+template <typename T, bool XF32, int YEL, int Y2EL, bool TWO = false>
+OMGSR_DEVINL void gn_apply_any_body(const void* __restrict__ x, void* __restrict__ y,
+                                    const float* __restrict__ mean, const float* __restrict__ rstd,
+                                    const float* __restrict__ gamma, const float* __restrict__ beta,
+                                    int64_t HW, int C, int G, int act, int64_t px_per_block, int stat_rows,
+                                    void* __restrict__ y2, unsigned* __restrict__ ovf, const int n, const int bx,
+                                    const void* __restrict__ xb = nullptr, const int Ca = 0) {
     extern __shared__ __attribute__((aligned(16))) float gn_lds[];
     float amax = 0.0f;
     auto note8 = [&](const float (&v)[8]) {
@@ -166,7 +207,7 @@
     };
     float* sc = gn_lds;
     float* sh = gn_lds + C;
-    const int t = threadIdx.x, n = blockIdx.y;
+    const int t = threadIdx.x;
     const int ns = n % stat_rows;
     const int cpg = C / G;
     for (int c = t; c < C; c += 256) {
@@ -178,7 +219,7 @@
     }
     __syncthreads();
     const int nch8 = C >> 3;
-    const int64_t p0 = (int64_t)blockIdx.x * px_per_block;
+    const int64_t p0 = (int64_t)bx * px_per_block;
     int64_t p1 = p0 + px_per_block; if (p1 > HW) p1 = HW;
     const int total = (int)((p1 - p0) * nch8);
     const int64_t pix0 = (int64_t)n * HW + p0;
@@ -208,13 +249,20 @@
         if constexpr (Y2EL == 3) store8_mx<T>(y2, pix * 4 * C, C, cc8 * 8, v);
         else if constexpr (Y2EL >= 0) store8<T, Y2EL>(y2, pix * (Y2EL == 2 ? 2 * C : C) + cc8 * 8, C, v);
     };
+    auto get = [&](const int64_t pix, const int cc8, float (&v)[8]) {
+        if constexpr (TWO) {
+            static_assert(XF32, "two-source apply: fp32 stream tensors");
+            if (cc8 * 8 < Ca) load8<T, true>(x, pix * Ca + cc8 * 8, v);
+            else load8<T, true>(xb, pix * (C - Ca) + (cc8 * 8 - Ca), v);
+        } else load8<T, XF32>(x, pix * C + cc8 * 8, v);
+    };
     int i = t;
     for (; i + 256 < total; i += 512) {
         int c8b = c8, pxb = px;
         advance(c8b, pxb);
         float f[8], h[8];
-        load8<T, XF32>(x, (pix0 + px) * C + c8 * 8, f);
-        load8<T, XF32>(x, (pix0 + pxb) * C + c8b * 8, h);
+        get(pix0 + px, c8, f);
+        get(pix0 + pxb, c8b, h);
         if constexpr (Y2EL >= 0) {
             note8(f); note8(h);
             put2(pix0 + px, c8, f);
@@ -229,7 +277,7 @@
     }
     for (; i < total; i += 256) {
         float f[8];
-        load8<T, XF32>(x, (pix0 + px) * C + c8 * 8, f);
+        get(pix0 + px, c8, f);
         if constexpr (Y2EL >= 0) { note8(f); put2(pix0 + px, c8, f); }
         transform(f, c8);
         put(pix0 + px, c8, f);
@@ -239,6 +287,58 @@
         if (ovf && __any(amax > 65504.0f) && (t & 63) == 0) atomicOr(ovf, 1u);
         if (Y2EL == 3 && ovf && __any(amax > 448.0f) && (t & 63) == 0) atomicOr(ovf, 2u);
     }
+}
+template <typename T, bool XF32, int YEL, int Y2EL = -1>
+__global__ __launch_bounds__(256) void gn_apply_any_kernel(const void* __restrict__ x, void* __restrict__ y,
+                                                            const float* __restrict__ mean, const float* __restrict__ rstd,
+                                                            const float* __restrict__ gamma, const float* __restrict__ beta,
+                                                            int64_t HW, int C, int G, int act, int64_t px_per_block, int stat_rows,
+                                                            void* __restrict__ y2 = nullptr, unsigned* __restrict__ ovf = nullptr) {
+    gn_apply_any_body<T, XF32, YEL, Y2EL>(x, y, mean, rstd, gamma, beta, HW, C, G, act, px_per_block, stat_rows, y2, ovf, (int)blockIdx.y, (int)blockIdx.x);
+}
+template <typename T, int YEL, int Y2EL = -1>
+__global__ __launch_bounds__(256) void gn_apply_two_kernel(const void* __restrict__ xa, const void* __restrict__ xb, int Ca, void* __restrict__ y,
+                                                            const float* __restrict__ mean, const float* __restrict__ rstd,
+                                                            const float* __restrict__ gamma, const float* __restrict__ beta,
+                                                            int64_t HW, int C, int G, int act, int64_t px_per_block, int stat_rows,
+                                                            void* __restrict__ y2, unsigned* __restrict__ ovf) {
+    gn_apply_any_body<T, true, YEL, Y2EL, true>(xa, y, mean, rstd, gamma, beta, HW, C, G, act, px_per_block, stat_rows, y2, ovf, (int)blockIdx.y, (int)blockIdx.x,
+                                                xb, Ca);
+}
+
+struct GnApplyMulti {
+    const void* x[OMGSR_GN_MAX_GROUPS];
+    void* y[OMGSR_GN_MAX_GROUPS];
+    void* y2[OMGSR_GN_MAX_GROUPS];
+    int64_t HW[OMGSR_GN_MAX_GROUPS];
+    int64_t ppb[OMGSR_GN_MAX_GROUPS];
+    int nblk[OMGSR_GN_MAX_GROUPS];
+    int start[OMGSR_GN_MAX_GROUPS + 1];
+    int count;
+};
+OMGSR_DEVINL int gn_multi_lookup(const GnApplyMulti& m, int& n, int& bx) {
+    int s = 0;
+    while (s + 1 < m.count && (int)blockIdx.x >= m.start[s + 1]) ++s;
+    const int local = (int)blockIdx.x - m.start[s];
+    n = local / m.nblk[s];
+    bx = local - n * m.nblk[s];
+    return s;
+}
+template <typename T>
+__global__ __launch_bounds__(256) void gn_apply_multi_kernel(const GnApplyMulti m, const float* __restrict__ mean, const float* __restrict__ rstd,
+                                                              const float* __restrict__ gamma, const float* __restrict__ beta,
+                                                              int C, int G, int act, int stat_rows) {
+    int n, bx;
+    const int s = gn_multi_lookup(m, n, bx);
+    gn_apply_body<T>((const T*)m.x[s], (T*)m.y[s], mean, rstd, gamma, beta, m.HW[s], C, G, act, m.ppb[s], stat_rows, n, bx);
+}
+template <typename T, bool XF32, int YEL, int Y2EL = -1>
+__global__ __launch_bounds__(256) void gn_apply_any_multi_kernel(const GnApplyMulti m, const float* __restrict__ mean, const float* __restrict__ rstd,
+                                                                  const float* __restrict__ gamma, const float* __restrict__ beta,
+                                                                  int C, int G, int act, int stat_rows, unsigned* __restrict__ ovf) {
+    int n, bx;
+    const int s = gn_multi_lookup(m, n, bx);
+    gn_apply_any_body<T, XF32, YEL, Y2EL>(m.x[s], m.y[s], mean, rstd, gamma, beta, m.HW[s], C, G, act, m.ppb[s], stat_rows, m.y2[s], ovf, n, bx);
 }
 
 __global__ void gn_scale_shift_kernel(const float* __restrict__ mean, const float* __restrict__ rstd, const float* __restrict__ gamma,
@@ -610,6 +710,51 @@
     if (var_out) var_out[i] = (float)vv;
 }
 
+constexpr int GN_MERGE_WIDE_PAIRS = 512, GN_MERGE_WIDE_WAVES = 16;
+__global__ __launch_bounds__(64 * GN_MERGE_WIDE_WAVES) void gn_finalize_merged_wide_kernel(const omgsr_gn_merge_args a, float* __restrict__ mean,
+                                                                                           float* __restrict__ rstd, float* __restrict__ var_out,
+                                                                                           int N, int G, float eps, int npairs) {
+    __shared__ double pm[GN_MERGE_WIDE_PAIRS], pv[GN_MERGE_WIDE_PAIRS], pw[GN_MERGE_WIDE_PAIRS];
+    __shared__ double red[4][2];
+    const int i = blockIdx.x, lane = threadIdx.x & 63, wave = __builtin_amdgcn_readfirstlane(threadIdx.x >> 6);
+    const int n = i / G, g = i - n * G;
+    for (int pair = wave; pair < npairs; pair += GN_MERGE_WIDE_WAVES) {
+        int k = 0, t = pair;
+        while (t >= a.tiles[k]) { t -= a.tiles[k]; ++k; }
+        const float* partial = a.partial[k];
+        const int nslot = a.nslot[k];
+        const int row = t * N + n;
+        double s = 0.0, q = 0.0;
+        const int entries = a.entries[k], epg = entries / G;
+        for (int c = lane; c < nslot; c += 64) {
+            const float* pp = partial + (((int64_t)row * nslot + c) * entries + g * epg) * 2;
+            for (int j = 0; j < epg; ++j) { s += (double)pp[2 * j]; q += (double)pp[2 * j + 1]; }
+        }
+#pragma unroll
+        for (int o = 32; o > 0; o >>= 1) { s += __shfl_xor(s, o); q += __shfl_xor(q, o); }
+        const double m = s / a.count[k];
+        double v = q / a.count[k] - m * m;
+        if (v < 0.0) v = 0.0;
+        if (lane == 0) { pm[pair] = m; pv[pair] = v; pw[pair] = (double)a.weight[k]; }
+    }
+    __syncthreads();
+    if (threadIdx.x < 4) {
+        double m_acc = 0.0, v_acc = 0.0;
+        for (int pair = threadIdx.x; pair < npairs; pair += 4) {
+            m_acc += pw[pair] * pm[pair];
+            v_acc += pw[pair] * pv[pair];
+        }
+        red[threadIdx.x][0] = m_acc; red[threadIdx.x][1] = v_acc;
+    }
+    __syncthreads();
+    if (threadIdx.x != 0) return;
+    const double mm = ((red[0][0] + red[1][0]) + red[2][0]) + red[3][0];
+    const double vv = ((red[0][1] + red[1][1]) + red[2][1]) + red[3][1];
+    mean[i] = (float)mm;
+    rstd[i] = (float)(1.0 / sqrt(vv + (double)eps));
+    if (var_out) var_out[i] = (float)vv;
+}
+
 }
 namespace {
 int gn_apply_launch(const void* x, void* y, const float* mean, const float* rstd, const float* gamma,
@@ -635,7 +780,13 @@
     if (!a || !mean || !rstd || N <= 0 || G <= 0 || a->ngroups <= 0 || a->ngroups > OMGSR_GN_MAX_GROUPS) return OMGSR_E_BADARG;
     for (int k = 0; k < a->ngroups; ++k)
         if (!a->partial[k] || a->tiles[k] <= 0 || a->nslot[k] <= 0 || a->count[k] <= 0.0 || a->entries[k] < G || (a->entries[k] % G)) return OMGSR_E_BADARG;
-    hipLaunchKernelGGL(gn_finalize_merged_kernel, dim3(N * G), dim3(256), 0, (hipStream_t)stream, *a, mean, rstd, var_out, N, G, eps);
+    int npairs = 0;
+    for (int k = 0; k < a->ngroups; ++k) npairs += a->tiles[k];
+    static const char* narrow = getenv("OMGSR_GN_MERGE_NARROW");
+    if (npairs <= GN_MERGE_WIDE_PAIRS && !(narrow && narrow[0] == '1'))
+        hipLaunchKernelGGL(gn_finalize_merged_wide_kernel, dim3(N * G), dim3(64 * GN_MERGE_WIDE_WAVES), 0, (hipStream_t)stream, *a, mean, rstd, var_out, N, G, eps, npairs);
+    else
+        hipLaunchKernelGGL(gn_finalize_merged_kernel, dim3(N * G), dim3(256), 0, (hipStream_t)stream, *a, mean, rstd, var_out, N, G, eps);
     return (int)hipGetLastError();
 }
 
@@ -654,9 +805,41 @@
 }
 
 namespace {
-int gn_apply_launch(const void* x, void* y, const float* mean, const float* rstd, const float* gamma,
-                    const float* beta, int32_t N, int64_t HW, int32_t C, int32_t G, int32_t act, int32_t stat_rows, int32_t x_el,
-                    int32_t y_el, void* y2, int32_t y2_el, uint32_t* ovf, void* stream) {
+struct GnApplyCtx {
+    const GnApplyMulti* multi;
+    dim3 grid;
+    size_t lds;
+    hipStream_t st;
+    const void* x; void* y; void* y2;
+    const float *mean, *rstd, *gamma, *beta;
+    int64_t HW, ppb;
+    int C, G, act, stat_rows;
+    uint32_t* ovf;
+    const void* xb; int Ca;
+};
+template <typename T, bool XF32, int YEL, int Y2EL = -1>
+void gn_any_go(const GnApplyCtx& c) {
+    if constexpr (XF32) {
+        if (c.xb) {
+            hipLaunchKernelGGL((gn_apply_two_kernel<T, YEL, Y2EL>), c.grid, dim3(256), c.lds, c.st, c.x, c.xb, c.Ca, c.y, c.mean, c.rstd, c.gamma, c.beta, c.HW, c.C,
+                               c.G, c.act, c.ppb, c.stat_rows, c.y2, c.ovf);
+            return;
+        }
+    }
+    if (c.multi) hipLaunchKernelGGL((gn_apply_any_multi_kernel<T, XF32, YEL, Y2EL>), c.grid, dim3(256), c.lds, c.st, *c.multi, c.mean, c.rstd, c.gamma, c.beta,
+                                    c.C, c.G, c.act, c.stat_rows, c.ovf);
+    else hipLaunchKernelGGL((gn_apply_any_kernel<T, XF32, YEL, Y2EL>), c.grid, dim3(256), c.lds, c.st, c.x, c.y, c.mean, c.rstd, c.gamma, c.beta, c.HW, c.C, c.G,
+                            c.act, c.ppb, c.stat_rows, c.y2, c.ovf);
+}
+template <typename T>
+void gn_plain_go(const GnApplyCtx& c) {
+    if (c.multi) hipLaunchKernelGGL(gn_apply_multi_kernel<T>, c.grid, dim3(256), c.lds, c.st, *c.multi, c.mean, c.rstd, c.gamma, c.beta, c.C, c.G, c.act, c.stat_rows);
+    else hipLaunchKernelGGL(gn_apply_kernel<T>, c.grid, dim3(256), c.lds, c.st, (const T*)c.x, (T*)c.y, c.mean, c.rstd, c.gamma, c.beta, c.HW, c.C, c.G, c.act,
+                            c.ppb, c.stat_rows);
+}
+
+int gn_apply_check(const void* x, void* y, const float* mean, const float* rstd, int32_t N, int64_t HW, int32_t C, int32_t G, int32_t act, int32_t x_el,
+                   int32_t y_el, void* y2, int32_t y2_el) {
     if (!x || !y || !mean || !rstd || N <= 0 || HW <= 0 || C <= 0 || G <= 0) return OMGSR_E_BADARG;
     if ((x_el != OMGSR_EL_16 && x_el != OMGSR_EL_F32) || (y_el != OMGSR_EL_16 && y_el != OMGSR_EL_SPLIT && y_el != OMGSR_EL_MX && y_el != OMGSR_EL_MX6)) return OMGSR_E_BADARG;
     if ((y_el == OMGSR_EL_MX || y_el == OMGSR_EL_MX6) && ((C & 63) || omgsr::compute_dtype() != 1)) return OMGSR_E_SHAPE;
@@ -664,7 +847,10 @@
     if (y2 && y2_el == OMGSR_EL_MX && ((C & 63) || omgsr::compute_dtype() != 1)) return OMGSR_E_SHAPE;
     if ((C & 7) || (C % G) || C > 8192) return OMGSR_E_SHAPE;
     if (act != OMGSR_ACT_NONE && act != OMGSR_ACT_SILU) return OMGSR_E_BADARG;
-    hipStream_t st = (hipStream_t)stream;
+    return 0;
+}
+
+int64_t gn_apply_ppb(int32_t N, int64_t HW, int32_t C) {
     static const char* ppe = getenv("OMGSR_GN_BLOCK_ELEMS");
     static const int64_t belems = ppe ? atol(ppe) : 16384;
     int64_t ppb = (belems + C - 1) / C;
@@ -673,47 +859,110 @@
         ppb = (HW * N + 511) / 512;
         if (ppb < 8) ppb = 8;
     }
-    const int nblk = (int)((HW + ppb - 1) / ppb);
-    omgsr::TimingScope ts(OMGSR_TK_GN, 0.0, ((x_el == OMGSR_EL_F32 ? 4.0 : 2.0) + (y_el == OMGSR_EL_16 ? 2.0 : 4.0) +
-                                             (y2 ? (y2_el == OMGSR_EL_16 ? 2.0 : 4.0) : 0.0)) * N * (double)HW * C, st);
-    const size_t lds = 2 * C * sizeof(float);
-    const dim3 grid(nblk, N);
-#define OMGSR_GN_ANY2(YE, Y2) OMGSR_DISPATCH_T(hipLaunchKernelGGL((gn_apply_any_kernel<T, true, YE, Y2>), grid, dim3(256), lds, st, x, y, mean, rstd, gamma, beta, HW, C, G, act, ppb, stat_rows, y2, ovf))
-#define OMGSR_GN_ANY(XF, YE) OMGSR_DISPATCH_T(hipLaunchKernelGGL((gn_apply_any_kernel<T, XF, YE>), grid, dim3(256), lds, st, x, y, mean, rstd, gamma, beta, HW, C, G, act, ppb, stat_rows))
+    return ppb;
+}
+
+double gn_apply_bytes(int32_t x_el, int32_t y_el, bool has_y2, int32_t y2_el) {
+    return (x_el == OMGSR_EL_F32 ? 4.0 : 2.0) + (y_el == OMGSR_EL_16 ? 2.0 : 4.0) + (has_y2 ? (y2_el == OMGSR_EL_16 ? 2.0 : 4.0) : 0.0);
+}
+
+void gn_apply_dispatch(const GnApplyCtx& c, int32_t x_el, int32_t y_el, bool y2, int32_t y2_el) {
     if (y_el == OMGSR_EL_MX6) {
         using T = f16_t;
-#define OMGSR_GN_6(XF, Y2) hipLaunchKernelGGL((gn_apply_any_kernel<T, XF, 4, Y2>), grid, dim3(256), lds, st, x, y, mean, rstd, gamma, beta, HW, C, G, act, ppb, stat_rows, y2, ovf)
-        if (y2 && y2_el == OMGSR_EL_MX) OMGSR_GN_6(true, 3);
-        else if (y2 && y2_el == OMGSR_EL_SPLIT) OMGSR_GN_6(true, 2);
-        else if (y2) OMGSR_GN_6(true, 0);
-        else if (x_el == OMGSR_EL_F32) hipLaunchKernelGGL((gn_apply_any_kernel<T, true, 4>), grid, dim3(256), lds, st, x, y, mean, rstd, gamma, beta, HW, C, G, act, ppb, stat_rows, nullptr, nullptr);
-        else hipLaunchKernelGGL((gn_apply_any_kernel<T, false, 4>), grid, dim3(256), lds, st, x, y, mean, rstd, gamma, beta, HW, C, G, act, ppb, stat_rows, nullptr, nullptr);
-#undef OMGSR_GN_6
+        if (y2 && y2_el == OMGSR_EL_MX) gn_any_go<T, true, 4, 3>(c);
+        else if (y2 && y2_el == OMGSR_EL_SPLIT) gn_any_go<T, true, 4, 2>(c);
+        else if (y2) gn_any_go<T, true, 4, 0>(c);
+        else if (x_el == OMGSR_EL_F32) gn_any_go<T, true, 4>(c);
+        else gn_any_go<T, false, 4>(c);
     } else if (y2 && y2_el == OMGSR_EL_MX) {
         using T = f16_t;
-        if (y_el == OMGSR_EL_MX) hipLaunchKernelGGL((gn_apply_any_kernel<T, true, 3, 3>), grid, dim3(256), lds, st, x, y, mean, rstd, gamma, beta, HW, C, G, act, ppb, stat_rows, y2, ovf);
-        else if (y_el == OMGSR_EL_SPLIT) hipLaunchKernelGGL((gn_apply_any_kernel<T, true, 2, 3>), grid, dim3(256), lds, st, x, y, mean, rstd, gamma, beta, HW, C, G, act, ppb, stat_rows, y2, ovf);
-        else hipLaunchKernelGGL((gn_apply_any_kernel<T, true, 0, 3>), grid, dim3(256), lds, st, x, y, mean, rstd, gamma, beta, HW, C, G, act, ppb, stat_rows, y2, ovf);
+        if (y_el == OMGSR_EL_MX) gn_any_go<T, true, 3, 3>(c);
+        else if (y_el == OMGSR_EL_SPLIT) gn_any_go<T, true, 2, 3>(c);
+        else gn_any_go<T, true, 0, 3>(c);
     } else if (y_el == OMGSR_EL_MX) {
         using T = f16_t;
-        if (y2 && y2_el == OMGSR_EL_SPLIT) hipLaunchKernelGGL((gn_apply_any_kernel<T, true, 3, 2>), grid, dim3(256), lds, st, x, y, mean, rstd, gamma, beta, HW, C, G, act, ppb, stat_rows, y2, ovf);
-        else if (y2) hipLaunchKernelGGL((gn_apply_any_kernel<T, true, 3, 0>), grid, dim3(256), lds, st, x, y, mean, rstd, gamma, beta, HW, C, G, act, ppb, stat_rows, y2, ovf);
-        else if (x_el == OMGSR_EL_F32) hipLaunchKernelGGL((gn_apply_any_kernel<T, true, 3>), grid, dim3(256), lds, st, x, y, mean, rstd, gamma, beta, HW, C, G, act, ppb, stat_rows, nullptr, nullptr);
-        else hipLaunchKernelGGL((gn_apply_any_kernel<T, false, 3>), grid, dim3(256), lds, st, x, y, mean, rstd, gamma, beta, HW, C, G, act, ppb, stat_rows, nullptr, nullptr);
+        if (y2 && y2_el == OMGSR_EL_SPLIT) gn_any_go<T, true, 3, 2>(c);
+        else if (y2) gn_any_go<T, true, 3, 0>(c);
+        else if (x_el == OMGSR_EL_F32) gn_any_go<T, true, 3>(c);
+        else gn_any_go<T, false, 3>(c);
     } else if (y2) {
-        if (y_el == OMGSR_EL_SPLIT && y2_el == OMGSR_EL_SPLIT) OMGSR_GN_ANY2(2, 2);
-        else if (y_el == OMGSR_EL_SPLIT) OMGSR_GN_ANY2(2, 0);
-        else if (y2_el == OMGSR_EL_SPLIT) OMGSR_GN_ANY2(0, 2);
-        else OMGSR_GN_ANY2(0, 0);
-    } else if (x_el == OMGSR_EL_F32 && y_el == OMGSR_EL_SPLIT) OMGSR_GN_ANY(true, 2);
-    else if (x_el == OMGSR_EL_F32) OMGSR_GN_ANY(true, 0);
-    else if (y_el == OMGSR_EL_SPLIT) OMGSR_GN_ANY(false, 2);
-    else OMGSR_DISPATCH_T(hipLaunchKernelGGL(gn_apply_kernel<T>, grid, dim3(256), lds, st, (const T*)x,
-                                             (T*)y, mean, rstd, gamma, beta, HW, C, G, act, ppb, stat_rows));
-#undef OMGSR_GN_ANY
-#undef OMGSR_GN_ANY2
-    return (int)hipGetLastError();
-}
+        if (y_el == OMGSR_EL_SPLIT && y2_el == OMGSR_EL_SPLIT) OMGSR_DISPATCH_T((gn_any_go<T, true, 2, 2>(c)));
+        else if (y_el == OMGSR_EL_SPLIT) OMGSR_DISPATCH_T((gn_any_go<T, true, 2, 0>(c)));
+        else if (y2_el == OMGSR_EL_SPLIT) OMGSR_DISPATCH_T((gn_any_go<T, true, 0, 2>(c)));
+        else OMGSR_DISPATCH_T((gn_any_go<T, true, 0, 0>(c)));
+    } else if (x_el == OMGSR_EL_F32 && y_el == OMGSR_EL_SPLIT) OMGSR_DISPATCH_T((gn_any_go<T, true, 2>(c)));
+    else if (x_el == OMGSR_EL_F32) OMGSR_DISPATCH_T((gn_any_go<T, true, 0>(c)));
+    else if (y_el == OMGSR_EL_SPLIT) OMGSR_DISPATCH_T((gn_any_go<T, false, 2>(c)));
+    else OMGSR_DISPATCH_T(gn_plain_go<T>(c));
+}
+
+int gn_apply_launch(const void* x, void* y, const float* mean, const float* rstd, const float* gamma,
+                    const float* beta, int32_t N, int64_t HW, int32_t C, int32_t G, int32_t act, int32_t stat_rows, int32_t x_el,
+                    int32_t y_el, void* y2, int32_t y2_el, uint32_t* ovf, void* stream) {
+    if (const int e = gn_apply_check(x, y, mean, rstd, N, HW, C, G, act, x_el, y_el, y2, y2_el)) return e;
+    hipStream_t st = (hipStream_t)stream;
+    const int64_t ppb = gn_apply_ppb(N, HW, C);
+    const int nblk = (int)((HW + ppb - 1) / ppb);
+    omgsr::TimingScope ts(OMGSR_TK_GN, 0.0, gn_apply_bytes(x_el, y_el, y2 != nullptr, y2_el) * N * (double)HW * C, st);
+    const GnApplyCtx c{nullptr, dim3(nblk, N), 2 * C * sizeof(float), st, x, y, y2, mean, rstd, gamma, beta, HW, ppb, C, G, act, stat_rows, y2 ? ovf : nullptr,
+                       nullptr, 0};
+    gn_apply_dispatch(c, x_el, y_el, y2 != nullptr, y2_el);
+    return (int)hipGetLastError();
+}
+}
+
+extern "C" int omgsr_groupnorm_finalize2(const float* partial_a, int32_t nslot_a, int32_t Ca, const float* partial_b, int32_t nslot_b, int32_t Cb,
+                                         float* mean, float* rstd, float* var_out, int32_t N, int32_t G, double count, float eps, void* stream) {
+    if (!partial_a || !partial_b || !mean || !rstd || N <= 0 || G <= 0 || nslot_a <= 0 || nslot_b <= 0 || Ca <= 0 || Cb <= 0 || count <= 0.0) return OMGSR_E_BADARG;
+    if ((Ca + Cb) % G) return OMGSR_E_SHAPE;
+    hipLaunchKernelGGL(gn_finalize2_kernel, dim3(N * G), dim3(64), 0, (hipStream_t)stream, partial_a, partial_b, mean, rstd, var_out, N, G, nslot_a, nslot_b, Ca, Cb,
+                       count, eps);
+    return (int)hipGetLastError();
+}
+
+extern "C" int omgsr_groupnorm_apply2(const void* xa, const void* xb, int32_t Ca, void* y, const float* mean, const float* rstd, const float* gamma,
+                                      const float* beta, int32_t N, int64_t HW, int32_t C, int32_t G, int32_t act, int32_t y_el, void* y2, int32_t y2_el,
+                                      uint32_t* overflow_flag, void* stream) {
+    if (!xb || Ca <= 0 || Ca >= C || (Ca & 7)) return OMGSR_E_BADARG;
+    if (const int e = gn_apply_check(xa, y, mean, rstd, N, HW, C, G, act, OMGSR_EL_F32, y_el, y2, y2_el)) return e;
+    hipStream_t st = (hipStream_t)stream;
+    const int64_t ppb = gn_apply_ppb(N, HW, C);
+    const int nblk = (int)((HW + ppb - 1) / ppb);
+    omgsr::TimingScope ts(OMGSR_TK_GN, 0.0, gn_apply_bytes(OMGSR_EL_F32, y_el, y2 != nullptr, y2_el) * N * (double)HW * C, st);
+    const GnApplyCtx c{nullptr, dim3(nblk, N), 2 * C * sizeof(float), st, xa, y, y2, mean, rstd, gamma, beta, HW, ppb, C, G, act, N, y2 ? overflow_flag : nullptr,
+                       xb, Ca};
+    gn_apply_dispatch(c, OMGSR_EL_F32, y_el, y2 != nullptr, y2_el);
+    return (int)hipGetLastError();
+}
+
+extern "C" int omgsr_groupnorm_apply_multi(const omgsr_gn_apply_group* groups, int32_t ngroups, const float* mean, const float* rstd,
+                                           const float* gamma, const float* beta, int32_t C, int32_t G, int32_t act, int32_t stat_rows,
+                                           int32_t x_el, int32_t y_el, int32_t y2_el, uint32_t* overflow_flag, void* stream) {
+    if (!groups || ngroups <= 0 || ngroups > OMGSR_GN_MAX_GROUPS || stat_rows <= 0) return OMGSR_E_BADARG;
+    const bool has_y2 = groups[0].y2 != nullptr;
+    GnApplyMulti m{};
+    double elems = 0.0;
+    int64_t blocks = 0;
+    for (int k = 0; k < ngroups; ++k) {
+        const omgsr_gn_apply_group& g = groups[k];
+        if ((g.y2 != nullptr) != has_y2 || g.rows <= 0 || g.rows % stat_rows) return OMGSR_E_BADARG;
+        if (const int e = gn_apply_check(g.x, g.y, mean, rstd, g.rows, g.HW, C, G, act, x_el, y_el, g.y2, y2_el)) return e;
+        m.x[k] = g.x; m.y[k] = g.y; m.y2[k] = g.y2; m.HW[k] = g.HW;
+        m.ppb[k] = gn_apply_ppb(g.rows, g.HW, C);
+        m.nblk[k] = (int)((g.HW + m.ppb[k] - 1) / m.ppb[k]);
+        m.start[k] = (int)blocks;
+        blocks += (int64_t)m.nblk[k] * g.rows;
+        if (blocks >= (1ll << 31)) return OMGSR_E_SHAPE;
+        elems += (double)g.rows * (double)g.HW * C;
+    }
+    m.start[ngroups] = (int)blocks;
+    m.count = ngroups;
+    hipStream_t st = (hipStream_t)stream;
+    omgsr::TimingScope ts(OMGSR_TK_GN, 0.0, gn_apply_bytes(x_el, y_el, has_y2, y2_el) * elems, st);
+    const GnApplyCtx c{&m, dim3((unsigned)blocks), 2 * C * sizeof(float), st, nullptr, nullptr, nullptr, mean, rstd, gamma, beta, 0, 0, C, G, act, stat_rows,
+                       has_y2 ? overflow_flag : nullptr, nullptr, 0};
+    gn_apply_dispatch(c, x_el, y_el, has_y2, y2_el);
+    return (int)hipGetLastError();
 }
 
 namespace {
diff --git a/omgsr_amd/diffusers_api/autoencoder_kl.py b/omgsr_amd/diffusers_api/autoencoder_kl.py
--- a/omgsr_amd/diffusers_api/autoencoder_kl.py
+++ b/omgsr_amd/diffusers_api/autoencoder_kl.py
@@ -33,7 +33,10 @@
         self.nonlinearity = nn.SiLU()
 
     def nhwc(self, x, conv1_bias=None, out_for=None):
-        if self.conv_shortcut is not None and x.dtype == torch.float32:
+        if isinstance(x, tuple):
+            h, xc = self.norm1.nhwc_pair(x[0], x[1], ops.ACT_SILU, split=self.conv1.in_split(), also_cast=self.conv_shortcut.in_split())
+            h = self.conv1.nhwc(h, bias_override=conv1_bias, gn_groups=self.norm2.num_groups)
+        elif self.conv_shortcut is not None and x.dtype == torch.float32:
             h, xc = self.norm1.nhwc(x, ops.ACT_SILU, split=self.conv1.in_split(), also_cast=self.conv_shortcut.in_split())
             h = self.conv1.nhwc(h, bias_override=conv1_bias, gn_groups=self.norm2.num_groups)
         else:
diff --git a/omgsr_amd/diffusers_api/unet_2d_condition.py b/omgsr_amd/diffusers_api/unet_2d_condition.py
--- a/omgsr_amd/diffusers_api/unet_2d_condition.py
+++ b/omgsr_amd/diffusers_api/unet_2d_condition.py
@@ -283,12 +283,16 @@
             up = blk.upsamplers[0].conv if blk.upsamplers is not None else None
             for j, r in enumerate(blk.resnets):
                 last = up if j == len(blk.resnets) - 1 else None
-                h = ops.concat_channels(h, skips.pop())
+                skip = skips.pop()
+                if h.dtype == torch.float32 and r.conv_shortcut is not None:
+                    h = (h, skip)
+                else:
+                    h = ops.concat_channels(h, skip)
                 h = r.nhwc(h, fb[id(r)], out_for=last if blk.attentions is None else None)
                 if blk.attentions is not None:
                     h = blk.attentions[j].nhwc(h, ehs, out_for=last)
             if blk.upsamplers is not None:
-                h = blk.upsamplers[0].nhwc(h)
+                h = blk.upsamplers[0].nhwc(h, gn_groups=g if ops.precise() else 0)
         return self.conv_out.nhwc(h, gn=self.conv_norm_out.spec(h, ops.ACT_SILU))
 
     def forward(self, sample: torch.Tensor, timestep, encoder_hidden_states: torch.Tensor, return_dict: bool = True):
diff --git a/omgsr_amd/nn.py b/omgsr_amd/nn.py
--- a/omgsr_amd/nn.py
+++ b/omgsr_amd/nn.py
@@ -160,6 +160,10 @@
         g, b = self._affine()
         return ops.group_norm(x, g, b, self.num_groups, self.eps, act, split=split, also_cast=also_cast)
 
+    def nhwc_pair(self, a, b, act=ops.ACT_NONE, split=1, also_cast=0):
+        g, bt = self._affine()
+        return ops.group_norm_pair(a, b, g, bt, self.num_groups, self.eps, act, split=split, also_cast=also_cast)
+
     def stats(self, x):
         return ops.group_norm_stats(x, self.num_groups, self.eps)
 
@@ -176,6 +180,10 @@
         if mean.shape[0] != x.shape[0]:
             return ops.group_norm_apply_shared(x, mean, rstd, g, b, self.num_groups, act, split=split, also_cast=also_cast)
         return ops.group_norm_apply(x, mean, rstd, g, b, self.num_groups, act, split=split, also_cast=also_cast)
+
+    def apply_stats_multi(self, xs, mean, rstd, act=ops.ACT_NONE, split=1, also_cast=0):
+        g, b = self._affine()
+        return ops.group_norm_apply_multi(xs, mean, rstd, g, b, self.num_groups, act, split=split, also_cast=also_cast)
 
     def forward(self, x):
         shp = x.shape
diff --git a/omgsr_amd/ops.py b/omgsr_amd/ops.py
--- a/omgsr_amd/ops.py
+++ b/omgsr_amd/ops.py
@@ -1000,6 +1000,28 @@
     return (y, y2) if also_cast else y
 
 
+def group_norm_apply_multi(xs, mean: torch.Tensor, rstd: torch.Tensor, gamma, beta, groups: int, act: int = ACT_NONE, split: int = 1,
+                           also_cast: int = 0):
+    if not 0 < len(xs) <= _lib.GN_MAX_GROUPS:
+        raise ValueError(f"1 ... {_lib.GN_MAX_GROUPS} tile shape groups")
+    xel = _el(xs[0], "x")
+    Cc = xs[0].shape[-1]
+    if any(_el(x, "x") != xel or x.shape[-1] != Cc for x in xs):
+        raise ValueError("group_norm_apply_multi: one channel count and element kind per launch")
+    ys = [_operand_like(x, split) for x in xs]
+    y2s = [_cast_twin(x, xel, also_cast) for x in xs]
+    fused = bool(also_cast) and xel == EL_F32
+    desc = (_lib.GnApplyGroup * len(xs))()
+    for k, x in enumerate(xs):
+        desc[k].x, desc[k].y, desc[k].y2 = x.data_ptr(), ys[k].data_ptr(), (y2s[k].data_ptr() if fused else None)
+        desc[k].rows, desc[k].HW = x.shape[0], x.numel() // (x.shape[0] * Cc)
+    check(_lib.load().omgsr_groupnorm_apply_multi(desc, len(xs), mean.data_ptr(), rstd.data_ptr(), _ptr(gamma), _ptr(beta), Cc, groups, act,
+                                                  mean.shape[0], xel, _el_of_split(split), _el_of_split(also_cast) if also_cast else EL_16,
+                                                  _ovf(xs[0].device) if fused else None, _stream()),
+          "omgsr_groupnorm_apply_multi")
+    return list(zip(ys, y2s)) if also_cast else ys
+
+
 def group_norm_apply(x: torch.Tensor, mean: torch.Tensor, rstd: torch.Tensor, gamma: Optional[torch.Tensor],
                      beta: Optional[torch.Tensor], groups: int, act: int = ACT_NONE, inplace: bool = False, split: int = 1,
                      also_cast: int = 0):
@@ -1020,6 +1042,54 @@
 def group_norm(x: torch.Tensor, gamma, beta, groups: int, eps: float, act: int = ACT_NONE, split: int = 1, also_cast: int = 0):
     mean, rstd, _ = group_norm_stats(x, groups, eps)
     return group_norm_apply(x, mean, rstd, gamma, beta, groups, act, split=split, also_cast=also_cast)
+
+
+def _fused_gn_channels(x: torch.Tensor, N: int):
+    fused = getattr(x, "_omgsr_gn", None)
+    if fused is not None and fused[2] == x.data_ptr() and fused[3] == x._version and fused[0].shape[0] == N and fused[0].shape[2] == x.shape[-1]:
+        return fused[0]
+    return None
+
+
+def group_norm_pair_stats(a: torch.Tensor, b: torch.Tensor, groups: int, eps: float):
+    N, Ca, Cb = a.shape[0], a.shape[-1], b.shape[-1]
+    if not (a.dtype == torch.float32 and b.dtype == torch.float32 and a.shape[:-1] == b.shape[:-1] and Ca % 8 == 0 and Cb % 8 == 0
+            and (Ca + Cb) % groups == 0 and a.is_contiguous() and b.is_contiguous()):
+        return None
+    pa, pb = _fused_gn_channels(a, N), _fused_gn_channels(b, N)
+    if pa is None or pb is None:
+        return None
+    HW = a.numel() // (N * Ca)
+    mean = torch.empty((N, groups), device=a.device, dtype=torch.float32)
+    rstd = torch.empty_like(mean)
+    var = torch.empty_like(mean)
+    check(_lib.load().omgsr_groupnorm_finalize2(pa.data_ptr(), pa.shape[1], Ca, pb.data_ptr(), pb.shape[1], Cb, mean.data_ptr(), rstd.data_ptr(),
+                                                var.data_ptr(), N, groups, float(HW) * ((Ca + Cb) // groups), eps, _stream()),
+          "omgsr_groupnorm_finalize2")
+    return mean, rstd, var
+
+
+def group_norm_apply_pair(a: torch.Tensor, b: torch.Tensor, mean: torch.Tensor, rstd: torch.Tensor, gamma, beta, groups: int, act: int = ACT_NONE,
+                          split: int = 1, also_cast: int = 0):
+    _req(a, torch.float32, "a"); _req(b, torch.float32, "b")
+    N, Ca, Cb = a.shape[0], a.shape[-1], b.shape[-1]
+    if a.shape[:-1] != b.shape[:-1]:
+        raise ValueError("group_norm_apply_pair: a and b differ in more than the channel count")
+    HW = a.numel() // (N * Ca)
+    y = torch.empty((*a.shape[:-1], (Ca + Cb) * min(split, 2)), device=a.device, dtype=_ACT)
+    y2 = torch.empty((*a.shape[:-1], (Ca + Cb) * min(also_cast, 2)), device=a.device, dtype=_ACT) if also_cast else None
+    check(_lib.load().omgsr_groupnorm_apply2(a.data_ptr(), b.data_ptr(), Ca, y.data_ptr(), mean.data_ptr(), rstd.data_ptr(), _ptr(gamma), _ptr(beta),
+                                             N, HW, Ca + Cb, groups, act, _el_of_split(split), _ptr(y2),
+                                             _el_of_split(also_cast) if also_cast else EL_16, _ovf(a.device) if also_cast else None, _stream()),
+          "omgsr_groupnorm_apply2")
+    return (y, y2) if also_cast else y
+
+
+def group_norm_pair(a: torch.Tensor, b: torch.Tensor, gamma, beta, groups: int, eps: float, act: int = ACT_NONE, split: int = 1, also_cast: int = 0):
+    st = group_norm_pair_stats(a, b, groups, eps)
+    if st is None:
+        return group_norm(concat_channels(a, b), gamma, beta, groups, eps, act, split=split, also_cast=also_cast)
+    return group_norm_apply_pair(a, b, st[0], st[1], gamma, beta, groups, act, split=split, also_cast=also_cast)
 
 
 
diff --git a/omgsr_amd/pipelines/vaehook.py b/omgsr_amd/pipelines/vaehook.py
--- a/omgsr_amd/pipelines/vaehook.py
+++ b/omgsr_amd/pipelines/vaehook.py
@@ -121,12 +121,15 @@
                         for k in groups:
                             res[k].append(op[4].nhwc(groups[k], pad=0))
                     continue
-                for k in groups:
-                    if op[4] is not None:
-                        groups[k], xc = norm.apply_stats(groups[k], mean, rstd, act, split=op[3].in_split(), also_cast=op[4].in_split())
+                keys = list(groups)
+                if op[4] is not None:
+                    outs = norm.apply_stats_multi([groups[k] for k in keys], mean, rstd, act, split=op[3].in_split(), also_cast=op[4].in_split())
+                    for k, (y, xc) in zip(keys, outs):
+                        groups[k] = y
                         res[k].append(op[4].nhwc(xc, pad=0))
-                    else:
-                        groups[k] = norm.apply_stats(groups[k], mean, rstd, act, split=op[3].in_split())
+                else:
+                    for k, y in zip(keys, norm.apply_stats_multi([groups[k] for k in keys], mean, rstd, act, split=op[3].in_split())):
+                        groups[k] = y
             elif kind == "conv":
                 keys = list(groups)
                 for k, y in zip(keys, op[1].nhwc_multi([groups[k] for k in keys], gn=pending, **op[2])):
```

Result: faster. 20.74 images/s, median of 6 (+1.4%).
